# huggingface/tokenizers

Hardware: AMD Instinct MI355X
Metric: GB input text/sec (whole node), GPT-2 BPE encode_batch (higher is better)
Workload: dtype u8->u32

## Files before the change

### tokenizers_amd/csrc/capi/handle.cpp

```cpp

struct Workspace {
    std::mutex mu;
    std::function<uint32_t(uint32_t)> pad_exchange;
    uint32_t h_padmax = 0;
    bool busy = false;
    bool device_bound = false;
    hipStream_t bound_stream = nullptr;
    hipStream_t own_stream = nullptr;
    hipStream_t io_in = nullptr, io_out = nullptr;
    hipEvent_t ev_in[2] = {nullptr, nullptr}, ev_out[2] = {nullptr, nullptr};
    DevBuf w_l3_tiles;
    DevBuf w_ms_dmask, w_pprefix, w_pt_word;
    DevBuf w_docmask, w_startmask, w_wprefix, w_bsum, w_tile_w, w_pt_start, w_tok0, w_pt_tokoff, w_tmp_ids, w_tmp_end, w_rows;
    DevBuf w_len1, w_fin, w_fbsum, w_pad_count, w_keep, w_type_ids2, w_seq_ids2;
    DevBuf w_ovf_parts, w_enc_base, w_enc_doc, w_enc_start, w_enc_cnt;
    DevBuf w_enc_idx, w_enc_win;
    DevBuf w_queues, w_qcount, w_cstate;
    DevBuf w_doc_off;
    DevBuf w_chunk_lo;
    DevBuf w_ids, w_doc_pt, w_tok_offsets, w_scalars, w_offsets, w_word_ids;
    DevBuf dw_ids, dw_tok_off, dw_first, dw_bad, dw_dup, dw_len, dw_bsum, dw_pos, dw_out_off, dw_bytes, dw_total;
    DevBuf w_endmask, w_pt_end, w_keepmask, w_kprefix, w_ntext, w_norig, w_ndoc_off, w_slow_docs, w_leadmask, w_lprefix, w_need, w_need_bsum, w_huge, w_list_huge, w_wbase, w_norig_e, w_ids2, w_tok_offsets2, w_offsets2, w_word_ids2, w_candmask, w_matchmask, w_spanmask, w_stopmask, w_hardmask, w_boundmask, w_bprefix, w_seg_off, w_xseg_off,
        w_match_docs, w_match_list;
    DevBuf h_text, h_doc_off, h_seq_off, h_inp_off;
    DevBuf w_tok_b8;
    DevBuf w_trim1;
    const uint8_t* cur_trim1 = nullptr;
    DevBuf w_cache_keys, w_cache_rows;
    DevBuf w_claims, w_claim_rows, w_claim_pos;
    DevBuf w_phases;
    uint64_t cache_epoch = 0;
    DevBuf w_seq_off, w_seq_tok_off, w_word_idx, w_first_tok;
    std::vector<StageRec> pending;
    const uint8_t* last_text = nullptr;
    const int64_t* last_doc_off = nullptr;
    const int64_t* last_seq_off = nullptr;
    int64_t last_n_seqs = -1;
    const int64_t* last_inp_off = nullptr;
    int64_t last_n_inputs = -1;
    DevBuf w_inp_off;
    DevBuf w_mask_dirty;
    int64_t last_n_bytes = 0;
    uint32_t last_flags = 0;
    tkamd_device_result last_result{};
    int64_t last_n_docs = 0;
    int64_t last_n_enc = -1;
    int last_ntok_slot = 1;
    uint32_t last_counters[CNT_COUNT] = {0};
    bool force_general = false;
    bool last_note_added = false;
    bool last_used_claims = false;
    ~Workspace() {
        if (own_stream) (void)hipStreamDestroy(own_stream);
        if (io_in) (void)hipStreamDestroy(io_in);
        if (io_out) (void)hipStreamDestroy(io_out);
        for (int i = 0; i < 2; ++i) {
            if (ev_in[i]) (void)hipEventDestroy(ev_in[i]);
            if (ev_out[i]) (void)hipEventDestroy(ev_out[i]);
        }
    }
};

struct tkamd_tokenizer {
    HostModel hm;
    int device = -1;
    DevTables dt{};
    std::mutex mu;
    std::condition_variable cv;
    std::vector<std::unique_ptr<Workspace>> pool;
    Workspace* last_used = nullptr;
    DevBuf t_ucc1, t_ucc2;
    DevBuf t_uc1, t_uc2, t_byte_id, t_merges, t_long_blob, t_long_off, t_long_id, t_long_table;
    DevBuf t_hot;
    DevBuf t_shortw, t_shortw_k3, t_shortw_disp;
    DevBuf t_char_id;
    DevBuf t_at_id[2], t_at_flags[2], t_at_blob[2], t_at_off[2], t_at_first[2];
    DevBuf t_pp_single, t_pp_single_plain;
    DevBuf t_pp_pair, t_pp_pair_plain;
    DevBuf t_pp_prefix, t_pp_suffix, t_pp_prefix_ty, t_pp_suffix_ty, t_bn1, t_bn2, t_bn_map, t_merge_disp, t_dec_entry, t_dec_blob, t_trie;
    int n_cu = 256;
    int n_direct = 0;
    int n_hot = 0;
    int cp_grid = 0;
    std::atomic<int> claims_pause{0};
    std::atomic<int> added_spec_pause{0};
    int added_spec_len = 32;
    int claims_pause_len = 32;
    std::atomic<uint32_t> q16_div{4};
    std::atomic<bool> prof{false};
    std::atomic<bool> encode_special{false};
    std::atomic<bool> word_cache{false};
    std::atomic<uint64_t> cache_epoch{1};
    std::vector<tkamd_stage_time> acc;
    std::vector<int> devices;
    std::vector<std::unique_ptr<tkamd_tokenizer>> replicas;
    std::mutex group_mu;
    std::atomic<int> collect{0};
    std::string collect_note;
    std::vector<std::unique_ptr<DevBuf>> g_root;
    std::vector<void*> rccl_comms;
    int64_t shard_min_bytes = 1 << 20;
    std::vector<double> shard_ms;
    std::vector<int64_t> shard_bytes;
};

constexpr size_t PHASE_WGS = 1 << 17;
constexpr size_t MAX_HOST_WORKSPACES = 4;

struct PinnedBlock {
    void* p = nullptr;
    size_t cap = 0;
};
static std::mutex g_pin_mu;
static std::vector<PinnedBlock> g_pin_free;

static PinnedBlock pinned_get(size_t bytes) {
    if (bytes < 64) bytes = 64;
    {
        std::lock_guard<std::mutex> lk(g_pin_mu);
        size_t best = (size_t)-1;
        for (size_t i = 0; i < g_pin_free.size(); ++i)
            if (g_pin_free[i].cap >= bytes && (best == (size_t)-1 || g_pin_free[i].cap < g_pin_free[best].cap)) best = i;
        if (best != (size_t)-1 && g_pin_free[best].cap <= 2 * bytes + (1u << 20)) {
            PinnedBlock b = g_pin_free[best];
            g_pin_free.erase(g_pin_free.begin() + best);
            return b;
        }
    }
    PinnedBlock b;
    size_t want = bytes + bytes / 8;
    HIP_CHECK(hipHostMalloc(&b.p, want, hipHostMallocPortable));
    b.cap = want;
    return b;
}
static void pinned_put(PinnedBlock b) {
    if (!b.p || g_forked) return;
    std::lock_guard<std::mutex> lk(g_pin_mu);
    if (g_pin_free.size() >= 16) { (void)hipHostFree(b.p); return; }
    g_pin_free.push_back(b);
}

struct tkamd_batch {
    int64_t n_docs = 0, n_tokens = 0;
    PinnedBlock ids, tok_offsets, offsets, word_ids, pad_counts, type_ids, seq_ids, enc_docs, enc_parts;
    bool has_offsets = false, has_words = false, has_pads = false, has_types = false, has_enc_docs = false, has_enc_parts = false;
    ~tkamd_batch() { pinned_put(ids); pinned_put(tok_offsets); pinned_put(offsets); pinned_put(word_ids); pinned_put(pad_counts); pinned_put(type_ids); pinned_put(seq_ids); pinned_put(enc_docs); pinned_put(enc_parts); }
};

struct tkamd_text {
    int64_t n_docs = 0, n_bytes = 0;
    PinnedBlock bytes, doc_offsets;
    ~tkamd_text() { pinned_put(bytes); pinned_put(doc_offsets); }
};
```

### tokenizers_amd/csrc/capi/pipeline.cpp

```cpp

int lookup_grid(const tkamd_tokenizer* t) { return std::min(3 * t->n_cu, (int)NSQ); }

struct QueueSizes {
    uint32_t sq_cap[4], row_base[4];
    size_t total;
};
static bool rerun_wanted(tkamd_tokenizer* t, Workspace* w, int raw) {
    const int err = raw & ~NOTE_BITS;
    bool again = false;
    if (raw & NOTE_ADDED_SEEN) { t->added_spec_pause = t->added_spec_len; w->force_general = true; again = true; }
    if (err == ERR_QUEUE_FULL && t->q16_div > 1) { t->q16_div = t->q16_div > 2 ? 2 : 1; again = true; }
    return again;
}

QueueSizes queue_sizes(size_t N, uint32_t q16_div, int grid) {
    QueueSizes z{};
    const size_t n_tiles = N / LOOKUP_TILE_BYTES + 1;
    const size_t per_sq = ((n_tiles + grid - 1) / grid) * LOOKUP_TILE_BYTES;
    z.sq_cap[0] = (uint32_t)(per_sq / q16_div + 64);
    z.sq_cap[1] = (uint32_t)(per_sq / 17 + 16);
    z.sq_cap[2] = (uint32_t)(per_sq / 33 + 16);
    z.sq_cap[3] = (uint32_t)(per_sq / 65 + 16);
    size_t acc = 0;
    for (int c = 0; c < 4; ++c) { z.row_base[c] = (uint32_t)acc; acc += (size_t)z.sq_cap[c] * (size_t)grid; }
    z.total = acc;
    return z;
}

void reserve_workspace(tkamd_tokenizer* t, Workspace* w, int64_t n_bytes, int64_t n_docs, uint32_t flags, bool want_meta) {
    int64_t W = (n_bytes >> 6) + 2;
    size_t N = (size_t)n_bytes;
    w->w_docmask.reserve(W * 8);
    w->w_startmask.reserve(W * 8);
    w->w_wprefix.reserve(W * 4);
    w->w_bsum.reserve((W / 256 + 2) * 4);
    w->w_tok0.reserve((N + 4) * 4);
    w->w_tmp_ids.reserve((N + 4) * 4);
    const QueueSizes z = queue_sizes(N, t->q16_div, lookup_grid(t));
    w->w_rows.reserve(z.total * 16);
    w->w_queues.reserve(z.total * 8);
    w->w_cstate.reserve((N / COMPACT_CHUNK + 4) * 8 + 16);
    w->w_chunk_lo.reserve((N / COMPACT_CHUNK + 4) * 4);
    w->w_qcount.reserve((size_t)QCNT_WORDS * 4);
    w->w_pt_tokoff.reserve((N + 4) * 4);
    w->w_ids.reserve((N + 4) * 4);
    w->w_doc_pt.reserve((n_docs + 2) * 4);
    w->w_tok_offsets.reserve((n_docs + 2) * 8);
    w->w_scalars.reserve(SC_SLOTS * 8);
    if (want_meta) w->w_pt_start.reserve((N + 4) * 4);
    if (flags & TKAMD_OFFSETS_MASK) {
        w->w_tmp_end.reserve((N + 4) * 4);
        w->w_offsets.reserve((N + 4) * 8);
    }
    if (flags & TKAMD_WANT_WORD_IDS) w->w_word_ids.reserve((N + 4) * 4);
}

void run_pipeline(tkamd_tokenizer* t, Workspace* w, const uint8_t* d_text, const int64_t* d_doc_off, int64_t n_docs, int64_t n_bytes,
                  const int64_t* d_seq_off, int64_t n_seqs, uint32_t flags, hipStream_t st, tkamd_device_result* out,
                  const int64_t* d_inp_off = nullptr, int64_t n_inputs = -1) {
    HostModel& hm = t->hm;
    const int64_t* const d_doc_off_in = d_doc_off;
    const int64_t* const d_seq_off_in = d_seq_off;
    const int64_t* const d_inp_off_in = d_inp_off;
    const bool mixed = n_inputs >= 0;
    if (mixed && (flags & TKAMD_PAIRS)) throw Invalid("a mixed batch names the kind of every input itself: TKAMD_PAIRS must not be set");
    if (mixed && !d_inp_off) throw Invalid("null input offsets");
    bool rerun = false;
    const uint32_t off_mode = flags & TKAMD_OFFSETS_MASK;
    const bool want_words = (flags & TKAMD_WANT_WORD_IDS) != 0;
    const bool want_meta = off_mode != TKAMD_OFFSETS_NONE || want_words;
    if (off_mode == 3u) throw Invalid("bad offsets mode");
    const bool add_special = (flags & TKAMD_ADD_SPECIAL) != 0 && !(hm.pp_prefix.empty() && hm.pp_suffix.empty());
    if ((flags & TKAMD_ADD_SPECIAL) && !(flags & TKAMD_PAIRS) && !hm.pp_unsupported.empty()) throw Unsupported("add_special_tokens: " + hm.pp_unsupported);
    if (!(flags & TKAMD_PAIRS) && hm.pp_single_refused) throw Unsupported("post_processor: " + hm.pp_unsupported);
    if (mixed && (flags & TKAMD_ADD_SPECIAL) && !hm.pp_pair_unsupported.empty()) throw Unsupported("add_special_tokens on a pair: " + hm.pp_pair_unsupported);
    const bool prefix_space = hm.byte_level && hm.add_prefix_space;
    const bool metaspace = hm.pretok == PT_METASPACE;
    size_t at_min_len = (size_t)-1;
    for (int c = 0; c < 2; ++c)
        for (size_t k = 0; k + 1 < hm.at[c].off.size(); ++k) at_min_len = std::min<size_t>(at_min_len, hm.at[c].off[k + 1] - hm.at[c].off[k]);
    const bool have_added_tokens = at_min_len != (size_t)-1;
    const uint32_t mcap = have_added_tokens ? (uint32_t)std::min<size_t>((size_t)n_bytes / std::max<size_t>(at_min_len, 1) + 16, 0x7FFFFFF0u) : 0u;
    const int64_t n_x = (hm.norm == NORM_BERT) ? 3 * n_bytes + 64
                        : metaspace ? 3 * n_bytes + 3 * (n_docs + 2 * (int64_t)mcap + 1) + 64
                        : n_bytes + (prefix_space ? n_docs + (int64_t)mcap : 0);
    if (n_x >= (int64_t)0xFFFFFF00ll) throw Invalid("batch larger than 4 GiB: split it (byte offsets are 32-bit on the device)");
    const bool bpe_path = hm.model == MODEL_BPE && !hm.char_bpe && (hm.pretok == PT_BYTELEVEL_GPT2 || hm.pretok == PT_LLAMA3 || hm.pretok == PT_BYTELEVEL_NOREGEX);
    const bool local_pretok = hm.pretok == PT_WHITESPACE || hm.pretok == PT_WHITESPACE_SPLIT || hm.pretok == PT_BERT;
    const bool word_models = (hm.model == MODEL_WORDLEVEL || hm.model == MODEL_WORDPIECE) && local_pretok;
    const bool char_bpe = hm.model == MODEL_BPE && hm.char_bpe && (local_pretok || metaspace);
    if (!bpe_path && !word_models && !char_bpe)
        throw Unsupported("this build covers {ByteLevel(GPT-2 regex), Llama-3 Split+ByteLevel, ByteLevel(no regex)}+BPE and "
                          "{Whitespace,WhitespaceSplit,BertPreTokenizer}+{WordLevel,WordPiece,BPE over characters} and the U+2581 front+BPE over characters");
    if (prefix_space && hm.norm != NORM_NONE) throw Unsupported("ByteLevel add_prefix_space behind a normalizer");

    reserve_workspace(t, w, n_x, n_docs, flags, want_meta);
    int64_t* sc = w->w_scalars.as<int64_t>();
    int64_t* d_npretok = sc + SC_NPRETOK;
    int64_t* d_ntok_total = sc + SC_NTOK;
    int64_t* d_xlen = sc + SC_NKEPT;
    int* d_err = (int*)(sc + SC_ERR);
    uint32_t* d_counters = (uint32_t*)(sc + SC_COUNTERS);
    const int64_t W0 = (n_bytes >> 6) + 1;
    const int64_t W = (n_x >> 6) + 1;
    const int grid = t->n_cu * 8;
    Prof pf{t, w, st};
    using ull = unsigned long long;

    const char* const claims_hook = test_hook("TKAMD_CLAIMS");
    const bool claims_on = !(claims_hook && !strcmp(claims_hook, "0"));
    constexpr bool len_bound = true;
    bool use_claims = claims_on && !t->word_cache &&
                      (hm.model == MODEL_BPE || (hm.model == MODEL_WORDPIECE && hm.max_input_chars >= (uint32_t)WORD_MAX_KEY));
    if (use_claims) {
        int p = t->claims_pause.load();
        while (p > 0 && !t->claims_pause.compare_exchange_weak(p, p - 1)) {}
        if (p > 0) use_claims = false;
    }
    w->last_used_claims = use_claims;
    size_t claim_slots = 0;
    const size_t cstate_bytes = (((size_t)n_x / (size_t)COMPACT_CHUNK + 4) * 8 + 15) & ~(size_t)15;
    {
        ZeroRegions z{};
        z.add(sc, SC_SLOTS * 8);
        if (!(len_bound && (hm.norm == NORM_BERT || metaspace))) z.add(w->w_docmask.p, (size_t)(W + 1) * 8);
        z.add(w->w_qcount.p, (size_t)QCNT_WORDS * 4);
        z.add(w->w_cstate.p, cstate_bytes);
        if (hm.pretok == PT_LLAMA3 && split_rule_fast(hm.split_rule)) {
            w->w_l3_tiles.reserve(l3_tileflag_words(n_x) * 8);
            z.add(w->w_l3_tiles.p, l3_tileflag_words(n_x) * 8);
        }
        if (use_claims) {
            constexpr size_t per_slot = 64;
            int bits = 18;
            while (bits < 24 && ((size_t)1 << bits) < (size_t)n_bytes / per_slot) ++bits;
            claim_slots = (size_t)1 << bits;
            w->w_claims.reserve(claim_slots * 16);
            w->w_claim_rows.reserve(claim_slots * 16);
            z.add(w->w_claims.p, claim_slots * 16);
        }
        launch_zero_regions(st, t->n_cu * 4, z);
    }
    out->d_ids = w->w_ids.as<uint32_t>();
    out->d_tok_offsets = w->w_tok_offsets.as<int64_t>();
    out->d_offsets = nullptr;
    out->d_word_ids = nullptr;
    out->d_n_tokens = d_ntok_total;
    out->d_n_pretokens = d_npretok;
    out->ids_capacity = n_x + 4;
    w->last_n_docs = n_docs;
    w->cur_trim1 = nullptr;
    w->last_n_enc = -1;
    out->d_enc_docs = nullptr;
    out->d_n_encodings = nullptr;
    w->last_seq_off = d_seq_off;
    w->last_n_seqs = n_seqs;
    w->last_inp_off = d_inp_off;
    w->last_n_inputs = n_inputs;
    w->w_doc_off.reserve((size_t)(n_docs + 2) * 8);
    const bool lean = n_bytes > 0 && hm.at[0].size() == 0 && hm.at[1].size() == 0 && hm.norm == NORM_NONE && !prefix_space &&
                      (hm.pretok == PT_BYTELEVEL_GPT2 || hm.pretok == PT_BYTELEVEL_NOREGEX);
    const int64_t* const raw_doc_off = d_doc_off;
    if (!lean) {
        pf.begin("validate_csr");
        launch_validate_csr(st, d_doc_off, n_docs, n_bytes, d_err, w->w_doc_off.as<int64_t>());
        pf.end();
    }
    d_doc_off = w->w_doc_off.as<int64_t>();
    const bool words_in = n_seqs >= 0;
    if (words_in) {
        if (!d_seq_off) throw Invalid("null sequence offsets");
        w->w_seq_off.reserve((size_t)(n_seqs + 2) * 8);
        w->w_seq_tok_off.reserve((size_t)(n_seqs + 2) * 8);
        launch_validate_csr(st, d_seq_off, n_seqs, n_docs, d_err, w->w_seq_off.as<int64_t>());
        d_seq_off = w->w_seq_off.as<int64_t>();
        out->d_tok_offsets = w->w_seq_tok_off.as<int64_t>();
    }
    const int64_t* const e_tok_off = words_in ? w->w_seq_tok_off.as<int64_t>() : w->w_tok_offsets.as<int64_t>();
    const int64_t e_n = words_in ? n_seqs : n_docs;
    if (mixed) {
        w->w_inp_off.reserve((size_t)(n_inputs + 2) * 8);
        launch_validate_csr(st, d_inp_off, n_inputs, e_n, d_err, w->w_inp_off.as<int64_t>());
        d_inp_off = w->w_inp_off.as<int64_t>();
    }
    auto add_specials = [&]() {
        const size_t T2 = (size_t)n_x + 4 + (size_t)(e_n + 1) * (hm.pp_prefix.size() + hm.pp_suffix.size());
        w->w_ids2.reserve(T2 * 4);
        w->w_tok_offsets2.reserve((size_t)(e_n + 2) * 8);
        if (out->d_offsets) w->w_offsets2.reserve(T2 * 8);
        if (out->d_word_ids) w->w_word_ids2.reserve(T2 * 4);
        SpecialArgs sa{};
        sa.tok_offsets = e_tok_off;
        sa.n_docs = e_n;
        sa.ids = w->w_ids.as<uint32_t>();
        sa.offsets = out->d_offsets;
        sa.word_ids = out->d_word_ids;
        sa.prefix = t->t_pp_prefix.as<uint32_t>();
        sa.suffix = t->t_pp_suffix.as<uint32_t>();
        sa.n_prefix = (int32_t)hm.pp_prefix.size();
        sa.n_suffix = (int32_t)hm.pp_suffix.size();
        sa.tok_offsets2 = w->w_tok_offsets2.as<int64_t>();
        sa.ids2 = w->w_ids2.as<uint32_t>();
        sa.offsets2 = w->w_offsets2.as<uint32_t>();
        sa.word_ids2 = w->w_word_ids2.as<uint32_t>();
        sa.n_tok2 = sc + SC_NTOK2;
        pf.begin("add_specials");
        launch_add_specials(st, grid, sa);
        pf.end();
        out->d_ids = sa.ids2;
        out->ids_capacity = (int64_t)T2;
        out->d_tok_offsets = sa.tok_offsets2;
        if (out->d_offsets) out->d_offsets = sa.offsets2;
        if (out->d_word_ids) out->d_word_ids = sa.word_ids2;
        out->d_n_tokens = sa.n_tok2;
    };
    out->d_pad_counts = nullptr;
    out->d_type_ids = nullptr;
    out->d_seq_ids = nullptr;
    const bool pairs = (flags & TKAMD_PAIRS) != 0 || mixed;
    if (pairs && !mixed && (e_n & 1)) throw Invalid("TKAMD_PAIRS: an odd number of documents");
    if (pairs && (flags & TKAMD_ADD_SPECIAL) && !hm.pp_pair_unsupported.empty()) throw Unsupported("add_special_tokens on a pair: " + hm.pp_pair_unsupported);
    const bool typed_single = !pairs && hm.pp_single_typed;
    const bool epilogue = hm.trunc_on || hm.pad_on || pairs || typed_single;
    const bool want_overflow = (flags & TKAMD_WANT_OVERFLOW) != 0 && hm.trunc_on;
    out->d_enc_parts = nullptr;
    auto batch_longest = [&](uint32_t* d_target, bool* again) -> uint64_t {
        int64_t head[SC_PADMAX + 1];
        HIP_CHECK(hipMemcpyAsync(head, sc, sizeof(head), hipMemcpyDeviceToHost, st));
        uint32_t mx = 0;
        if (d_target != (uint32_t*)(sc + SC_PADMAX)) HIP_CHECK(hipMemcpyAsync(&mx, d_target, 4, hipMemcpyDeviceToHost, st));
        HIP_CHECK(hipStreamSynchronize(st));
        if (d_target == (uint32_t*)(sc + SC_PADMAX)) mx = *(const uint32_t*)&head[SC_PADMAX];
        if (!w->pad_exchange) return mx;
        if (rerun_wanted(t, w, *(const int*)&head[SC_ERR])) {
            *again = true;
            return 0;
        }
        const uint32_t all = w->pad_exchange(mx);
        if (all != mx) {
            w->h_padmax = all;
            HIP_CHECK(hipMemcpyAsync(d_target, &w->h_padmax, 4, hipMemcpyHostToDevice, st));
        }
        return all;
    };
    auto finalize_pairs = [&]() {
        const int64_t n_pairs = mixed ? n_inputs : e_n / 2;
        const bool tpl_on = (flags & TKAMD_ADD_SPECIAL) && !hm.pp_pair.empty();
        uint32_t n_special = 0;
        if (tpl_on) for (const HostModel::TplPiece& q : hm.pp_pair) n_special += q.kind == 2u;
        PairArgs pa{};
        pa.tok_offsets = e_tok_off;
        pa.n_pairs = n_pairs;
        if (mixed) {
            pa.inp_off = d_inp_off;
            pa.tpl1 = add_special ? t->t_pp_single.as<uint32_t>() : t->t_pp_single_plain.as<uint32_t>();
            pa.n_tpl1 = add_special ? (int32_t)hm.pp_single.size() : (int32_t)hm.pp_single_plain.size();
            pa.n_special1 = add_special ? (uint32_t)(hm.pp_prefix.size() + hm.pp_suffix.size()) : 0u;
        }
        const uint32_t n_special_max = std::max(n_special, pa.n_special1);
        pa.ids = w->w_ids.as<uint32_t>();
        pa.offsets = out->d_offsets;
        pa.word_ids = out->d_word_ids;
        pa.trim1 = pa.offsets ? w->cur_trim1 : nullptr;
        w->w_keep.reserve((size_t)(std::max(e_n, 2 * n_pairs) + 2) * 4);
        pa.tpl = tpl_on ? t->t_pp_pair.as<uint32_t>() : t->t_pp_pair_plain.as<uint32_t>();
        pa.n_tpl = tpl_on ? (int32_t)hm.pp_pair.size() : (int32_t)hm.pp_pair_plain.size();
        pa.n_special = n_special;
        pa.ovf_ty_tpl = (tpl_on && hm.pp_roberta) ? 1u : 0u;
        pa.trunc_on = hm.trunc_on ? 1u : 0u;
        pa.trunc_max = hm.trunc_max_length;
        pa.trunc_left = hm.trunc_left ? 1u : 0u;
        pa.trunc_strategy = (uint32_t)hm.trunc_strategy;
        pa.trunc_stride = hm.trunc_stride;
        pa.pad_on = hm.pad_on ? 1u : 0u;
        pa.pad_fixed = hm.pad_fixed ? 1u : 0u;
        pa.pad_length = hm.pad_length;
        pa.pad_multiple = hm.pad_multiple;
        pa.pad_left = hm.pad_left ? 1u : 0u;
        pa.pad_id = hm.pad_id;
        pa.pad_type_id = hm.pad_type_id;
        w->w_fbsum.reserve((size_t)((n_pairs + 1) / 256 + 2) * 4);
        pa.keep = w->w_keep.as<uint32_t>();
        pa.bsum = w->w_fbsum.as<uint32_t>();
        pa.target = (uint32_t*)(sc + SC_PADMAX);
        pa.n_tok2 = sc + SC_NTOK2;
        pa.err = d_err;
        for (int32_t k = 0; k < pa.n_tpl; ++k) {
            const uint32_t kind = (tpl_on ? hm.pp_pair : hm.pp_pair_plain)[(size_t)k].kind;
            if (kind < 2u) { pa.first_is_b = kind == 1u ? 1u : 0u; break; }
        }
        pf.begin("pair_epilogue");
        int64_t n_enc = n_pairs;
        bool overflow = want_overflow;
        if (overflow) {
            w->w_ovf_parts.reserve((size_t)(n_pairs + 2) * 4);
            w->w_enc_base.reserve((size_t)(n_pairs + 2) * 8);
            pa.ovf_parts = w->w_ovf_parts.as<uint32_t>();
            pa.enc_base = w->w_enc_base.as<int64_t>();
        } else {
            w->w_len1.reserve((size_t)(n_pairs + 2) * 4);
            pa.len1 = w->w_len1.as<uint32_t>();
        }
        launch_pair_lens(st, pa);
        if (overflow) {
            launch_pair_overflow_scan(st, pa, sc + SC_NENC);
            int64_t head[SC_NENC + 1];
            HIP_CHECK(hipMemcpyAsync(head, sc, sizeof(head), hipMemcpyDeviceToHost, st));
            HIP_CHECK(hipStreamSynchronize(st));
            const int err_now = *(const int*)&head[SC_ERR] & ~NOTE_BITS;
            if (rerun_wanted(t, w, *(const int*)&head[SC_ERR])) {
                rerun = true;
                pf.end();
                return;
            }
// ... 291 lines not shown
    if (have_added) HIP_CHECK(hipMemsetAsync(n_match, 0, 4, st));
    if (spec && setA.size() > 0) {
        pf.begin("added_token_match");
        launch_added_detect(st, args_of(0), d_text, n_bytes, nullptr, d_err);
        pf.end();
    }
    if (have_raw) {
        pf.begin("added_token_match");
        launch_added_match(st, args_of(0), d_text, n_bytes, nullptr, d_doc_off, n_docs, nullptr, nullptr, t->dt.uc1, t->dt.uc2, w->w_candmask.as<ull>(),
                           w->w_match_docs.as<uint32_t>(), d_counters + CNT_MATCH_DOCS, mlist, n_match, mcap, MATCH_LEN_ORIG, d_err);
        pf.end();
    }

    const uint8_t* x_text = d_text;
    bool lead_done = false;
    const int64_t* x_doc_off = d_doc_off;
    const int64_t* x_len_dev = nullptr;
    const uint32_t* norig = nullptr;
    const uint32_t* norig_e = nullptr;
    if (hm.norm == NORM_BERT || prefix_space || metaspace) {
        w->w_ntext.reserve((size_t)n_x + TKAMD_TEXT_PAD);
        w->w_ndoc_off.reserve((size_t)(n_docs + 2) * 8);
        if (hm.norm != NORM_BERT && !metaspace) HIP_CHECK(hipMemsetAsync(w->w_ntext.p, 0, (size_t)n_x + TKAMD_TEXT_PAD, st));
        else if (test_hook("TKAMD_POISON_NTEXT")) {
            HIP_CHECK(hipMemsetAsync(w->w_ntext.p, 0xFF, (size_t)n_x + TKAMD_TEXT_PAD, st));
            if (len_bound) HIP_CHECK(hipMemsetAsync(w->w_docmask.p, 0xFF, w->w_docmask.cap, st));
            HIP_CHECK(hipMemsetAsync(w->w_startmask.p, 0xFF, w->w_startmask.cap, st));
            HIP_CHECK(hipMemsetAsync(w->w_wprefix.p, 0xFF, w->w_wprefix.cap, st));
            if (w->w_endmask.p) HIP_CHECK(hipMemsetAsync(w->w_endmask.p, 0xFF, w->w_endmask.cap, st));
        }
        if (off_mode != TKAMD_OFFSETS_NONE) {
            w->w_norig.reserve(((size_t)n_x + 4) * 4);
            norig = w->w_norig.as<uint32_t>();
            if (hm.norm != NORM_BERT && !metaspace) {
                w->w_norig_e.reserve(((size_t)n_x + 4) * 4);
                norig_e = w->w_norig_e.as<uint32_t>();
            }
        }
    }
    if (hm.norm == NORM_BERT) {
        w->w_keepmask.reserve(bn_olen_bytes(n_bytes));
        w->w_kprefix.reserve((size_t)(W0 + 1) * 4);
        w->w_wbase.reserve((size_t)(W0 + 1) * 4);
        BnTables bt{t->t_bn1.as<uint16_t>(), t->t_bn2.as<uint8_t>(), t->t_bn_map.as<MergeSlot>(), hm.bn_mask, hm.bn_seed,
                    hm.bn_clean_text, hm.bn_handle_chinese, hm.bn_strip_accents, hm.bn_lowercase};
        const ull* verbatim = nullptr;
        if (have_raw) {
            scatter_masks(n_bytes, nullptr, false);
            launch_mask_or2(st, w->w_boundmask.as<ull>(), w->w_matchmask.as<ull>(), w->w_spanmask.as<ull>(), W0 + 1);
            verbatim = w->w_boundmask.as<ull>();
        }
        pf.begin("bert_normalize");
        launch_bert_normalize(st, bt, d_text, n_bytes, d_doc_off, n_docs, verbatim, w->w_keepmask.as<uint8_t>(), w->w_kprefix.as<uint32_t>(),
                              w->w_bsum.as<uint32_t>(), w->w_wbase.as<uint32_t>(), d_xlen, w->w_ntext.as<uint8_t>(), (uint32_t*)norig, (uint32_t*)norig_e,
                              w->w_ndoc_off.as<int64_t>(), d_err);
        launch_zero_tail(st, w->w_ntext.as<uint8_t>(), d_xlen, TKAMD_TEXT_PAD, len_bound ? w->w_docmask.as<ull>() : nullptr, W + 1, t->n_cu * 4);
        pf.end();
        if (have_raw) launch_translate_matches_norm(st, mlist, n_match, w->w_keepmask.as<uint8_t>(), w->w_wbase.as<uint32_t>(), n_bytes, d_xlen);
        x_text = w->w_ntext.as<uint8_t>();
        x_doc_off = w->w_ndoc_off.as<int64_t>();
        x_len_dev = d_xlen;
    }
    const int64_t n_in = hm.norm == NORM_BERT ? n_x : n_bytes;
    if (spec && setB.size() > 0) {
        pf.begin("added_token_match2");
        launch_added_detect(st, args_of(1), x_text, n_in, x_len_dev, d_err);
        pf.end();
    }
    if (have_norm) {
        const int64_t* seg = x_doc_off;
        const int64_t* nseg_dev = nullptr;
        int64_t nseg_bound = n_docs;
        if (have_raw) {
            scatter_masks(n_in, x_len_dev, false);
            seg = build_pieces(x_doc_off, n_in, x_len_dev);
            nseg_dev = d_nseg;
            nseg_bound = (int64_t)seg_cap;
        }
        pf.begin("added_token_match2");
        launch_added_match(st, args_of(1), x_text, n_in, x_len_dev, seg, nseg_bound, nseg_dev, have_raw ? w->w_matchmask.as<ull>() : nullptr, t->dt.uc1, t->dt.uc2,
                           w->w_candmask.as<ull>(), w->w_match_docs.as<uint32_t>(), d_counters + CNT_MATCH_DOCS2, mlist, n_match, mcap,
                           hm.norm == NORM_NONE ? MATCH_LEN_ORIG : 0u, d_err);
        pf.end();
    }
    if (have_added && !prefix_space && !metaspace) {
        scatter_masks(n_in, x_len_dev, off_mode != TKAMD_OFFSETS_NONE);
        matchmask = w->w_matchmask.as<ull>();
    }
    const int64_t* piece_off = nullptr;
    const int64_t* piece_n_dev = nullptr;
    if (prefix_space) {
        const int64_t* seg = d_doc_off;
        const int64_t* nseg_dev = nullptr;
        int64_t nseg_bound = n_docs;
        if (have_added) {
            scatter_masks(n_bytes, nullptr, false);
            seg = build_pieces(d_doc_off, n_bytes, nullptr);
            nseg_dev = d_nseg;
            nseg_bound = (int64_t)seg_cap;
            w->w_xseg_off.reserve((seg_cap + 2) * 8);
        }
        w->w_need.reserve((size_t)(nseg_bound + 2) * 4);
        w->w_need_bsum.reserve((size_t)((nseg_bound + 1) / 256 + 2) * 4);
        int64_t* xseg = have_added ? w->w_xseg_off.as<int64_t>() : w->w_ndoc_off.as<int64_t>();
        pf.begin("prefix_space");
        launch_prefix_space(st, d_text, seg, nseg_bound, nseg_dev, have_added ? w->w_matchmask.as<ull>() : nullptr, w->w_need.as<uint32_t>(),
                            w->w_need_bsum.as<uint32_t>(), xseg, d_xlen, w->w_ntext.as<uint8_t>(), (uint32_t*)norig, (uint32_t*)norig_e, grid);
        if (have_added) {
            launch_prefix_doc_csr(st, d_doc_off, n_docs, w->w_boundmask.as<ull>(), w->w_bprefix.as<uint32_t>(), n_bytes, nullptr, d_nseg, xseg, w->w_ndoc_off.as<int64_t>());
            launch_translate_matches_prefix(st, mlist, n_match, w->w_boundmask.as<ull>(), w->w_bprefix.as<uint32_t>(), n_bytes, nullptr, d_nseg, xseg);
        }
        pf.end();
        x_text = w->w_ntext.as<uint8_t>();
        x_doc_off = w->w_ndoc_off.as<int64_t>();
        x_len_dev = d_xlen;
        if (have_added) {
            scatter_masks(n_x, x_len_dev, off_mode != TKAMD_OFFSETS_NONE);
            matchmask = w->w_matchmask.as<ull>();
            piece_off = xseg;
            piece_n_dev = d_nseg;
        }
    } else if (metaspace) {
        w->w_ms_dmask.reserve((size_t)(W0 + 2) * 8);
        HIP_CHECK(hipMemsetAsync(w->w_ms_dmask.p, 0, (size_t)(W0 + 2) * 8, st));
        launch_mark_doc_starts_n(st, d_doc_off, n_docs, n_bytes, nullptr, w->w_ms_dmask.as<ull>(), d_err);
        const ull* pstart = w->w_ms_dmask.as<ull>();
        if (have_added) {
            scatter_masks(n_bytes, nullptr, false);
            build_pieces(d_doc_off, n_bytes, nullptr);
            pstart = w->w_boundmask.as<ull>();
        }
        w->w_keepmask.reserve(bn_olen_bytes(n_bytes));
        w->w_kprefix.reserve((size_t)(W0 + 1) * 4);
        w->w_wbase.reserve((size_t)(W0 + 1) * 4);
        pf.begin("metaspace");
        launch_metaspace(st, d_text, n_bytes, d_doc_off, n_docs, pstart, w->w_ms_dmask.as<ull>(), have_added ? w->w_matchmask.as<ull>() : nullptr,
                         have_added ? w->w_spanmask.as<ull>() : nullptr, (uint32_t)hm.ms_prepend, w->w_keepmask.as<uint8_t>(), w->w_kprefix.as<uint32_t>(),
                         w->w_bsum.as<uint32_t>(), w->w_wbase.as<uint32_t>(), d_xlen, w->w_ntext.as<uint8_t>(), (uint32_t*)norig, w->w_ndoc_off.as<int64_t>());
        launch_zero_tail(st, w->w_ntext.as<uint8_t>(), d_xlen, TKAMD_TEXT_PAD, len_bound ? w->w_docmask.as<ull>() : nullptr, W + 1, t->n_cu * 4);
        pf.end();
        if (have_added) launch_translate_matches_norm(st, mlist, n_match, w->w_keepmask.as<uint8_t>(), w->w_wbase.as<uint32_t>(), n_bytes, d_xlen);
        x_text = w->w_ntext.as<uint8_t>();
        x_doc_off = w->w_ndoc_off.as<int64_t>();
        x_len_dev = d_xlen;
        if (have_added) {
            scatter_masks(n_x, x_len_dev, off_mode != TKAMD_OFFSETS_NONE);
            matchmask = w->w_matchmask.as<ull>();
        }
    } else if (have_added && hm.pretok == PT_LLAMA3) {
        piece_off = build_pieces(x_doc_off, n_in, x_len_dev);
        piece_n_dev = d_nseg;
    }

    pf.begin("mark_doc_starts");
    launch_mark_doc_starts_n(st, lean ? raw_doc_off : x_doc_off, n_docs, n_x, x_len_dev, w->w_docmask.as<ull>(), d_err);
    if (matchmask) launch_mask_or(st, w->w_docmask.as<ull>(), w->w_hardmask.as<ull>(), W, n_match);
    pf.end();

    uint32_t* pt_end = nullptr;
    bool has_end = false;
    bool meta_masks = false;
    auto after_masks = [&]() {
        if (want_meta && !meta_masks) {
            pf.begin("emit_pretok");
            launch_emit_pretok(st, w->w_startmask.as<ull>(), w->w_wprefix.as<uint32_t>(), n_x, x_len_dev, d_npretok, w->w_pt_start.as<uint32_t>());
            if (pt_end) launch_emit_pretok_end(st, w->w_startmask.as<ull>(), w->w_endmask.as<ull>(), w->w_wprefix.as<uint32_t>(), n_x, x_len_dev, pt_end);
            pf.end();
        }
        pf.begin("doc_first_pretok");
        launch_doc_first_pretok(st, lean ? raw_doc_off : x_doc_off, n_docs, n_x, w->w_startmask.as<ull>(), w->w_wprefix.as<uint32_t>(),
                                d_npretok, w->w_doc_pt.as<uint32_t>(), w->w_chunk_lo.as<uint32_t>(),
                                lean ? d_err : nullptr, lean ? w->w_doc_off.as<int64_t>() : nullptr);
        pf.end();
    };
    if (hm.pretok == PT_BYTELEVEL_GPT2) {
        pf.begin("pretok_gpt2_seq");
        if (off_mode == TKAMD_OFFSETS_CHAR && x_text == d_text && !x_len_dev && n_x == n_bytes) {
            w->w_leadmask.reserve((size_t)(W0 + 1) * 8);
            lead_done = true;
        }
        launch_pretok_gpt2(st, x_text, n_x, x_len_dev, w->w_docmask.as<ull>(), t->dt.uc1, t->dt.uc2, w->w_startmask.as<ull>(), lead_done ? w->w_leadmask.as<ull>() : nullptr);
        pf.end();
    } else if (hm.pretok == PT_LLAMA3) {
        w->w_endmask.reserve((size_t)(W + 1) * 8);
        w->w_slow_docs.reserve((size_t)(n_docs + 1) * 4);
        if (off_mode == TKAMD_OFFSETS_CHAR && x_text == d_text && !x_len_dev && n_x == n_bytes && (split_rule_fast(hm.split_rule) || (split_rule_fast_cs(hm.split_rule) && t->t_ucc1.p))) {
            w->w_leadmask.reserve((size_t)(W0 + 1) * 8);
            lead_done = true;
        }
        pf.begin("pretok_llama3");
        w->w_slow_docs.reserve((size_t)((piece_off ? seg_cap : (size_t)n_docs) + 1) * 4);
        launch_pretok_llama3(st, x_text, n_x, x_len_dev, w->w_docmask.as<ull>(), t->dt.uc1, t->dt.uc2, w->w_startmask.as<ull>(),
                             w->w_endmask.as<ull>(), piece_off ? piece_off : x_doc_off, piece_off ? (int64_t)seg_cap : n_docs, piece_n_dev,
                             w->w_slow_docs.as<uint32_t>(), d_counters + CNT_SLOW_DOCS, hm.split_rule,
                             t->t_ucc1.p ? t->t_ucc1.as<uint16_t>() : nullptr, t->t_ucc2.p ? t->t_ucc2.as<uint8_t>() : nullptr,
                             w->w_l3_tiles.p ? w->w_l3_tiles.as<ull>() : nullptr, lead_done ? w->w_leadmask.as<ull>() : nullptr);
        pf.end();
    } else if (metaspace) {
        pf.begin("metaspace_units");
        launch_ms_units(st, x_text, n_x, x_len_dev, w->w_docmask.as<ull>(), w->w_startmask.as<ull>(), W, hm.ms_split);
        pf.end();
    } else if (hm.pretok == PT_BYTELEVEL_NOREGEX) {
        HIP_CHECK(hipMemcpyAsync(w->w_startmask.p, w->w_docmask.p, (size_t)W * 8, hipMemcpyDeviceToDevice, st));
    } else {
        w->w_endmask.reserve((size_t)(W + 1) * 8);
        has_end = true;
        if (want_meta) {
            w->w_pt_end.reserve(((size_t)n_x + 4) * 4);
            pt_end = w->w_pt_end.as<uint32_t>();
        }
        pf.begin("pretok_local");
        launch_pretok_local(st, (int)hm.pretok, x_text, n_x, x_len_dev, w->w_docmask.as<ull>(), t->dt.uc1, t->dt.uc2,
                            w->w_startmask.as<ull>(), w->w_endmask.as<ull>(), len_bound);
        pf.end();
    }
    if (matchmask)
        launch_apply_matches(st, w->w_startmask.as<ull>(), has_end ? w->w_endmask.as<ull>() : nullptr, matchmask, w->w_spanmask.as<ull>(),
                             w->w_stopmask.as<ull>(), W, n_match);
    {
        pf.begin("mask_scan");
        meta_masks = want_meta && !(hm.char_bpe && !hm.unk_configured && !hm.byte_fallback);
        if (meta_masks) w->w_tile_w.reserve(((size_t)n_x / META_TILE + 4) * 4);
        launch_mask_scan(st, w->w_startmask.as<ull>(), W, w->w_bsum.as<uint32_t>(), w->w_wprefix.as<uint32_t>(), d_npretok, len_bound ? x_len_dev : nullptr,
                         meta_masks ? w->w_tile_w.as<uint32_t>() : nullptr);
        pf.end();
        after_masks();
    }

    const uint32_t* pt_word = nullptr;
    if (metaspace && !hm.ms_split && want_words && !words_in) {
        w->w_pprefix.reserve((size_t)(W + 2) * 4);
        w->w_pt_word.reserve(((size_t)n_x + 4) * 4);
        pf.begin("metaspace_words");
        launch_mask_scan(st, w->w_docmask.as<ull>(), W, w->w_bsum.as<uint32_t>(), w->w_pprefix.as<uint32_t>(), sc + SC_NPIECE, len_bound ? x_len_dev : nullptr);
        launch_ms_piece_rank(st, w->w_startmask.as<ull>(), w->w_wprefix.as<uint32_t>(), w->w_docmask.as<ull>(), w->w_pprefix.as<uint32_t>(), n_x, x_len_dev,
                             w->w_pt_word.as<uint32_t>());
        pf.end();
        pt_word = w->w_pt_word.as<uint32_t>();
    }

    uint32_t* tmp_end = (off_mode != TKAMD_OFFSETS_NONE) ? w->w_tmp_end.as<uint32_t>() : nullptr;
    const size_t N = (size_t)n_x;
    const QueueSizes qz = queue_sizes(N, t->q16_div, lookup_grid(t));
    static const size_t row_limit = [] { const char* e = test_hook("TKAMD_ROW_LIMIT_BITS"); return e ? std::min<size_t>((size_t)1 << std::max(8, atoi(e)), ROW_INDEX_LIMIT) : (size_t)ROW_INDEX_LIMIT; }();
    if (qz.total >= row_limit) throw Invalid("batch too large for the work queues (row indices are 30-bit: about 3 GB of text): split it");
    QueuePlan plan{};
    for (int c = 0; c < 4; ++c) {
        plan.v[c].q = (QItem*)(w->w_queues.as<uint8_t>() + (size_t)qz.row_base[c] * 8);
        plan.v[c].counts = w->w_qcount.as<uint32_t>() + (size_t)c * NSQ * QCNT_STRIDE;
        plan.v[c].sq_cap = qz.sq_cap[c];
        plan.v[c].row_base = qz.row_base[c];
    }
    const ull* endmask = has_end ? w->w_endmask.as<ull>() : nullptr;
    const bool phases_on = test_hook("TKAMD_PHASES") != nullptr;
    auto phases_of = [&](int which) -> void* {
        if (!phases_on) return nullptr;
        if (!w->w_phases.p) {
            w->w_phases.reserve(2 * PHASE_WGS * 64);
            HIP_CHECK(hipMemsetAsync(w->w_phases.p, 0, 2 * PHASE_WGS * 64, st));
        }
        return (uint8_t*)w->w_phases.p + (size_t)which * PHASE_WGS * 64;
    };
    WordCache wc{nullptr, nullptr, nullptr, 0u, nullptr};
    auto open_word_cache = [&]() {
        const size_t slots = (size_t)1 << WORD_CACHE_BITS;
        if (use_claims) {
            uint32_t* cpos = nullptr;
            if (off_mode != TKAMD_OFFSETS_NONE) { w->w_claim_pos.reserve(claim_slots * 4); cpos = w->w_claim_pos.as<uint32_t>(); }
            wc = WordCache{nullptr, w->w_claim_rows.p, (unsigned long long*)w->w_claims.p, (uint32_t)(claim_slots - 1), cpos};
            return;
        }
        if (!t->word_cache || off_mode != TKAMD_OFFSETS_NONE) return;
        w->w_cache_keys.reserve(slots * sizeof(CacheKey));
        w->w_cache_rows.reserve(slots * 16);
        const uint64_t epoch = t->cache_epoch;
        if (w->cache_epoch != epoch) {
            HIP_CHECK(hipMemsetAsync(w->w_cache_keys.p, 0, slots * sizeof(CacheKey), st));
            w->cache_epoch = epoch;
        }
        wc = WordCache{(CacheKey*)w->w_cache_keys.p, w->w_cache_rows.p, nullptr, 0u, nullptr};
    };
    DevTables mdt = t->dt;
    mdt.err = d_err;
    mdt.probes = t->prof ? d_counters + CNT_MERGE_PROBES : nullptr;
    auto set_publish = [&]() {
        if (wc.claims) { mdt.pub_rows = wc.rows; mdt.pub_mask = wc.claim_mask; mdt.pub_pos = wc.claim_pos; }
    };
    if (hm.model == MODEL_BPE) {
        pf.begin("lookup");
        open_word_cache();
        set_publish();
        launch_lookup(st, lookup_grid(t), t->dt, x_text, n_x, x_len_dev, w->w_startmask.as<ull>(), endmask, w->w_wprefix.as<uint32_t>(),
                      w->w_tok0.as<uint32_t>(), plan, d_err, matchmask, t->t_hot.p, wc, 0u, 0u, phases_of(0), d_counters);
        pf.end();
        if (hm.ignore_merges)
            launch_long_vocab3(st, t->n_cu, t->dt, x_text, plan.v[1], plan.v[2], plan.v[3], w->w_rows.p, 0u, d_err, wc);
        const bool lds16 = t->dt.newid_affine && !test_hook("TKAMD_FORCE_LANE_MERGE");
        const bool lds32 = lds16;
        const bool can_one = wc.claims && lds16 && lds32 && !test_hook("TKAMD_MERGE_TWO");
        const char* const pair_hook = test_hook("TKAMD_MERGE_PAIR");
        const bool pair = can_one && !(pair_hook && pair_hook[0] == '0');
        const bool one = can_one && !pair;
        const size_t huge_words = std::min<size_t>((size_t)6 * N + 4096, (size_t)1 << 28);
        const bool huge_possible = N > (size_t)LONG_PT_MAX;
        if (huge_possible) {
            w->w_huge.reserve(huge_words * 4);
            w->w_list_huge.reserve((N / LONG_PT_MAX + 16) * 4);
        } else {
            w->w_huge.reserve(64);
            w->w_list_huge.reserve(64);
        }
        if (hm.char_bpe) {
            auto long_only = [&](const QView& q) {
                launch_bpe_merge_long_only(st, t->n_cu * 2, mdt, x_text, q, w->w_rows.p, w->w_tmp_ids.as<uint32_t>(), tmp_end, w->w_list_huge.as<uint32_t>(), d_counters + CNT_LISTH);
            };
            pf.begin("bpe_merge_lds32");
            if (t->dt.newid_affine) launch_bpe_merge(st, t->n_cu, 6, mdt, x_text, plan.v[1], w->w_rows.p, w->w_tmp_ids.as<uint32_t>(), tmp_end, nullptr);
            else long_only(plan.v[1]);
            pf.end();
            pf.begin("bpe_merge_lds");
            if (t->dt.newid_affine) launch_bpe_merge(st, t->n_cu, 5, mdt, x_text, plan.v[0], w->w_rows.p, w->w_tmp_ids.as<uint32_t>(), tmp_end);
            else long_only(plan.v[0]);
            pf.end();
            pf.begin("bpe_merge_long");
            long_only(plan.v[2]);
            launch_bpe_merge_long(st, t->n_cu, mdt, x_text, plan.v[3], w->w_rows.p, w->w_tmp_ids.as<uint32_t>(), tmp_end, w->w_list_huge.as<uint32_t>(),
                                  d_counters + CNT_LISTH, w->w_huge.as<uint32_t>(), (unsigned long long)(huge_possible ? huge_words : 0),
                                  (unsigned long long*)(sc + SC_HUGE_USED), d_err);
            pf.end();
        } else {
        if (pair) {
            pf.begin("bpe_merge_lds_pair");
            launch_bpe_merge_pair(st, t->n_cu, mdt, x_text, plan.v[0], plan.v[1], w->w_rows.p, w->w_tmp_ids.as<uint32_t>(), tmp_end);
            pf.end();
        } else {
            pf.begin(lds32 ? "bpe_merge_lds32" : "bpe_merge_lane32");
            launch_bpe_merge(st, lds32 ? t->n_cu : grid, lds32 ? 6 : 2, mdt, x_text, plan.v[1], w->w_rows.p, w->w_tmp_ids.as<uint32_t>(), tmp_end, one ? &plan.v[0] : nullptr);
            pf.end();
        }
        if (!can_one) {
            pf.begin(lds16 ? "bpe_merge_lds" : "bpe_merge_lane");
            launch_bpe_merge(st, lds16 ? t->n_cu : grid, lds16 ? 5 : 1, mdt, x_text, plan.v[0], w->w_rows.p, w->w_tmp_ids.as<uint32_t>(), tmp_end);
            pf.end();
        }
        pf.begin("bpe_merge64");
        launch_bpe_merge(st, grid, 64, mdt, x_text, plan.v[2], w->w_rows.p, w->w_tmp_ids.as<uint32_t>(), tmp_end);
        pf.end();
        pf.begin("bpe_merge_long");
        launch_bpe_merge_long(st, t->n_cu, mdt, x_text, plan.v[3], w->w_rows.p,
                              w->w_tmp_ids.as<uint32_t>(), tmp_end, w->w_list_huge.as<uint32_t>(), d_counters + CNT_LISTH, w->w_huge.as<uint32_t>(),
                              (unsigned long long)(huge_possible ? huge_words : 0), (unsigned long long*)(sc + SC_HUGE_USED), d_err);
        pf.end();
        }
        if (wc.keys) {
            pf.begin("word_cache_insert");
            launch_word_cache_insert(st, grid, mdt, x_text, plan.v[0], w->w_rows.p, wc);
            pf.end();
        }
    } else if (hm.model == MODEL_WORDLEVEL) {
        DevTables wt = t->dt;
        wt.ignore_merges = 1;
        pf.begin("wordlevel_lookup");
        launch_lookup(st, lookup_grid(t), wt, x_text, n_x, x_len_dev, w->w_startmask.as<ull>(), endmask, w->w_wprefix.as<uint32_t>(),
                      w->w_tok0.as<uint32_t>(), plan, d_err, matchmask, t->t_hot.p, WordCache{nullptr, nullptr, nullptr, 0u, nullptr}, 0u, 1u, nullptr, nullptr);
        launch_long_vocab3(st, t->n_cu, wt, x_text, plan.v[1], plan.v[2], plan.v[3], w->w_rows.p, 1u, d_err, WordCache{nullptr, nullptr, nullptr, 0u, nullptr});
        pf.end();
    } else {
        const bool shortcut = hm.max_input_chars >= (uint32_t)WORD_MAX_KEY;
        DevTables wt = t->dt;
        wt.ignore_merges = 1;
        wt.long_probe_max_len = hm.max_input_chars;
        if (shortcut) open_word_cache();
        set_publish();
        pf.begin("wordpiece_word_lookup");
        launch_lookup(st, lookup_grid(t), wt, x_text, n_x, x_len_dev, w->w_startmask.as<ull>(), endmask, w->w_wprefix.as<uint32_t>(),
                      w->w_tok0.as<uint32_t>(), plan, d_err, matchmask, t->t_hot.p, wc, shortcut ? 0u : 1u, 0u, phases_of(0), d_counters);
        pf.end();
        pf.begin("wordpiece");
        launch_wordpiece_all(st, grid, t->n_cu, mdt, x_text, plan, w->w_rows.p, w->w_tmp_ids.as<uint32_t>(), tmp_end, d_err);
        pf.end();
        if (wc.keys) {
            pf.begin("word_cache_insert");
            launch_word_cache_insert(st, grid, t->dt, x_text, plan.v[0], w->w_rows.p, wc);
            pf.end();
        }
    }
    if (matchmask)
        launch_apply_match_ids(st, w->w_match_list.as<uint32_t>(), d_counters + CNT_MATCHES, w->w_startmask.as<ull>(),
                               w->w_wprefix.as<uint32_t>(), w->w_tok0.as<uint32_t>());
    uint8_t* tok_b8 = nullptr;
    if (tmp_end) { w->w_tok_b8.reserve((size_t)n_x + 64); tok_b8 = w->w_tok_b8.as<uint8_t>(); }
    pf.begin("compact");
    launch_compact(st, t->cp_grid, w->w_tok0.as<uint32_t>(), w->w_rows.p, wc.rows, w->w_tmp_ids.as<uint32_t>(), d_npretok, w->w_cstate.as<ull>(),
                   d_ntok_total, want_meta ? w->w_pt_tokoff.as<uint32_t>() : nullptr, w->w_ids.as<uint32_t>(), w->w_chunk_lo.as<uint32_t>(),
                   w->w_doc_pt.as<uint32_t>(), n_docs, w->w_tok_offsets.as<int64_t>(), (size_t)t->cp_grid <= PHASE_WGS ? phases_of(1) : nullptr, tok_b8);
    pf.end();
    const uint32_t* word_of_doc = nullptr;
    const int64_t* first_tok = nullptr;
    if (words_in) {
        if (want_words) { w->w_word_idx.reserve((size_t)(n_docs + 2) * 4); word_of_doc = w->w_word_idx.as<uint32_t>(); }
        if (off_mode != TKAMD_OFFSETS_NONE && hm.trim_offsets) { w->w_first_tok.reserve((size_t)(n_docs + 2) * 8); first_tok = w->w_first_tok.as<int64_t>(); }
        launch_seq_regroup(st, d_seq_off, n_seqs, n_docs, w->w_tok_offsets.as<int64_t>(), w->w_seq_tok_off.as<int64_t>(), (uint32_t*)word_of_doc, (int64_t*)first_tok);
    }
    if (want_meta) {
        MetaArgs a{};
        a.word_of_doc = word_of_doc;
        a.pt_word = pt_word;
        a.first_tok = first_tok;
        a.x_text = x_text;
        a.text = d_text;
        a.pt_start = meta_masks ? nullptr : w->w_pt_start.as<uint32_t>();
        a.pt_end = meta_masks ? nullptr : pt_end;
        a.startmask = w->w_startmask.as<ull>();
        a.endmask = has_end ? w->w_endmask.as<ull>() : nullptr;
        a.wprefix = w->w_wprefix.as<uint32_t>();
        a.tile_w = meta_masks ? w->w_tile_w.as<uint32_t>() : nullptr;
        a.n_mask_words = W;
        a.x_len_dev = x_len_dev;
        a.x_len_host = n_x;
        a.n_tok = d_ntok_total;
        a.pt_tokoff = w->w_pt_tokoff.as<uint32_t>();
        a.tmp_end = tmp_end;
        a.tok_b8 = tok_b8;
        a.tok0 = wc.claims ? w->w_tok0.as<uint32_t>() : nullptr;
        a.claim_pos = wc.claims ? wc.claim_pos : nullptr;
        a.n_pretok = d_npretok;
        a.doc_pt = w->w_doc_pt.as<uint32_t>();
        a.chunk_lo = w->w_chunk_lo.as<uint32_t>();
        a.chunk = (uint32_t)COMPACT_CHUNK;
        a.n_docs = n_docs;
        a.x_doc_off = x_doc_off;
        a.doc_off = d_doc_off;
        a.norig = norig;
        a.norig_e = norig_e;
        a.byte_level = hm.byte_level;
        a.snap_chars = hm.byte_level || hm.char_bpe;
        if (hm.char_bpe && !hm.unk_configured && !hm.byte_fallback) {
            a.char_id = t->dt.char_id;
            a.cb = t->dt.cb;
            if (hm.ignore_merges) { a.ww_tok0 = w->w_tok0.as<uint32_t>(); a.ww_rows = w->w_rows.p; a.ww_crows = wc.rows; }
        }
        a.trim_offsets = hm.trim_offsets;
        a.trim_matches_only = !hm.byte_level;
        a.pp_add_prefix_space = hm.pp_add_prefix_space;
        a.want_offsets = off_mode != TKAMD_OFFSETS_NONE;
        a.char_mode = off_mode == TKAMD_OFFSETS_CHAR;
        a.want_words = want_words;
        a.matchmask = matchmask;
        a.uc1 = t->dt.uc1;
        a.uc2 = t->dt.uc2;
        a.offsets = w->w_offsets.as<uint32_t>();
        a.word_ids = w->w_word_ids.as<uint32_t>();
        if (a.want_offsets && a.trim_offsets && a.pp_add_prefix_space && hm.trunc_on) {
            w->w_trim1.reserve((size_t)n_x + 8);
            a.trim1 = w->w_trim1.as<uint8_t>();
            w->cur_trim1 = a.trim1;
        }
        if (a.char_mode) {
            w->w_leadmask.reserve((size_t)(W0 + 1) * 8);
            w->w_lprefix.reserve((size_t)(W0 + 1) * 4);
            pf.begin("leadmask_scan");
            if (!lead_done) launch_leadmask(st, d_text, n_bytes, w->w_leadmask.as<ull>());
            launch_mask_scan(st, w->w_leadmask.as<ull>(), W0, w->w_bsum.as<uint32_t>(), w->w_lprefix.as<uint32_t>(), sc + SC_NCHARS);
            pf.end();
            a.leadmask = w->w_leadmask.as<ull>();
            a.lprefix = w->w_lprefix.as<uint32_t>();
        }
        pf.begin("token_meta");
        launch_token_meta(st, grid, a);
        pf.end();
        if (a.want_offsets) out->d_offsets = a.offsets;
        if (a.want_words) out->d_word_ids = a.word_ids;
    }
    if (pairs) finalize_pairs();
    else if (epilogue) finalize();
    else if (add_special) add_specials();
    if (rerun) {
        run_pipeline(t, w, d_text, d_doc_off_in, n_docs, n_bytes, d_seq_off_in, n_seqs, flags, st, out, d_inp_off_in, n_inputs);
        return;
    }
    w->last_ntok_slot = (add_special || epilogue) ? SC_NTOK2 : SC_NTOK;
    HIP_CHECK(hipGetLastError());
}

int read_scalars(tkamd_tokenizer* t, Workspace* w, hipStream_t st, int64_t* n_tok, int64_t* n_pretok);

int finish_batch(tkamd_tokenizer* t, Workspace* w, hipStream_t st, int64_t* n_tok, int64_t* n_pretok) {
    int bits = read_scalars(t, w, st, n_tok, n_pretok);
    while (rerun_wanted(t, w, bits | (w->last_note_added ? NOTE_ADDED_SEEN : 0))) {
        tkamd_device_result again{};
        run_pipeline(t, w, w->last_text, w->last_doc_off, w->last_n_docs, w->last_n_bytes, w->last_seq_off, w->last_n_seqs, w->last_flags, st, &again,
                     w->last_inp_off, w->last_n_inputs);
        if (again.d_ids != w->last_result.d_ids || again.d_tok_offsets != w->last_result.d_tok_offsets ||
            again.d_offsets != w->last_result.d_offsets || again.d_word_ids != w->last_result.d_word_ids || again.d_pad_counts != w->last_result.d_pad_counts || again.d_type_ids != w->last_result.d_type_ids ||
            again.d_enc_docs != w->last_result.d_enc_docs) {
            if (w->device_bound) throw HipError("result buffers moved while a batch was run again");
            w->last_result = again;
        }
        bits = read_scalars(t, w, st, n_tok, n_pretok);
    }
    return bits;
}

int read_scalars(tkamd_tokenizer* t, Workspace* w, hipStream_t st, int64_t* n_tok, int64_t* n_pretok) {
// ... 55 lines not shown
```

### tokenizers_amd/csrc/kernels.hpp

```cpp
#pragma once
#include <hip/hip_runtime_api.h>
#include <cstdint>

#include "tables.hpp"

namespace tkamd {

struct DevTables {
    const uint16_t* uc1;
    const uint8_t* uc2;
    const uint32_t* byte_id;
    const MergeSlot* merges;
    const uint16_t* merge_disp;
    uint32_t merge_mask, merge_seed, merge_bmask;
    uint32_t newid_affine, newid_base;
    const uint32_t* char_id;
    uint32_t cb;
    int* err;
    uint32_t* probes;
    void* pub_rows;
    uint32_t* pub_pos;
    uint32_t pub_mask;
    uint32_t word_seed;
    const void* shortw;
// ... 96 lines not shown
    uint32_t byte_level, trim_offsets, pp_add_prefix_space, want_offsets, char_mode, want_words;
    uint32_t trim_matches_only;
    uint32_t snap_chars;
    const uint32_t* char_id;
    uint32_t cb;
    const uint32_t* ww_tok0;
    const void* ww_rows;
    const void* ww_crows;
    const unsigned long long* matchmask;
    const uint16_t* uc1;
    const uint8_t* uc2;
    uint32_t* offsets;
    uint32_t* word_ids;
    uint8_t* trim1;
};

struct AddedArgs {
    const uint8_t* blob;
    const uint32_t* off;
    const uint32_t* first;
    const uint32_t* id;
    const uint32_t* flags;
    unsigned long long first_set[4];
    uint32_t n_first;
    uint32_t first_byte[4];
    uint32_t skip_special;
};

struct SpecialArgs {
    const int64_t* tok_offsets;
    int64_t n_docs;
    const uint32_t* ids;
    const uint32_t* offsets;
    const uint32_t* word_ids;
    const uint32_t* prefix;
    const uint32_t* suffix;
    int32_t n_prefix, n_suffix;
    int64_t* tok_offsets2;
    uint32_t* ids2;
    uint32_t* offsets2;
    uint32_t* word_ids2;
    int64_t* n_tok2;
};

struct FinalArgs {
    const int64_t* tok_offsets;
    int64_t n_docs;
    const uint32_t* ids;
    const uint32_t* offsets;
    const uint32_t* word_ids;
    const uint8_t* trim1;
    const uint32_t* prefix;
    const uint32_t* suffix;
    int32_t n_prefix, n_suffix;
    uint32_t trunc_len;
    uint32_t trunc_left;
    uint32_t trunc_needs_pair;
    uint32_t trunc_stride;
    uint32_t pad_on, pad_fixed, pad_length, pad_multiple, pad_left, pad_id;
    uint32_t* ovf_parts;
    int64_t* enc_base;
    uint32_t* enc_doc;
    uint32_t* enc_start;
    uint32_t* enc_cnt;
    uint32_t* len1;
    uint32_t* fin;
    uint32_t* target;
    uint32_t* bsum;
    int64_t* tok_offsets2;
    uint32_t* ids2;
    uint32_t* offsets2;
    uint32_t* word_ids2;
    uint32_t* pad_count;
    int64_t* n_tok2;
    int* err;
    uint8_t* type_ids2;
    uint8_t* seq_ids2;
    const uint8_t* prefix_ty;
    const uint8_t* suffix_ty;
    uint32_t seq_ty;
    uint32_t pad_type_id;
};

struct PairArgs {
    const int64_t* tok_offsets;
    int64_t n_pairs;
    const uint32_t* ids;
    const uint32_t* offsets;
    const uint32_t* word_ids;
    const uint8_t* trim1;
    const uint32_t* tpl;
    int32_t n_tpl;
    uint32_t n_special;
    const int64_t* inp_off;
    const uint32_t* tpl1;
    int32_t n_tpl1;
    uint32_t n_special1;
    uint32_t trunc_on, trunc_max, trunc_left, trunc_strategy, trunc_stride;
    uint32_t pad_on, pad_fixed, pad_length, pad_multiple, pad_left, pad_id, pad_type_id;
    uint32_t* keep;
    uint32_t first_is_b;
    uint32_t ovf_ty_tpl;
    uint32_t* ovf_parts;
    int64_t* enc_base;
    uint32_t* enc_doc;
    uint32_t* enc_idx;
    uint32_t* enc_win;
    uint32_t* len1;
    uint32_t* fin;
    uint32_t* target;
    uint32_t* bsum;
    int64_t* tok_offsets2;
    uint32_t* ids2;
    uint32_t* offsets2;
    uint32_t* word_ids2;
    uint8_t* type_ids2;
    uint8_t* seq_ids2;
    uint32_t* pad_count;
    int64_t* n_tok2;
    int* err;
};

enum : int {
    ERR_BAD_OFFSETS = 1,
    ERR_PRETOKEN_TOO_LONG = 2,
    ERR_ADDED_SPLIT = 4,
    ERR_NON_ASCII_NORM = 8,
    ERR_MISSING_UNK = 16,
    ERR_INTERNAL = 32,
    ERR_QUEUE_FULL = 64,
    ERR_TRUNC_SECOND = 128,
    ERR_TOO_MANY_TOKENS = 256,
    ERR_TRUNC_SHORT = 512,
    ERR_TRUNC_STRIDE = 1024,
    ERR_INPUT_KIND = 8192,
    ERR_UNK_OOV = 4096,
    NOTE_REORDER_SEEN = 2048,
    NOTE_ADDED_SEEN = 16384,
    NOTE_BITS = NOTE_REORDER_SEEN | NOTE_ADDED_SEEN,
    ERR_QUEUE_FULL_PAD = 0,
};

enum : int { CNT_LIST16 = 0, CNT_LIST64 = 1, CNT_LISTL = 2, CNT_LIST32 = 3, CNT_SLOW_DOCS = 4, CNT_CLAIM_CANDS = 5, CNT_CLAIM_SHARED = 6, CNT_LISTH = 7, CNT_MATCH_DOCS = 8,
              CNT_MATCHES = 9, CNT_MATCH_DOCS2 = 10, CNT_CLAIM_GAVE_UP = 11, CNT_MERGE_PROBES = 12, CNT_COUNT = 13 };

constexpr uint32_t MATCH_LEN_ORIG = 0x80000000u;
constexpr int TEXT_PAD = 64;
constexpr int LONG_PT_MAX = 8192;

void launch_mark_doc_starts(hipStream_t st, const int64_t* doc_off, int64_t n_docs, int64_t n_bytes,
                            unsigned long long* docmask, int* err);
void launch_validate_csr(hipStream_t st, const int64_t* doc_off, int64_t n_docs, int64_t n_bytes, int* err, int64_t* san);
void launch_pretok_gpt2(hipStream_t st, const uint8_t* text, int64_t n_bytes, const int64_t* len_dev, const unsigned long long* docmask,
                        const uint16_t* uc1, const uint8_t* uc2, unsigned long long* startmask, unsigned long long* leadmask = nullptr);
void launch_mask_scan(hipStream_t st, const unsigned long long* mask, int64_t n_words, uint32_t* bsum, uint32_t* wprefix,
                      int64_t* total, const int64_t* len_dev = nullptr, uint32_t* tile_w = nullptr);
void launch_emit_pretok(hipStream_t st, const unsigned long long* startmask, const uint32_t* wprefix, int64_t n_bytes,
                        const int64_t* len_dev, const int64_t* n_pretok, uint32_t* pt_start);
void launch_prefix_space(hipStream_t st, const uint8_t* text, const int64_t* seg_off, int64_t n_bound, const int64_t* n_dev, const unsigned long long* matchmask,
                         uint32_t* need, uint32_t* bsum, int64_t* xseg_off, int64_t* x_len, uint8_t* xtext, uint32_t* nos, uint32_t* noe, int grid);
void launch_doc_first_pretok(hipStream_t st, const int64_t* doc_off, int64_t n_docs, int64_t n_bytes,
                             const unsigned long long* startmask, const uint32_t* wprefix, const int64_t* n_pretok, uint32_t* doc_pt, uint32_t* chunk_lo,
                             const int* err = nullptr, int64_t* san = nullptr);
void launch_lookup(hipStream_t st, int grid, const DevTables& t, const uint8_t* text, int64_t n_bytes, const int64_t* len_dev,
                   const unsigned long long* startmask, const unsigned long long* endmask, const uint32_t* wprefix, uint32_t* tok0,
                   const QueuePlan& plan, int* err, const unsigned long long* matchmask, const void* hot, const WordCache& wc,
                   uint32_t no_hits, uint32_t miss_is_unk, void* phases = nullptr, uint32_t* counters = nullptr);
void launch_bpe_merge(hipStream_t st, int grid, int group, const DevTables& t, const uint8_t* text, const QView& v, void* rows,
                      uint32_t* tmp_ids, uint32_t* tmp_end, const QView* also = nullptr);
void launch_bpe_merge_pair(hipStream_t st, int n_cu, const DevTables& t, const uint8_t* text, const QView& v16, const QView& v32, void* rows,
                           uint32_t* tmp_ids, uint32_t* tmp_end);
int pair_merge_occupancy();
inline size_t bn_olen_bytes(int64_t n_bytes) { return (((size_t)n_bytes + 64 + 15) & ~(size_t)15) + ((size_t)n_bytes >> 4) + 64; }
inline uint8_t* bn_ltot_of(uint8_t* olen, int64_t n_bytes) { return olen + (((size_t)n_bytes + 64 + 15) & ~(size_t)15); }
void launch_mark_doc_starts_n(hipStream_t st, const int64_t* doc_off, int64_t n_docs, int64_t n_bytes, const int64_t* len_dev,
                              unsigned long long* docmask, int* err);
void launch_pretok_local(hipStream_t st, int kind, const uint8_t* text, int64_t n_bytes, const int64_t* len_dev, const unsigned long long* docmask,
                         const uint16_t* uc1, const uint8_t* uc2, unsigned long long* startmask, unsigned long long* endmask, bool len_bound = false);
void launch_emit_pretok_end(hipStream_t st, const unsigned long long* startmask, const unsigned long long* endmask,
                            const uint32_t* wprefix, int64_t n_bytes, const int64_t* len_dev, uint32_t* pt_end);
void launch_bert_normalize(hipStream_t st, const BnTables& bt, const uint8_t* text, int64_t n_bytes, const int64_t* doc_off, int64_t n_docs,
                           const unsigned long long* verbatim, uint8_t* olen, uint32_t* wsum, uint32_t* bsum, uint32_t* wbase, int64_t* x_len, uint8_t* ntext,
                           uint32_t* nos, uint32_t* noe, int64_t* ndoc_off, int* err);
void launch_long_vocab3(hipStream_t st, int grid, const DevTables& t, const uint8_t* text, const QView& v1, const QView& v2, const QView& v3, void* rows, uint32_t miss_is_unk,
                        int* err, const WordCache& wc);
void launch_wordpiece_all(hipStream_t st, int grid_short, int grid_long, const DevTables& t, const uint8_t* text, const QueuePlan& plan, void* rows, uint32_t* tmp_ids,
                          uint32_t* tmp_end, int* err);
void launch_pretok_llama3(hipStream_t st, const uint8_t* text, int64_t n_bytes, const int64_t* len_dev, const unsigned long long* docmask,
                          const uint16_t* uc1, const uint8_t* uc2, unsigned long long* startmask, unsigned long long* slowmask,
                          const int64_t* doc_off, int64_t n_docs, const int64_t* n_docs_dev, uint32_t* slow_docs, uint32_t* n_slow_docs,
                          SplitRule rule, const uint16_t* ucc1, const uint8_t* ucc2, unsigned long long* tileflags, unsigned long long* leadmask = nullptr);
inline size_t l3_tileflag_words(int64_t n_bytes) { return (size_t)((n_bytes + 1) / 2048 + 1) / 64 + 2; }
void launch_leadmask(hipStream_t st, const uint8_t* text, int64_t n_bytes, unsigned long long* leadmask);
void launch_seq_regroup(hipStream_t st, const int64_t* seq_off, int64_t n_seqs, int64_t n_words, const int64_t* word_tok_off, int64_t* seq_tok_off, uint32_t* widx,
                        int64_t* first_tok);
void launch_token_meta(hipStream_t st, int grid, const MetaArgs& a);
void launch_add_specials(hipStream_t st, int grid, const SpecialArgs& a);
void launch_add_i64(hipStream_t st, int64_t* data, int64_t n, int64_t delta);
void launch_add_u32(hipStream_t st, uint32_t* data, int64_t n, uint32_t delta);
void launch_final_lens(hipStream_t st, const FinalArgs& a);
void launch_overflow_count(hipStream_t st, const FinalArgs& a, int64_t* n_enc);
void launch_overflow_ranges(hipStream_t st, const FinalArgs& a);
void launch_final_offsets(hipStream_t st, const FinalArgs& a);
void launch_finalize(hipStream_t st, int grid, const FinalArgs& a);
void launch_pair_lens(hipStream_t st, const PairArgs& a);
void launch_pair_overflow_scan(hipStream_t st, const PairArgs& a, int64_t* n_enc);
void launch_pair_ranges(hipStream_t st, const PairArgs& a);
void launch_pair_finalize(hipStream_t st, int grid, const PairArgs& a);
void launch_added_match(hipStream_t st, const AddedArgs& a, const uint8_t* text, int64_t n_bytes, const int64_t* len_dev, const int64_t* seg_off, int64_t n_segs,
                        const int64_t* n_segs_dev, const unsigned long long* skipmask, const uint16_t* uc1, const uint8_t* uc2, unsigned long long* candmask,
                        uint32_t* sents, uint32_t* n_sents, uint32_t* match_list, uint32_t* n_match, uint32_t cap, uint32_t len_flag, int* err);
void launch_added_detect(hipStream_t st, const AddedArgs& a, const uint8_t* text, int64_t n_bytes, const int64_t* len_dev, int* note);
void launch_scatter_matches(hipStream_t st, const uint32_t* list, const uint32_t* n_list, int64_t n_bytes, const int64_t* len_dev, unsigned long long* matchmask,
                            unsigned long long* spanmask, unsigned long long* stopmask, unsigned long long* hardmask, uint32_t* tmp_end, uint32_t* dirty);
void launch_mask_or2(hipStream_t st, unsigned long long* dst, const unsigned long long* a, const unsigned long long* b, int64_t n_words);
void launch_emit_boundaries(hipStream_t st, const unsigned long long* mask, const uint32_t* wprefix, int64_t n_bytes, const int64_t* len_dev, const int64_t* total, int64_t* out);
void launch_metaspace(hipStream_t st, const uint8_t* text, int64_t n_bytes, const int64_t* doc_off, int64_t n_docs, const unsigned long long* pstart,
                      const unsigned long long* dstart, const unsigned long long* mmask, const unsigned long long* smask, uint32_t prepend, uint8_t* olen,
                      uint32_t* wsum, uint32_t* bsum, uint32_t* wbase, int64_t* x_len, uint8_t* xtext, uint32_t* nos, int64_t* xdoc_off);
void launch_ms_units(hipStream_t st, const uint8_t* xtext, int64_t n_x, const int64_t* x_len, const unsigned long long* pmask, unsigned long long* startmask,
                     int64_t n_words, bool split);
void launch_ms_piece_rank(hipStream_t st, const unsigned long long* startmask, const uint32_t* wprefix, const unsigned long long* pmask, const uint32_t* pprefix,
                          int64_t n_x, const int64_t* x_len, uint32_t* pt_word);
void launch_translate_matches_norm(hipStream_t st, uint32_t* list, const uint32_t* n_list, const uint8_t* olen, const uint32_t* wbase, int64_t n_bytes, const int64_t* x_len);
void launch_translate_matches_prefix(hipStream_t st, uint32_t* list, const uint32_t* n_list, const unsigned long long* bmask, const uint32_t* wprefix, int64_t n_bytes,
                                     const int64_t* len_dev, const int64_t* total, const int64_t* xseg_off);
void launch_prefix_doc_csr(hipStream_t st, const int64_t* doc_off, int64_t n_docs, const unsigned long long* bmask, const uint32_t* wprefix, int64_t n_bytes,
                           const int64_t* len_dev, const int64_t* total, const int64_t* xseg_off, int64_t* xdoc_off);
void launch_mask_or(hipStream_t st, unsigned long long* dst, const unsigned long long* src, int64_t n_words, const uint32_t* n_list);
void launch_apply_matches(hipStream_t st, unsigned long long* startmask, unsigned long long* endmask, const unsigned long long* matchmask,
                          const unsigned long long* spanmask, const unsigned long long* stopmask, int64_t n_words, const uint32_t* n_list);
void launch_apply_match_ids(hipStream_t st, const uint32_t* match_list, const uint32_t* n_match, const unsigned long long* startmask,
                            const uint32_t* wprefix, uint32_t* tok0);
void launch_decode(hipStream_t st, const uint32_t* ids, const int64_t* tok_off, int64_t n_docs, int64_t n_tok, const void* entry, uint32_t n_ids,
                   const uint8_t* blob, uint32_t skip_special, uint32_t* firstmask, uint32_t* len, uint32_t* bsum, uint32_t* pos, int64_t* total,
                   int64_t* out_off, uint8_t* out_bytes_or_null, uint32_t from_end = 0, uint32_t* badmask = nullptr, uint32_t* dupmask = nullptr);
int prepare_long_kernel();
void launch_bpe_merge_long(hipStream_t st, int grid, const DevTables& t, const uint8_t* text, const QView& v, void* rows,
                           uint32_t* tmp_ids, uint32_t* tmp_end, uint32_t* list_huge, uint32_t* n_huge,
                           uint32_t* scratch, unsigned long long scratch_words, unsigned long long* scratch_used, int* err);
void launch_bpe_merge_long_only(hipStream_t st, int grid, const DevTables& t, const uint8_t* text, const QView& v, void* rows, uint32_t* tmp_ids, uint32_t* tmp_end,
                                uint32_t* list_huge, uint32_t* n_huge);
void launch_word_cache_insert(hipStream_t st, int grid, const DevTables& t, const uint8_t* text, const QView& v, const void* rows, const WordCache& wc);
void launch_compact(hipStream_t st, int grid, const uint32_t* tok0, const void* rows, const void* cache_rows, const uint32_t* tmp_ids, const int64_t* n_pretok,
                    unsigned long long* state, int64_t* n_tok, uint32_t* pt_tokoff, uint32_t* ids, const uint32_t* chunk_lo, const uint32_t* doc_pt,
                    int64_t n_docs, int64_t* tok_offsets, void* phases = nullptr, uint8_t* tok_b8 = nullptr);
int compact_grid(int n_cu);
void launch_zero_regions(hipStream_t st, int grid, const ZeroRegions& z);
void launch_zero_tail(hipStream_t st, uint8_t* p, const int64_t* len_dev, int n, unsigned long long* mask = nullptr, int64_t mask_words = 0, int grid = 1);
constexpr int CP_ITEMS_PER_LANE = 4;
constexpr int COMPACT_CHUNK = 256 * CP_ITEMS_PER_LANE;
const char* test_hook(const char* name);

}
```

### tokenizers_amd/csrc/kernels/bpe.hip

```cpp


__device__ __forceinline__ void load_key16(const uint8_t* __restrict__ text, uint32_t s, uint32_t len, uint64_t* lo, uint64_t* hi) {
    const Unaligned16 v = *(const Unaligned16*)(text + s);
    uint32_t nl = min(len, 8u), nh = min(len, 16u) - nl;
    uint32_t m0 = nl >= 4 ? 0xFFFFFFFFu : ((1u << (8 * nl)) - 1u);
    uint32_t m1 = nl >= 8 ? 0xFFFFFFFFu : (nl > 4 ? ((1u << (8 * (nl - 4))) - 1u) : 0u);
    uint32_t m2 = nh >= 4 ? 0xFFFFFFFFu : ((1u << (8 * nh)) - 1u);
    uint32_t m3 = nh >= 8 ? 0xFFFFFFFFu : (nh > 4 ? ((1u << (8 * (nh - 4))) - 1u) : 0u);
    *lo = ((uint64_t)(v.b & m1) << 32) | (v.a & m0);
    *hi = ((uint64_t)(v.d & m3) << 32) | (v.c & m2);
}

constexpr uint32_t CLAIM_MAX_LEN = 32u;
constexpr uint32_t CLAIM_KEY_MAX = 15u;
__device__ __forceinline__ uint32_t claim_hash_long(uint32_t h16, uint32_t k4, uint32_t k5, uint32_t k6, uint32_t k7) {
    return mix32(h16 ^ (k4 * 0x9E3779B1u) ^ (k5 * 0x85EBCA77u) ^ (k6 * 0xC2B2AE3Du) ^ (k7 * 0x27D4EB2Fu));
}
__device__ __forceinline__ uint32_t claim_slot(uint32_t h, uint32_t mask) { return (word_hash2(h) >> 7) & mask; }
__device__ __forceinline__ uint32_t claim_slot_of(const uint8_t* __restrict__ text, uint32_t s, uint32_t len, uint32_t seed, uint32_t mask) {
    uint64_t lo, hi;
    load_key16(text, s, min(len, 16u), &lo, &hi);
    uint32_t h = word_hash1(lo, hi, len, seed);
    if (len > 16u) {
        uint64_t lo2, hi2;
        load_key16(text, s + 16u, len - 16u, &lo2, &hi2);
        h = claim_hash_long(h, (uint32_t)lo2, (uint32_t)(lo2 >> 32), (uint32_t)hi2, (uint32_t)(hi2 >> 32));
    }
    return claim_slot(h, mask);
}
__device__ __forceinline__ void claim_publish_item(const uint8_t* __restrict__ text, uint32_t seed, uint32_t s, uint32_t len_word, const uint4& row,
                                                   uint32_t claim_mask, uint4* __restrict__ crows, uint32_t* __restrict__ cpos) {
    if (!(len_word & QLEN_CLAIM)) return;
    const uint32_t slot = claim_slot_of(text, s, qitem_len(len_word), seed, claim_mask);
    crows[slot] = row;
    if (cpos) cpos[slot] = s;
}
#define TKAMD_PUBLISH_ROW(t_, text_, s_, lenw_, row_) do { if ((t_).pub_rows) claim_publish_item((text_), (t_).word_seed, (s_), (lenw_), (row_), (t_).pub_mask, (uint4*)(t_).pub_rows, (t_).pub_pos); } while (0)

__device__ __forceinline__ bool long_probe(const DevTables& t, const uint8_t* __restrict__ w, uint32_t len, uint32_t* id) {
    uint32_t h = long_key_hash_init(len);
    const uint32_t nw = len >> 2, tail = len & 3u, tmask = (1u << (8u * tail)) - 1u;
    for (uint32_t i = 0; i < nw; ++i) h = long_key_hash_step(h, ((const Unaligned4*)(w + 4u * i))->v);
    if (tail) h = long_key_hash_step(h, ((const Unaligned4*)(w + 4u * nw))->v & tmask);
    h &= t.long_mask;
    for (;;) {
        uint32_t e = t.long_table[h];
        if (!e) return false;
        uint32_t o = t.long_off[e - 1], l = t.long_off[e] - o;
        if (l == len) {
            const uint8_t* b = t.long_blob + o;
            uint32_t i = 0;
            while (i < nw && ((const Unaligned4*)(b + 4u * i))->v == ((const Unaligned4*)(w + 4u * i))->v) ++i;
            if (i == nw && (!tail || ((((const Unaligned4*)(b + 4u * nw))->v ^ ((const Unaligned4*)(w + 4u * nw))->v) & tmask) == 0u)) { *id = t.long_id[e - 1]; return true; }
        }
        h = (h + 1) & t.long_mask;
    }
}


__device__ __forceinline__ void merge_probe_d(const DevTables& t, const uint16_t* disp, uint32_t a, uint32_t b, uint32_t* rank, uint32_t* new_id) {
    uint32_t d = disp[merge_hash1(a, b, t.merge_seed) & t.merge_bmask];
    uint4 x = ((const uint4*)t.merges)[ph_slot(merge_hash2(a, b, t.merge_seed), d, t.merge_mask)];
    bool hit = x.x == a && x.y == b;
    *rank = hit ? x.z : RANK_NONE;
    *new_id = hit ? x.w : 0u;
}
__device__ __forceinline__ void merge_probe2_d(const DevTables& t, const uint16_t* disp, uint32_t a1, uint32_t b1, uint32_t a2, uint32_t b2, uint32_t* rank1, uint32_t* rank2) {
    const uint32_t d1 = disp[merge_hash1(a1, b1, t.merge_seed) & t.merge_bmask], d2 = disp[merge_hash1(a2, b2, t.merge_seed) & t.merge_bmask];
    const uint4* const m = (const uint4*)t.merges;
    const uint32_t s1 = ph_slot(merge_hash2(a1, b1, t.merge_seed), d1, t.merge_mask), s2 = ph_slot(merge_hash2(a2, b2, t.merge_seed), d2, t.merge_mask);
    __builtin_amdgcn_sched_barrier(0);
    const uint4 x1 = m[s1], x2 = m[s2];
    __builtin_amdgcn_sched_barrier(0);
    *rank1 = (x1.x == a1 && x1.y == b1) ? x1.z : RANK_NONE;
    *rank2 = (x2.x == a2 && x2.y == b2) ? x2.z : RANK_NONE;
}
__device__ __forceinline__ void merge_probe(const DevTables& t, uint32_t a, uint32_t b, uint32_t* rank, uint32_t* new_id) {
    merge_probe_d(t, t.merge_disp, a, b, rank, new_id);
}

template <int G>
__global__ __launch_bounds__(256) void k_bpe_merge(DevTables t, const uint8_t* __restrict__ text, QView v, uint4* __restrict__ rows,
                                                   uint32_t* __restrict__ tmp_ids, uint32_t* __restrict__ tmp_end) {
    constexpr int GPW = 64 / G;
    __shared__ uint32_t s_qpre[NSQ + 1];
    const int lane = lane_id();
    const int sub = lane / G, c = lane % G, gbase = sub * G;
    const uint32_t n = qview_prefix(v, s_qpre);
    const uint32_t wave_global = blockIdx.x * 4 + (threadIdx.x >> 6);
    const uint32_t n_waves = gridDim.x * 4;
    for (uint32_t base = wave_global * GPW; base < n; base += n_waves * GPW) {
        uint32_t item = base + sub;
        bool valid = item < n;
        uint32_t s = 0, len = 0, pos = 0, lenw = 0;
        if (valid) { pos = qview_pos(s_qpre, v.sq_cap, item); const QItem it = v.q[pos]; s = it.s; lenw = it.len; len = qitem_len(lenw); }
        valid = valid && len != 0u;
        bool act = (uint32_t)c < len;
        uint32_t id = act ? t.byte_id[text[s + c]] : 0xFFFFFFFFu;
        uint64_t am = (len >= 64) ? ~0ull : ((1ull << len) - 1ull);
        uint32_t rank = RANK_NONE, new_id = 0;
        {
            uint32_t nid = (uint32_t)__shfl((int)id, gbase + ((c + 1) % G), 64);
            if ((uint32_t)(c + 1) < len) merge_probe(t, id, nid, &rank, &new_id);
        }
        while (true) {
            uint32_t key = (rank == RANK_NONE) ? 0xFFFFFFFFu : ((rank << 6) | (uint32_t)c);
            uint32_t mn = (G == 16) ? row16_allmin(key) : wave_allmin(key);
            bool has = mn != 0xFFFFFFFFu;
            if (!__any(has)) break;
            uint32_t wpos = mn & 63u;
            uint32_t npos = 0;
            if (has) {
                uint64_t rest = am >> (wpos + 1);
                npos = wpos + 1 + (uint32_t)(__ffsll((unsigned long long)rest) - 1);
                am &= ~(1ull << npos);
                if ((uint32_t)c == wpos) id = new_id;
                if ((uint32_t)c == npos) rank = RANK_NONE;
            }
            uint64_t mine = ((uint32_t)c + 1 < 64u) ? (am >> (c + 1)) : 0ull;
            bool has_next = mine != 0ull;
            uint32_t nx = has_next ? (uint32_t)c + 1 + (uint32_t)(__ffsll((unsigned long long)mine) - 1) : (uint32_t)c;
            uint32_t nid = (uint32_t)__shfl((int)id, gbase + (int)nx, 64);
            bool alive = (am >> c) & 1ull;
            if (has && alive && ((uint32_t)c == wpos || (has_next && nx == wpos))) {
                if (has_next) merge_probe(t, id, nid, &rank, &new_id);
                else rank = RANK_NONE;
            }
        }
        const uint32_t count = (uint32_t)__popcll(am);
        uint32_t r1 = 0, r2 = 0, r3 = 0;
        {
            uint64_t m = am & ~1ull;
            const int p1 = m ? __ffsll((unsigned long long)m) - 1 : 0; m &= m - 1ull;
            const int p2 = m ? __ffsll((unsigned long long)m) - 1 : 0; m &= m - 1ull;
            const int p3 = m ? __ffsll((unsigned long long)m) - 1 : 0;
            r1 = (uint32_t)__shfl((int)id, gbase + p1, 64);
            r2 = (uint32_t)__shfl((int)id, gbase + p2, 64);
            r3 = (uint32_t)__shfl((int)id, gbase + p3, 64);
        }
        bool alive = act && ((am >> c) & 1ull);
        if (valid && alive) {
            uint32_t j = (uint32_t)__popcll(am & ((1ull << c) - 1ull));
            if (j == 0) { const uint4 row_ = make_row(count, s, id, r1, r2, r3); rows[v.row_base + pos] = row_; TKAMD_PUBLISH_ROW(t, text, s, lenw, row_); }
            else if (count > 4u) tmp_ids[s + j] = id;
            if (tmp_end) {
                uint64_t mine = ((uint32_t)c + 1 < 64u) ? (am >> (c + 1)) : 0ull;
                uint32_t endc = mine ? (uint32_t)c + 1 + (uint32_t)(__ffsll((unsigned long long)mine) - 1) : len;
                tmp_end[s + j] = endc;
            }
        }
    }
}
template __global__ void k_bpe_merge<64>(DevTables, const uint8_t*, QView, uint4*, uint32_t*, uint32_t*);

__device__ __forceinline__ uint32_t select_bit32(uint32_t m, uint32_t k) {
    uint32_t pos = 0, c;
    c = __popc(m & 0xFFFFu); if (k >= c) { k -= c; pos += 16; m >>= 16; }
    c = __popc(m & 0xFFu);   if (k >= c) { k -= c; pos += 8;  m >>= 8; }
    c = __popc(m & 0xFu);    if (k >= c) { k -= c; pos += 4;  m >>= 4; }
    c = __popc(m & 0x3u);    if (k >= c) { k -= c; pos += 2;  m >>= 2; }
    c = m & 1u;              if (k >= c) { pos += 1; }
    return pos;
}

template <int S>
__global__ __launch_bounds__(256) void k_bpe_merge_lane(DevTables t, const uint8_t* __restrict__ text, QView v, uint4* __restrict__ rows,
                                                        uint32_t* __restrict__ tmp_ids, uint32_t* __restrict__ tmp_end) {
    __shared__ uint32_t s_qpre[NSQ + 1];
    constexpr uint32_t PB = (S == 16) ? 4 : 5;
    __shared__ uint32_t s_byte_id[256];
    __shared__ uint16_t s_disp[DISP_LDS_MAX];
    __shared__ uint32_t s_hist[S + 1];
    __shared__ uint4 s_sort[256];
    s_byte_id[threadIdx.x] = t.byte_id[threadIdx.x];
    const bool disp_in_lds = t.merge_bmask < (uint32_t)DISP_LDS_MAX;
    if (disp_in_lds)
        for (uint32_t i = threadIdx.x; i <= t.merge_bmask; i += 256) s_disp[i] = t.merge_disp[i];
    __syncthreads();
    const uint16_t* disp = disp_in_lds ? (const uint16_t*)s_disp : t.merge_disp;
    const uint32_t n_items = qview_prefix(v, s_qpre);
    const uint32_t stride = gridDim.x * 256;
    for (uint32_t base = blockIdx.x * 256; base < n_items; base += stride) {
        const uint32_t item = base + threadIdx.x;
        bool valid = item < n_items;
        uint32_t p = 0, s = 0, len = 0, claim = 0;
        if (valid) { p = qview_pos(s_qpre, v.sq_cap, item); const QItem it = v.q[p]; s = it.s; len = qitem_len(it.len); claim = it.len & QLEN_CLAIM; }
        valid = valid && len != 0u;
        {
            __syncthreads();
            if (threadIdx.x <= S) s_hist[threadIdx.x] = 0;
            __syncthreads();
            const uint32_t bin = valid ? len : (uint32_t)S;
            const uint32_t within = atomicAdd(&s_hist[bin], 1u);
            __syncthreads();
            uint32_t before = 0;
            for (uint32_t b = 0; b < bin; ++b) before += s_hist[b];
            const uint32_t slot = before + within;
            s_sort[slot] = make_uint4(p, s, len | claim, valid ? 1u : 0u);
            __syncthreads();
            const uint4 it = s_sort[threadIdx.x];
            p = it.x; s = it.y; len = qitem_len(it.z); claim = it.z & QLEN_CLAIM; valid = it.w != 0u;
        }
        uint64_t key[S / 8];
#pragma unroll
        for (int q = 0; q < S / 8; ++q) key[q] = 0;
        if (valid) {
            load_key16(text, s, min(len, 16u), &key[0], &key[1]);
            if (S == 32 && len > 16) load_key16(text, s + 16, len - 16, &key[S / 8 - 2], &key[S / 8 - 1]);
        }
        uint32_t ids[S], rk[S], nd[S];
#pragma unroll
        for (int i = 0; i < S; ++i) {
            uint32_t b = (uint32_t)((key[i / 8] >> (8 * (i % 8))) & 0xFFu);
            ids[i] = s_byte_id[b];
            rk[i] = RANK_NONE;
            nd[i] = 0;
        }
#pragma unroll
        for (int i = 0; i < S - 1; ++i)
            if ((uint32_t)(i + 1) < len) merge_probe_d(t, disp, ids[i], ids[i + 1], &rk[i], &nd[i]);
        uint32_t n = len;
        uint32_t starts = (len >= 32) ? 0xFFFFFFFFu : ((1u << len) - 1u);
        bool active = valid && len > 1;
        while (__any(active)) {
            if (active) {
                uint32_t best = 0xFFFFFFFFu;
#pragma unroll
                for (int i = 0; i < S - 1; ++i) {
                    uint32_t k = (rk[i] << PB) | (uint32_t)i;
                    if ((uint32_t)(i + 1) < n && rk[i] != RANK_NONE) best = min(best, k);
                }
                if (best == 0xFFFFFFFFu) active = false;
                else {
                    const uint32_t w = best & (uint32_t)(S - 1);
                    uint32_t new_id = 0;
#pragma unroll
                    for (int i = 0; i < S - 1; ++i) new_id = ((uint32_t)i == w) ? nd[i] : new_id;
#pragma unroll
                    for (int i = 0; i < S; ++i) {
                        uint32_t nxt_id = (i + 1 < S) ? ids[i + 1] : 0u;
                        ids[i] = ((uint32_t)i == w) ? new_id : (((uint32_t)i > w) ? nxt_id : ids[i]);
                    }
#pragma unroll
                    for (int i = 0; i < S - 1; ++i) {
                        uint32_t nr = (i + 1 < S - 1) ? rk[i + 1] : RANK_NONE, nn = (i + 1 < S - 1) ? nd[i + 1] : 0u;
                        if ((uint32_t)i >= w) { rk[i] = nr; nd[i] = nn; }
                    }
                    if (tmp_end) starts &= ~(1u << select_bit32(starts, w + 1));
                    n -= 1;
                    uint32_t left = 0, right = 0;
#pragma unroll
                    for (int i = 0; i < S; ++i) {
                        left = ((uint32_t)i + 1 == w) ? ids[i] : left;
                        right = ((uint32_t)i == w + 1) ? ids[i] : right;
                    }
                    uint32_t r1 = RANK_NONE, n1 = 0, r2 = RANK_NONE, n2 = 0;
                    if (w > 0) merge_probe_d(t, disp, left, new_id, &r1, &n1);
                    if (w + 1 < n) merge_probe_d(t, disp, new_id, right, &r2, &n2);
#pragma unroll
                    for (int i = 0; i < S - 1; ++i) {
                        if ((uint32_t)i + 1 == w) { rk[i] = r1; nd[i] = n1; }
                        if ((uint32_t)i == w) { rk[i] = r2; nd[i] = n2; }
                    }
                    if (n < 2) active = false;
                }
            }
        }
        if (valid) {
            if (tmp_end && n >= 2u && n <= 4u) {
                uint32_t m = starts & (starts - 1u);
#pragma unroll
                for (int j = 1; j < 4; ++j)
                    if (m) { ids[j] |= row_boundary(text, s, (uint32_t)(__ffs(m) - 1), true); m &= m - 1u; }
            }
            { const uint4 row_ = make_row(n, s, ids[0], ids[1], ids[2], ids[3]); rows[v.row_base + p] = row_; TKAMD_PUBLISH_ROW(t, text, s, len | claim, row_); }
            if (n > 4u) {
#pragma unroll
                for (int j = 1; j < S; ++j)
                    if ((uint32_t)j < n) tmp_ids[s + j] = ids[j];
            }
            if (tmp_end) {
                uint32_t m = starts & (starts - 1u);
#pragma unroll
                for (int j = 0; j < S; ++j) {
                    if ((uint32_t)j < n) {
                        uint32_t e = m ? (uint32_t)(__ffs(m) - 1) : len;
                        tmp_end[s + j] = e;
                        m &= m - 1u;
                    }
                }
            }
        }
    }
}
template __global__ void k_bpe_merge_lane<16>(DevTables, const uint8_t*, QView, uint4*, uint32_t*, uint32_t*);
template __global__ void k_bpe_merge_lane<32>(DevTables, const uint8_t*, QView, uint4*, uint32_t*, uint32_t*);

template <int S, int NT, int NL, bool SYM_REGS, bool CHARS, bool TWO_Q>
__device__ __forceinline__ void bpe_merge_lds_unit(const DevTables& t, const uint8_t* __restrict__ text, const QView& v, const uint32_t* s_qpre, const uint32_t n_first,
                                                   const QView& v2, const uint32_t* s_qpre2, const uint32_t n_items, const uint32_t base, const uint32_t take,
                                                   uint32_t* lds_words, const uint16_t* const disp, uint32_t* s_probes, uint4* __restrict__ rows,
                                                   uint32_t* __restrict__ tmp_ids, uint32_t* __restrict__ tmp_end) {
    static_assert(NL <= NT && NL % 64 == 0 && 4 * NT <= S * NL, "whole wavefronts hold the words; the sort's items fit the key area");
    constexpr uint32_t PB = (S == 16) ? 4 : 5;
// ... 472 lines not shown
```

### tokenizers_amd/csrc/kernels/bpe_huge.hip

```cpp

constexpr int HUGE_CHUNK = 64;

__device__ __forceinline__ unsigned long long huge_chunk_min(const uint32_t* __restrict__ rnk, uint32_t c, uint32_t len) {
    unsigned long long best = ~0ull;
    uint32_t lo = c * HUGE_CHUNK, hi = min(lo + (uint32_t)HUGE_CHUNK, len);
    for (uint32_t i = lo; i < hi; ++i) {
        uint32_t r = rnk[i];
        if (r != RANK_NONE) { unsigned long long k = ((unsigned long long)r << 32) | i; best = k < best ? k : best; }
    }
    return best;
}

__global__ __launch_bounds__(256) void k_bpe_merge_huge(DevTables t, const uint8_t* __restrict__ text,
                                                        const QItem* __restrict__ q, uint4* __restrict__ rows, uint32_t row_base,
                                                        const uint32_t* __restrict__ list, const uint32_t* __restrict__ n_list,
                                                        uint32_t* __restrict__ tmp_ids, uint32_t* __restrict__ tmp_end,
                                                        uint32_t* __restrict__ scratch, unsigned long long scratch_words,
                                                        unsigned long long* __restrict__ scratch_used, int* __restrict__ err) {
    __shared__ unsigned long long red[4];
    __shared__ unsigned long long base_s;
    __shared__ uint32_t touched[3];
    __shared__ uint32_t cnt_s;
    __shared__ uint32_t wcnt[4];
    const int tid = (int)threadIdx.x;
    __shared__ uint32_t first_s;
    const uint32_t n = *n_list;
    for (uint32_t item = blockIdx.x; item < n; item += gridDim.x) {
        const uint32_t p = list[item];
        const QItem it = q[p];
        const uint32_t s = it.s, len = qitem_len(it.len);
        const uint32_t n_chunks = (len + HUGE_CHUNK - 1) / HUGE_CHUNK;
        const unsigned long long need = 5ull * len + 2ull * n_chunks + 1ull;
        __syncthreads();
        if (tid == 0) base_s = atomicAdd(scratch_used, need);
        __syncthreads();
        if (base_s + need > scratch_words) {
            if (tid == 0) { atomicOr(err, ERR_PRETOKEN_TOO_LONG); rows[row_base + p] = make_uint4(0u, 0u, 0u, 0u); }
            continue;
        }
        uint32_t* sym = scratch + base_s;
        uint32_t* rnk = sym + len;
        uint32_t* nid = rnk + len;
        uint32_t* nxt = nid + len;
        uint32_t* prv = nxt + len;
        unsigned long long* cmin = (unsigned long long*)(prv + len + ((base_s + 5ull * len) & 1ull));
        if (!(t.cb & CB_ON)) {
            for (uint32_t i = tid; i < len; i += 256) {
                sym[i] = t.byte_id[text[s + i]];
                nxt[i] = (i + 1 < len) ? i + 1 : 0xFFFFFFFFu;
                prv[i] = (i > 0) ? i - 1 : 0xFFFFFFFFu;
            }
        } else {
            for (uint32_t i = tid; i < len; i += 256) {
                const uint32_t b0 = text[s + i];
                uint32_t own = CHAR_NONE;
                if ((b0 & 0xC0u) != 0x80u) {
                    const uint32_t cl = b0 < 0x80u ? 1u : b0 < 0xE0u ? 2u : b0 < 0xF0u ? 3u : 4u;
                    uint32_t cp = b0 < 0x80u ? b0 : b0 < 0xE0u ? (b0 & 0x1Fu) : b0 < 0xF0u ? (b0 & 0x0Fu) : (b0 & 0x07u);
                    for (uint32_t q = 1; q < cl; ++q) cp = (cp << 6) | (i + q < len ? (text[s + i + q] & 0x3Fu) : 0u);
                    const uint32_t var = ((i != 0 && (t.cb & CB_PREFIX)) ? 1u : 0u) | ((i + cl >= len && (t.cb & CB_SUFFIX)) ? 2u : 0u);
                    if (cp < 0x110000u) own = t.char_id[(cp << 2) | var];
                }
                nid[i] = own;
                sym[i] = 0xFFFFFFFFu;
                nxt[i] = prv[i] = 0xFFFFFFFFu;
            }
            __syncthreads();
            if (tid == 0) {
                bool unknown = false, prev_unk = false;
                uint32_t last = 0xFFFFFFFFu;
                for (uint32_t i = 0; i < len; ++i) {
                    const uint32_t b0 = text[s + i];
                    const bool lead = (b0 & 0xC0u) != 0x80u;
                    if (lead) unknown = nid[i] == CHAR_NONE;
                    uint32_t id = 0xFFFFFFFFu;
                    if (!unknown) { if (lead) { id = nid[i]; prev_unk = false; } }
                    else if (t.cb & CB_BYTES) { id = t.byte_id[b0]; prev_unk = false; }
                    else if (lead) {
                        if (t.cb & CB_UNK) {
                            if (!(prev_unk && (t.cb & CB_FUSE))) id = t.unk_id;
                            prev_unk = true;
                        } else if (t.cb & CB_UNK_MISSING) atomicOr(err, ERR_UNK_OOV);
                    }
                    if (id != 0xFFFFFFFFu) {
                        sym[i] = id;
                        prv[i] = last;
                        if (last != 0xFFFFFFFFu) nxt[last] = i;
                        last = i;
                    }
                }
            }
        }
        __syncthreads();
        for (uint32_t i = tid; i < len; i += 256) {
            uint32_t r = RANK_NONE, ni = 0;
            const uint32_t j = nxt[i];
            if (sym[i] != 0xFFFFFFFFu && j != 0xFFFFFFFFu) merge_probe(t, sym[i], sym[j], &r, &ni);
            rnk[i] = r;
            nid[i] = ni;
        }
        __syncthreads();
        for (uint32_t c = tid; c < n_chunks; c += 256) cmin[c] = huge_chunk_min(rnk, c, len);
        __syncthreads();
        while (true) {
            unsigned long long best = ~0ull;
            for (uint32_t c = tid; c < n_chunks; c += 256) { unsigned long long k = cmin[c]; best = k < best ? k : best; }
#pragma unroll
            for (int d = 32; d >= 1; d >>= 1) {
                unsigned long long o = __shfl_xor(best, d, 64);
                best = o < best ? o : best;
            }
            if ((tid & 63) == 0) red[tid >> 6] = best;
            __syncthreads();
            unsigned long long m01 = red[0] < red[1] ? red[0] : red[1];
            unsigned long long m23 = red[2] < red[3] ? red[2] : red[3];
            best = m01 < m23 ? m01 : m23;
            __syncthreads();
            if (best == ~0ull) break;
            if (tid == 0) {
                const uint32_t w = (uint32_t)best;
                const uint32_t r = nxt[w], rn = nxt[r], pw = prv[w];
                sym[w] = nid[w];
                rnk[r] = RANK_NONE;
                sym[r] = 0xFFFFFFFFu;
                nxt[w] = rn;
                if (rn != 0xFFFFFFFFu) prv[rn] = w;
                uint32_t r1 = RANK_NONE, n1 = 0, r2 = RANK_NONE, n2 = 0;
                if (pw != 0xFFFFFFFFu) merge_probe(t, sym[pw], sym[w], &r1, &n1);
                if (rn != 0xFFFFFFFFu) merge_probe(t, sym[w], sym[rn], &r2, &n2);
                if (pw != 0xFFFFFFFFu) { rnk[pw] = r1; nid[pw] = n1; }
                rnk[w] = r2;
                nid[w] = n2;
                touched[0] = w / HUGE_CHUNK;
                touched[1] = r / HUGE_CHUNK;
                touched[2] = (pw != 0xFFFFFFFFu) ? pw / HUGE_CHUNK : w / HUGE_CHUNK;
            }
            __syncthreads();
            if (tid < 3) {
                uint32_t c = touched[tid];
                bool dup = (tid == 1 && c == touched[0]) || (tid == 2 && (c == touched[0] || c == touched[1]));
                if (!dup) cmin[c] = huge_chunk_min(rnk, c, len);
            }
            __syncthreads();
        }
        if (tid == 0) cnt_s = 0;
        __syncthreads();
        for (uint32_t base = 0; base < len; base += 256) {
            uint32_t i = base + tid;
            bool alive = i < len && sym[i] != 0xFFFFFFFFu;
            uint64_t bm = __ballot(alive);
            if ((tid & 63) == 0) wcnt[tid >> 6] = (uint32_t)__popcll(bm);
            __syncthreads();
            uint32_t off = cnt_s;
            for (int w = 0; w < (tid >> 6); ++w) off += wcnt[w];
            if (alive) {
                uint32_t j = off + (uint32_t)mbcnt64(bm);
                if (j == 0) first_s = sym[i];
                else tmp_ids[s + j] = sym[i];
                if (tmp_end) { uint32_t e = nxt[i]; tmp_end[s + j] = (e == 0xFFFFFFFFu) ? len : e; }
            }
            __syncthreads();
            if (tid == 0) cnt_s += wcnt[0] + wcnt[1] + wcnt[2] + wcnt[3];
            __syncthreads();
        }
        if (tid == 0) rows[row_base + p] = make_uint4((cnt_s ? first_s : 0u) | (ROW_CNT_MORE << ROW_CNT_SHIFT), s, cnt_s, 0u);
    }
}
```

### tokenizers_amd/csrc/kernels/documents.hip

```cpp

__global__ void k_mark_doc_starts(const int64_t* __restrict__ doc_off, int64_t n_docs, int64_t n_bytes_host,
                                  const int64_t* __restrict__ len_dev,
                                  unsigned long long* __restrict__ docmask, int* __restrict__ err) {
    int64_t d = (int64_t)blockIdx.x * blockDim.x + threadIdx.x;
    if (d > n_docs) return;
    const int64_t n_bytes = len_dev ? *len_dev : n_bytes_host;
    int64_t g = doc_off[d];
    if (d == 0 && g != 0) atomicOr(err, ERR_BAD_OFFSETS);
    if (d == n_docs) {
        if (g != n_bytes) atomicOr(err, ERR_BAD_OFFSETS);
        return;
    }
    int64_t g1 = doc_off[d + 1];
    if (g < 0 || g1 < g || g1 > n_bytes) { atomicOr(err, ERR_BAD_OFFSETS); return; }
    if (docmask && g < n_bytes) atomicOr(&docmask[g >> 6], 1ull << (g & 63));
}
__global__ void k_sanitize_csr(const int64_t* __restrict__ doc_off, int64_t n_docs, int64_t n_bytes, const int* __restrict__ err,
                               int64_t* __restrict__ san) {
    int64_t d = (int64_t)blockIdx.x * blockDim.x + threadIdx.x;
    if (d > n_docs) return;
    const bool bad = (*err & ERR_BAD_OFFSETS) != 0;
    san[d] = bad ? (d == n_docs ? n_bytes : 0) : doc_off[d];
}

__device__ __forceinline__ void pair_probe2(const MergeSlot* __restrict__ tab, uint32_t mask, uint32_t seed, uint32_t a, uint32_t b,
                                            uint32_t* v0, uint32_t* v1) {
    uint4 x = ((const uint4*)tab)[merge_hash1(a, b, seed) & mask];
    uint4 y = ((const uint4*)tab)[merge_hash2(a, b, seed) & mask];
    if (x.x == a && x.y == b) { *v0 = x.z; *v1 = x.w; }
    else if (y.x == a && y.y == b) { *v0 = y.z; *v1 = y.w; }
    else { *v0 = RANK_NONE; *v1 = 0; }
}


__device__ __forceinline__ int added_longest(const AddedArgs& a, const uint8_t* __restrict__ text, int64_t i, int64_t end, uint32_t* len) {
    uint32_t b = text[i];
    int best = -1;
    uint32_t best_len = 0;
    for (uint32_t k = a.first[b]; k < a.first[b + 1]; ++k) {
        uint32_t o = a.off[k], l = a.off[k + 1] - o;
        if (i + l > end || l <= best_len) continue;
        uint32_t j = 1;
        while (j < l && text[i + j] == a.blob[o + j]) ++j;
        if (j == l) { best = (int)k; best_len = l; }
    }
    *len = best_len;
    return best;
}

__global__ __launch_bounds__(256) void k_added_candidates(AddedArgs a, const uint8_t* __restrict__ text, int64_t n_bytes_host,
                                                          const int64_t* __restrict__ len_dev, unsigned long long* __restrict__ candmask, int* __restrict__ note) {
    const int64_t n_bytes = len_dev ? *len_dev : n_bytes_host;
    const int64_t i0 = ((int64_t)blockIdx.x * 256 + threadIdx.x) * 16;
    uint32_t cand = 0u;
    if (i0 < n_bytes) {
        const Unaligned16 t = *(const Unaligned16*)(text + i0);
        const uint32_t x[4] = {t.a, t.b, t.c, t.d};
        bool any = a.n_first > 4u;
        if (!any) {
            uint32_t f = 0u;
            for (uint32_t q = 0; q < a.n_first; ++q) {
                const uint32_t c = a.first_byte[q] * 0x01010101u;
#pragma unroll
                for (int k = 0; k < 4; ++k) { const uint32_t z = x[k] ^ c; f |= (z - 0x01010101u) & ~z; }
            }
            any = (f & 0x80808080u) != 0u;
        }
        if (any) {
            const int nv = (int)min((int64_t)16, n_bytes - i0);
            for (int j = 0; j < nv; ++j) {
                const uint32_t b = (x[j >> 2] >> (8 * (j & 3))) & 0xFFu;
                const unsigned long long set = b < 128u ? (b < 64u ? a.first_set[0] : a.first_set[1]) : (b < 192u ? a.first_set[2] : a.first_set[3]);
                if ((set >> (b & 63u)) & 1ull) { uint32_t l; if (added_longest(a, text, i0 + j, n_bytes, &l) >= 0) cand |= 1u << j; }
            }
        }
    }
    if (note) {
        if (__ballot(cand != 0u) != 0ull && lane_id() == 0) atomicOr(note, NOTE_ADDED_SEEN);
        return;
    }
    unsigned long long m = (unsigned long long)cand << (16 * (threadIdx.x & 3));
    m |= ((unsigned long long)(uint32_t)__shfl_xor((int)(uint32_t)(m >> 32), 1, 64) << 32) | (uint32_t)__shfl_xor((int)(uint32_t)m, 1, 64);
    m |= ((unsigned long long)(uint32_t)__shfl_xor((int)(uint32_t)(m >> 32), 2, 64) << 32) | (uint32_t)__shfl_xor((int)(uint32_t)m, 2, 64);
    if ((threadIdx.x & 3) == 0 && i0 <= n_bytes_host) candmask[i0 >> 6] = m;
}

__device__ __forceinline__ void mask_set_range(unsigned long long* m, int64_t a, int64_t b) {
    for (int64_t w = a >> 6; a < b && w <= (b - 1) >> 6; ++w) {
        int64_t lo = w << 6, hi = lo + 64;
        unsigned long long v = ~0ull;
        if (a > lo) v &= ~0ull << (a - lo);
        if (b < hi) v &= ~0ull >> (hi - b);
        atomicOr(&m[w], v);
    }
}

__global__ void k_added_resolve(AddedArgs a, const uint8_t* __restrict__ text, const int64_t* __restrict__ seg_off,
                                const uint32_t* __restrict__ sents, const uint32_t* __restrict__ n_sents,
                                const unsigned long long* __restrict__ candmask, const unsigned long long* __restrict__ skipmask,
                                const uint16_t* __restrict__ uc1, const uint8_t* __restrict__ uc2,
                                uint32_t* __restrict__ match_list, uint32_t* __restrict__ n_match, uint32_t cap, uint32_t len_flag, int* __restrict__ err) {
    const uint32_t n = *n_sents;
    for (uint32_t q = blockIdx.x * blockDim.x + threadIdx.x; q < n; q += gridDim.x * blockDim.x) {
        const int64_t da = seg_off[sents[q]], db = seg_off[sents[q] + 1];
        if (db <= da) continue;
        if (skipmask && ((skipmask[da >> 6] >> (da & 63)) & 1ull)) continue;
        int64_t cursor = da, start_offset = da;
        uint32_t prev = 0xFFFFFFFFu;
        for (int64_t w = da >> 6; w <= (db - 1) >> 6; ++w) {
            unsigned long long cm = candmask[w];
            while (cm) {
                const int64_t pos = (w << 6) + (__ffsll((unsigned long long)cm) - 1);
                cm &= cm - 1;
                if (pos < cursor || pos < da || pos >= db) continue;
                uint32_t len;
                const int k = added_longest(a, text, pos, db, &len);
                if (k < 0) continue;
                int64_t start = pos, stop = pos + len;
                cursor = stop;
                const uint32_t fl = a.flags[k];
                if ((fl & 8u) && a.skip_special) continue;
                if (fl & 1u) {
                    bool ok = true;
                    if (start > da) {
                        int64_t p = start - 1;
                        while (p > da && (text[p] & 0xC0u) == 0x80u) --p;
                        uint32_t l2;
                        ok = !(uc_flags(utf8_global(text, p, &l2), uc1, uc2) & UC_RX_W);
                    }
                    if (ok && stop < db) { uint32_t l2; ok = !(uc_flags(utf8_global(text, stop, &l2), uc1, uc2) & UC_RX_W); }
                    if (!ok) continue;
                }
                if (fl & 2u) {
                    int64_t ns = start;
                    while (ns > da) {
                        int64_t p = ns - 1;
                        while (p > da && (text[p] & 0xC0u) == 0x80u) --p;
                        uint32_t l2;
                        if (!(uc_flags(utf8_global(text, p, &l2), uc1, uc2) & UC_RX_S)) break;
                        ns = p;
                    }
                    start = ns > start_offset ? ns : start_offset;
                }
                if (fl & 4u) {
                    while (stop < db) {
                        uint32_t l2;
                        if (!(uc_flags(utf8_global(text, stop, &l2), uc1, uc2) & UC_RX_S)) break;
                        stop += l2;
                    }
                }
                if (prev != 0xFFFFFFFFu && start < start_offset) match_list[4 * prev + 1] = (uint32_t)start;
                if (stop <= start) {
                    if (stop < start) atomicOr(err, ERR_ADDED_SPLIT);
                    start_offset = stop > start_offset ? stop : start_offset;
                    continue;
                }
                const uint32_t mi = atomicAdd(n_match, 1u);
                if (mi < cap) {
                    match_list[4 * mi] = (uint32_t)start;
                    match_list[4 * mi + 1] = (uint32_t)stop;
                    match_list[4 * mi + 2] = a.id[k];
                    match_list[4 * mi + 3] = (uint32_t)(stop - start) | len_flag;
                    prev = mi;
                } else atomicOr(err, ERR_INTERNAL);
                start_offset = stop;
            }
        }
    }
// ... 145 lines not shown
```

### tokenizers_amd/csrc/kernels/launch.hip

```cpp

void launch_mark_doc_starts_n(hipStream_t st, const int64_t* doc_off, int64_t n_docs, int64_t n_bytes, const int64_t* len_dev,
                              unsigned long long* docmask, int* err) {
    hipLaunchKernelGGL(k_mark_doc_starts, dim3(blocks_for(n_docs + 1, 256)), dim3(256), 0, st, doc_off, n_docs, n_bytes, len_dev, docmask, err);
}
void launch_mark_doc_starts(hipStream_t st, const int64_t* doc_off, int64_t n_docs, int64_t n_bytes,
                            unsigned long long* docmask, int* err) {
    launch_mark_doc_starts_n(st, doc_off, n_docs, n_bytes, nullptr, docmask, err);
}
void launch_validate_csr(hipStream_t st, const int64_t* doc_off, int64_t n_docs, int64_t n_bytes, int* err, int64_t* san) {
    hipLaunchKernelGGL(k_mark_doc_starts, dim3(blocks_for(n_docs + 1, 256)), dim3(256), 0, st, doc_off, n_docs, n_bytes, (const int64_t*)nullptr,
                       (unsigned long long*)nullptr, err);
    hipLaunchKernelGGL(k_sanitize_csr, dim3(blocks_for(n_docs + 1, 256)), dim3(256), 0, st, doc_off, n_docs, n_bytes, (const int*)err, san);
}
void launch_pretok_gpt2(hipStream_t st, const uint8_t* text, int64_t n_bytes, const int64_t* len_dev, const unsigned long long* docmask,
                        const uint16_t* uc1, const uint8_t* uc2, unsigned long long* startmask, unsigned long long* leadmask) {
    if (leadmask) hipLaunchKernelGGL((k_pretok_gpt2_seq<SQ_LUT_COPIES, true>), dim3(blocks_for(n_bytes + 1, 256 * SQ_MAIN)), dim3(256), 0, st, text, n_bytes, len_dev, docmask, uc1, uc2, startmask, leadmask);
    else hipLaunchKernelGGL((k_pretok_gpt2_seq<SQ_LUT_COPIES, false>), dim3(blocks_for(n_bytes + 1, 256 * SQ_MAIN)), dim3(256), 0, st, text, n_bytes, len_dev, docmask, uc1, uc2, startmask, (unsigned long long*)nullptr);
}
void launch_mask_scan(hipStream_t st, const unsigned long long* mask, int64_t n_words, uint32_t* bsum, uint32_t* wprefix,
                      int64_t* total, const int64_t* len_dev, uint32_t* tile_w) {
    unsigned nb = blocks_for(n_words, 256 * WS_PER);
    hipLaunchKernelGGL(k_words_reduce, dim3(nb), dim3(256), 0, st, mask, n_words, bsum, len_dev);
    hipLaunchKernelGGL(k_scan_single, dim3(1), dim3(1024), 0, st, bsum, (int64_t)nb, (const int64_t*)nullptr, (int64_t)1, total);
    hipLaunchKernelGGL(k_words_down, dim3(nb), dim3(256), 0, st, mask, n_words, (const uint32_t*)bsum, wprefix, len_dev, tile_w);
}
void launch_emit_pretok(hipStream_t st, const unsigned long long* startmask, const uint32_t* wprefix, int64_t n_bytes,
                        const int64_t* len_dev, const int64_t* n_pretok, uint32_t* pt_start) {
    hipLaunchKernelGGL(k_emit_pretok, dim3(blocks_for(n_bytes + 1, 4 * 4096)), dim3(256), 0, st, startmask, wprefix, n_bytes, len_dev, n_pretok, pt_start);
}
void launch_doc_first_pretok(hipStream_t st, const int64_t* doc_off, int64_t n_docs, int64_t n_bytes,
                             const unsigned long long* startmask, const uint32_t* wprefix, const int64_t* n_pretok, uint32_t* doc_pt, uint32_t* chunk_lo,
                             const int* err, int64_t* san) {
    hipLaunchKernelGGL(k_doc_first_pretok, dim3(blocks_for(n_docs + 1, 256)), dim3(256), 0, st, doc_off, n_docs, n_bytes, startmask, wprefix, n_pretok, doc_pt, chunk_lo,
                       (uint32_t)COMPACT_CHUNK, err, san);
}

void launch_lookup(hipStream_t st, int grid, const DevTables& t, const uint8_t* text, int64_t n_bytes, const int64_t* len_dev,
                   const unsigned long long* startmask, const unsigned long long* endmask, const uint32_t* wprefix, uint32_t* tok0,
                   const QueuePlan& plan, int* err, const unsigned long long* matchmask, const void* hot, const WordCache& wc,
                   uint32_t no_hits, uint32_t miss_is_unk, void* phases, uint32_t* counters) {
    LookupArgs a{};
    a.counters = counters;
    a.shortw = (const uint4*)t.shortw;
    a.shortw_mask = t.shortw_mask;
    a.shortw_bmask = t.shortw_bmask;
    a.shortw_disp = t.shortw_disp;
    a.shortw_k3 = t.shortw_k3;
    a.word_seed = t.word_seed;
    a.any_hit_final = t.ignore_merges;
    a.unk_id = t.unk_id;
    a.has_unk = t.has_unk;
    a.text = text;
    a.n_bytes_host = n_bytes;
    a.len_dev = len_dev;
    a.startmask = startmask;
    a.endmask = endmask;
    a.wprefix = wprefix;
    a.tok0 = tok0;
    for (int c = 0; c < 4; ++c) a.v[c] = plan.v[c];
    a.err = err;
    a.matchmask = matchmask;
    a.hot = (const uint4*)hot;
    a.cache_keys = wc.keys;
    a.claims = wc.claims;
    a.claim_mask = wc.claim_mask;
    a.no_hits = no_hits;
    a.miss_is_unk = miss_is_unk;
    a.phases = (unsigned long long*)phases;
    const int lds = lookup_lds_bytes();
    if (phases) { if (endmask) hipLaunchKernelGGL((k_lookup<true, true>), dim3(grid), dim3(LU_NT), lds, st, a); else hipLaunchKernelGGL((k_lookup<false, true>), dim3(grid), dim3(LU_NT), lds, st, a); }
    else if (endmask) hipLaunchKernelGGL((k_lookup<true, false>), dim3(grid), dim3(LU_NT), lds, st, a);
    else hipLaunchKernelGGL((k_lookup<false, false>), dim3(grid), dim3(LU_NT), lds, st, a);
}
void launch_bpe_merge(hipStream_t st, int grid, int group, const DevTables& t, const uint8_t* text, const QView& v, void* rows,
                      uint32_t* tmp_ids, uint32_t* tmp_end, const QView* also) {
    uint4* r = (uint4*)rows;
    const QView none{};
    const bool disp_fits = t.merge_bmask < (uint32_t)DISP_LDS_MAX;
    if (group == 5 && disp_fits) launch_lds_merge<16, 640, true, true>(st, grid * 2, t, text, v, none, r, tmp_ids, tmp_end);
    else if (group == 5) launch_lds_merge<16, 640, false, true>(st, grid * 2, t, text, v, none, r, tmp_ids, tmp_end);
    else if (group == 6 && disp_fits) launch_lds_merge<32, 768, true, true>(st, grid, t, text, v, also ? *also : none, r, tmp_ids, tmp_end);
    else if (group == 6) launch_lds_merge<32, 768, false, true>(st, grid, t, text, v, also ? *also : none, r, tmp_ids, tmp_end);
    else if (group == 1)
        hipLaunchKernelGGL(k_bpe_merge_lane<16>, dim3(grid), dim3(256), 0, st, t, text, v, r, tmp_ids, tmp_end);
    else if (group == 2)
        hipLaunchKernelGGL(k_bpe_merge_lane<32>, dim3(grid), dim3(256), 0, st, t, text, v, r, tmp_ids, tmp_end);
    else
        hipLaunchKernelGGL(k_bpe_merge<64>, dim3(grid), dim3(256), 0, st, t, text, v, r, tmp_ids, tmp_end);
}
void launch_bpe_merge_pair(hipStream_t st, int n_cu, const DevTables& t, const uint8_t* text, const QView& v16, const QView& v32, void* rows,
                           uint32_t* tmp_ids, uint32_t* tmp_end) {
    launch_lds_merge_pair(st, n_cu, t, text, v16, v32, (uint4*)rows, tmp_ids, tmp_end);
}
template <int KIND>
static void launch_pretok_local_t(hipStream_t st, const uint8_t* text, int64_t n_bytes, const int64_t* len_dev, const unsigned long long* docmask,
                                  const uint16_t* uc1, const uint8_t* uc2, unsigned long long* startmask, unsigned long long* endmask, bool len_bound) {
    hipLaunchKernelGGL(k_pretok_local_lane<KIND>, dim3(blocks_for(n_bytes + 2, 256 * PLW_MAIN)), dim3(256), 0, st, text, n_bytes, len_dev, docmask, uc1, uc2, startmask, endmask,
                       (len_bound && len_dev) ? 1 : 0);
}
void launch_pretok_local(hipStream_t st, int kind, const uint8_t* text, int64_t n_bytes, const int64_t* len_dev, const unsigned long long* docmask,
                         const uint16_t* uc1, const uint8_t* uc2, unsigned long long* startmask, unsigned long long* endmask, bool len_bound) {
    if (kind == PT_WHITESPACE) launch_pretok_local_t<PT_WHITESPACE>(st, text, n_bytes, len_dev, docmask, uc1, uc2, startmask, endmask, len_bound);
    else if (kind == PT_WHITESPACE_SPLIT) launch_pretok_local_t<PT_WHITESPACE_SPLIT>(st, text, n_bytes, len_dev, docmask, uc1, uc2, startmask, endmask, len_bound);
    else launch_pretok_local_t<PT_BERT>(st, text, n_bytes, len_dev, docmask, uc1, uc2, startmask, endmask, len_bound);
}
void launch_emit_pretok_end(hipStream_t st, const unsigned long long* startmask, const unsigned long long* endmask,
                            const uint32_t* wprefix, int64_t n_bytes, const int64_t* len_dev, uint32_t* pt_end) {
    hipLaunchKernelGGL(k_emit_pretok_end, dim3(blocks_for(n_bytes + 64, 4 * 4096)), dim3(256), 0, st, startmask, endmask, wprefix, n_bytes, len_dev, pt_end);
}
void launch_bert_normalize(hipStream_t st, const BnTables& bt, const uint8_t* text, int64_t n_bytes, const int64_t* doc_off, int64_t n_docs,
                           const unsigned long long* verbatim, uint8_t* olen, uint32_t* wsum, uint32_t* bsum, uint32_t* wbase, int64_t* x_len, uint8_t* ntext,
                           uint32_t* nos, uint32_t* noe, int64_t* ndoc_off, int* err) {
    const int64_t n_words = (n_bytes >> 6) + 1;
    uint8_t* const ltot = bn_ltot_of(olen, n_bytes);
    const BnOlen ol{olen, ltot};
    hipLaunchKernelGGL(k_bn_count, dim3(blocks_for(n_bytes + 1, 256 * BN_LANE)), dim3(256), 0, st, bt, text, n_bytes, verbatim, olen, ltot, wsum, err);

    unsigned nb = blocks_for(n_words, 256);
    hipLaunchKernelGGL(k_u32_reduce, dim3(nb), dim3(256), 0, st, (const uint32_t*)wsum, n_words, bsum);
    hipLaunchKernelGGL(k_scan_single, dim3(1), dim3(1024), 0, st, bsum, (int64_t)nb, (const int64_t*)nullptr, (int64_t)1, x_len);
    hipLaunchKernelGGL(k_u32_down, dim3(nb), dim3(256), 0, st, (const uint32_t*)wsum, n_words, (const uint32_t*)bsum, wbase);
    hipLaunchKernelGGL(k_bn_write, dim3(blocks_for(n_bytes, 256 * BN_LANE)), dim3(256), 0, st, bt, text, n_bytes, verbatim, ol, (const uint32_t*)wbase, ntext, nos, noe);
    hipLaunchKernelGGL(k_bn_reorder_fix, dim3(std::min<unsigned>(blocks_for(n_bytes + 1, 256), 2048u)), dim3(256), 0, st, bt, text, n_bytes, verbatim, doc_off, n_docs,
                       ol, (const uint32_t*)wbase, ntext, nos, noe, err);
    hipLaunchKernelGGL(k_bn_doc_offsets, dim3(blocks_for(n_docs + 1, 256)), dim3(256), 0, st, doc_off, n_docs, n_bytes, ol,
                       (const uint32_t*)wbase, (const int64_t*)x_len, ndoc_off);
}
void launch_metaspace(hipStream_t st, const uint8_t* text, int64_t n_bytes, const int64_t* doc_off, int64_t n_docs, const unsigned long long* pstart,
                      const unsigned long long* dstart, const unsigned long long* mmask, const unsigned long long* smask, uint32_t prepend, uint8_t* olen,
                      uint32_t* wsum, uint32_t* bsum, uint32_t* wbase, int64_t* x_len, uint8_t* xtext, uint32_t* nos, int64_t* xdoc_off) {
    const int64_t n_words = (n_bytes >> 6) + 1;
    uint8_t* const ltot = bn_ltot_of(olen, n_bytes);
    const BnOlen ol{olen, ltot};
    const MsArgs a{text, n_bytes, pstart, dstart, mmask, smask, prepend};
    hipLaunchKernelGGL(k_ms_count, dim3(blocks_for(n_bytes + 1, 256 * BN_LANE)), dim3(256), 0, st, a, olen, ltot, wsum);
    unsigned nb = blocks_for(n_words, 256);
    hipLaunchKernelGGL(k_u32_reduce, dim3(nb), dim3(256), 0, st, (const uint32_t*)wsum, n_words, bsum);
    hipLaunchKernelGGL(k_scan_single, dim3(1), dim3(1024), 0, st, bsum, (int64_t)nb, (const int64_t*)nullptr, (int64_t)1, x_len);
    hipLaunchKernelGGL(k_u32_down, dim3(nb), dim3(256), 0, st, (const uint32_t*)wsum, n_words, (const uint32_t*)bsum, wbase);
    hipLaunchKernelGGL(k_ms_write, dim3(blocks_for(n_bytes, 256 * BN_LANE)), dim3(256), 0, st, a, ol, (const uint32_t*)wbase, xtext, nos);
    hipLaunchKernelGGL(k_bn_doc_offsets, dim3(blocks_for(n_docs + 1, 256)), dim3(256), 0, st, doc_off, n_docs, n_bytes, ol,
                       (const uint32_t*)wbase, (const int64_t*)x_len, xdoc_off);
}
void launch_ms_units(hipStream_t st, const uint8_t* xtext, int64_t n_x, const int64_t* x_len, const unsigned long long* pmask, unsigned long long* startmask,
                     int64_t n_words, bool split) {
    hipLaunchKernelGGL(k_ms_units, dim3(blocks_for(n_words, 256)), dim3(256), 0, st, xtext, n_x, x_len, pmask, startmask, n_words, split ? 1u : 0u);
}
void launch_ms_piece_rank(hipStream_t st, const unsigned long long* startmask, const uint32_t* wprefix, const unsigned long long* pmask, const uint32_t* pprefix,
                          int64_t n_x, const int64_t* x_len, uint32_t* pt_word) {
    hipLaunchKernelGGL(k_ms_piece_rank, dim3(blocks_for((n_x >> 6) + 1, 256)), dim3(256), 0, st, startmask, wprefix, pmask, pprefix, n_x, x_len, pt_word);
}
void launch_long_vocab3(hipStream_t st, int grid, const DevTables& t, const uint8_t* text, const QView& v1, const QView& v2, const QView& v3, void* rows, uint32_t miss_is_unk,
                        int* err, const WordCache& wc) {
    hipLaunchKernelGGL(k_long_vocab3, dim3(3 * grid), dim3(256), 0, st, t, text, v1, v2, v3, (uint4*)rows, miss_is_unk, err, wc.claim_mask,
                       wc.claims ? (uint4*)wc.rows : (uint4*)nullptr, wc.claim_pos);
}
void launch_wordpiece_all(hipStream_t st, int grid_short, int grid_long, const DevTables& t, const uint8_t* text, const QueuePlan& plan, void* rows, uint32_t* tmp_ids,
                          uint32_t* tmp_end, int* err) {
    hipLaunchKernelGGL(k_wordpiece_all, dim3(3 * grid_long + grid_short), dim3(256), 0, st, t, text, plan.v[0], plan.v[1], plan.v[2], plan.v[3], (uint4*)rows, tmp_ids, tmp_end, err,
                       (uint32_t)(3 * grid_long));
}
void launch_pretok_llama3(hipStream_t st, const uint8_t* text, int64_t n_bytes, const int64_t* len_dev, const unsigned long long* docmask,
                          const uint16_t* uc1, const uint8_t* uc2, unsigned long long* startmask, unsigned long long* slowmask,
                          const int64_t* doc_off, int64_t n_docs, const int64_t* n_docs_dev, uint32_t* slow_docs, uint32_t* n_slow_docs,
                          SplitRule rule, const uint16_t* ucc1, const uint8_t* ucc2, unsigned long long* tileflags, unsigned long long* leadmask) {
    const L3Seq q{uc1, uc2, ucc1, ucc2, rule};
    const unsigned doc_blocks = std::min<unsigned>(blocks_for(n_docs, 256), 4096u);
    if (split_rule_fast(rule)) {
        if (leadmask) hipLaunchKernelGGL((k_pretok_llama3_lane<false, true>), dim3(blocks_for(n_bytes + 1, 256 * L3W_MAIN)), dim3(256), 0, st, text, n_bytes, len_dev, docmask, uc1, uc2, startmask, slowmask, rule,
                           (const uint16_t*)nullptr, (const uint8_t*)nullptr, tileflags, leadmask);
        else hipLaunchKernelGGL((k_pretok_llama3_lane<false, false>), dim3(blocks_for(n_bytes + 1, 256 * L3W_MAIN)), dim3(256), 0, st, text, n_bytes, len_dev, docmask, uc1, uc2, startmask, slowmask, rule,
                           (const uint16_t*)nullptr, (const uint8_t*)nullptr, tileflags, (unsigned long long*)nullptr);
        const unsigned n_tiles = blocks_for(n_bytes + 1, PT_TILE);
        hipLaunchKernelGGL(k_pretok_llama3, dim3(tileflags ? blocks_for(n_tiles, 64) : n_tiles), dim3(256), 0, st, text, n_bytes, len_dev, docmask, uc1, uc2, startmask, slowmask,
                           (const unsigned long long*)tileflags, rule);
        hipLaunchKernelGGL(k_l3_slow_docs, dim3(doc_blocks), dim3(256), 0, st, (const unsigned long long*)slowmask, doc_off, n_docs, n_docs_dev, slow_docs, n_slow_docs);
        hipLaunchKernelGGL(k_pretok_llama3_slow, dim3(1024), dim3(64), 0, st, text, doc_off, (const uint32_t*)slow_docs, (const uint32_t*)n_slow_docs, q, startmask);
    } else if (split_rule_fast_cs(rule) && ucc1) {
        if (leadmask) hipLaunchKernelGGL((k_pretok_llama3_lane<true, true>), dim3(blocks_for(n_bytes + 1, 256 * L3W_MAIN)), dim3(256), 0, st, text, n_bytes, len_dev, docmask, uc1, uc2, startmask, slowmask, rule, ucc1, ucc2,
                           (unsigned long long*)nullptr, leadmask);
        else hipLaunchKernelGGL((k_pretok_llama3_lane<true, false>), dim3(blocks_for(n_bytes + 1, 256 * L3W_MAIN)), dim3(256), 0, st, text, n_bytes, len_dev, docmask, uc1, uc2, startmask, slowmask, rule, ucc1, ucc2,
                           (unsigned long long*)nullptr, (unsigned long long*)nullptr);
        hipLaunchKernelGGL(k_l3_slow_docs, dim3(doc_blocks), dim3(256), 0, st, (const unsigned long long*)slowmask, doc_off, n_docs, n_docs_dev, slow_docs, n_slow_docs);
        hipLaunchKernelGGL(k_pretok_llama3_slow, dim3(1024), dim3(64), 0, st, text, doc_off, (const uint32_t*)slow_docs, (const uint32_t*)n_slow_docs, q, startmask);
    } else {
        (void)hipMemsetAsync(startmask, 0, (size_t)((n_bytes >> 6) + 1) * 8, st);
        hipLaunchKernelGGL(k_l3_slow_docs, dim3(doc_blocks), dim3(256), 0, st, (const unsigned long long*)nullptr, doc_off, n_docs, n_docs_dev, slow_docs, n_slow_docs);
        hipLaunchKernelGGL(k_pretok_llama3_slow, dim3(8192), dim3(64), 0, st, text, doc_off, (const uint32_t*)slow_docs, (const uint32_t*)n_slow_docs, q, startmask);
    }
}
void launch_leadmask(hipStream_t st, const uint8_t* text, int64_t n_bytes, unsigned long long* leadmask) {
    hipLaunchKernelGGL(k_leadmask, dim3(blocks_for(n_bytes + 64, 256 * 16)), dim3(256), 0, st, text, n_bytes, leadmask);
}
void launch_seq_regroup(hipStream_t st, const int64_t* seq_off, int64_t n_seqs, int64_t n_words, const int64_t* word_tok_off, int64_t* seq_tok_off, uint32_t* widx,
                        int64_t* first_tok) {
    hipLaunchKernelGGL(k_seq_tok_offsets, dim3(blocks_for(n_seqs + 1, 256)), dim3(256), 0, st, seq_off, n_seqs, word_tok_off, seq_tok_off);
    if ((widx || first_tok) && n_words)
        hipLaunchKernelGGL(k_word_index, dim3(blocks_for(n_words, 256)), dim3(256), 0, st, seq_off, n_seqs, n_words, widx, (const int64_t*)seq_tok_off, first_tok);
}
template <bool E, bool S, bool C, bool M, bool N>
static void launch_tm(hipStream_t st, int grid, const MetaArgs& a) {
    static const int per_cu = [] {
        int n = 0;
        if (hipOccupancyMaxActiveBlocksPerMultiprocessor(&n, (const void*)k_token_meta<E, S, C, M, N>, 256, 0) != hipSuccess || n < 1) n = 4;
        return std::min(n, 8);
    }();
    hipLaunchKernelGGL((k_token_meta<E, S, C, M, N>), dim3(std::max(1, grid / 8) * per_cu), dim3(256), 0, st, a);
}
void launch_token_meta(hipStream_t st, int grid, const MetaArgs& a) {
    if (a.char_id) { hipLaunchKernelGGL(k_token_meta_seq, dim3(grid), dim3(256), 0, st, a); return; }
    const bool simple = !a.norig && !a.matchmask && !a.trim_offsets && !a.word_of_doc && !a.first_tok && a.x_doc_off == a.doc_off && a.x_text == a.text;
    const bool chars = simple && a.char_mode && a.want_offsets;
    const bool masks = !a.pt_start;
    const bool ends = a.pt_end || (masks && a.endmask);
    const bool norig_simple = masks && a.norig && !a.norig_e && !a.trim_offsets && !a.word_of_doc && !a.first_tok;
#define TKAMD_TM(E, S, C, M) launch_tm<E, S, C, M, false>(st, grid, a)
    if (norig_simple) { if (ends) launch_tm<true, true, false, true, true>(st, grid, a); else launch_tm<false, true, false, true, true>(st, grid, a); }
    else if (ends && masks) { if (chars) TKAMD_TM(true, true, true, true); else if (simple) TKAMD_TM(true, true, false, true); else TKAMD_TM(true, false, false, true); }
    else if (ends) { if (chars) TKAMD_TM(true, true, true, false); else if (simple) TKAMD_TM(true, true, false, false); else TKAMD_TM(true, false, false, false); }
    else if (masks) { if (chars) TKAMD_TM(false, true, true, true); else if (simple) TKAMD_TM(false, true, false, true); else TKAMD_TM(false, false, false, true); }
    else { if (chars) TKAMD_TM(false, true, true, false); else if (simple) TKAMD_TM(false, true, false, false); else TKAMD_TM(false, false, false, false); }
#undef TKAMD_TM
}
void launch_prefix_space(hipStream_t st, const uint8_t* text, const int64_t* seg_off, int64_t n_bound, const int64_t* n_dev, const unsigned long long* matchmask,
                         uint32_t* need, uint32_t* bsum, int64_t* xseg_off, int64_t* x_len, uint8_t* xtext, uint32_t* nos, uint32_t* noe, int grid) {
    unsigned nb = blocks_for(n_bound + 1, 256);
    hipLaunchKernelGGL(k_prefix_need, dim3(nb), dim3(256), 0, st, text, seg_off, n_bound, n_dev, matchmask, need);
    hipLaunchKernelGGL(k_u32_reduce, dim3(nb), dim3(256), 0, st, (const uint32_t*)need, n_bound + 1, bsum);
    hipLaunchKernelGGL(k_scan_single, dim3(1), dim3(1024), 0, st, bsum, (int64_t)nb, (const int64_t*)nullptr, (int64_t)1, x_len);
    hipLaunchKernelGGL(k_prefix_doc_offsets, dim3(nb), dim3(256), 0, st, (const uint32_t*)need, n_bound, n_dev, (const uint32_t*)bsum, seg_off, xseg_off, x_len);
    hipLaunchKernelGGL(k_prefix_copy, dim3(grid), dim3(256), 0, st, text, seg_off, (const int64_t*)xseg_off, n_bound, n_dev, xtext, nos, noe);
}
void launch_add_u32(hipStream_t st, uint32_t* data, int64_t n, uint32_t delta) {
    if (n > 0) hipLaunchKernelGGL(k_add_u32, dim3(blocks_for(n, 256)), dim3(256), 0, st, data, n, delta);
}
void launch_add_i64(hipStream_t st, int64_t* data, int64_t n, int64_t delta) {
    hipLaunchKernelGGL(k_add_i64, dim3(blocks_for(n, 256)), dim3(256), 0, st, data, n, delta);
}
void launch_added_match(hipStream_t st, const AddedArgs& a, const uint8_t* text, int64_t n_bytes, const int64_t* len_dev, const int64_t* seg_off, int64_t n_segs,
                        const int64_t* n_segs_dev, const unsigned long long* skipmask, const uint16_t* uc1, const uint8_t* uc2, unsigned long long* candmask,
                        uint32_t* sents, uint32_t* n_sents, uint32_t* match_list, uint32_t* n_match, uint32_t cap, uint32_t len_flag, int* err) {
    hipLaunchKernelGGL(k_added_candidates, dim3(blocks_for(n_bytes + 1, 256 * 16)), dim3(256), 0, st, a, text, n_bytes, len_dev, candmask, (int*)nullptr);
    hipLaunchKernelGGL(k_l3_slow_docs, dim3(std::min<unsigned>(blocks_for(n_segs, 256), 4096u)), dim3(256), 0, st, (const unsigned long long*)candmask, seg_off, n_segs, n_segs_dev, sents, n_sents);
    hipLaunchKernelGGL(k_added_resolve, dim3(1024), dim3(64), 0, st, a, text, seg_off, (const uint32_t*)sents, (const uint32_t*)n_sents,
                       (const unsigned long long*)candmask, skipmask, uc1, uc2, match_list, n_match, cap, len_flag, err);
}
void launch_added_detect(hipStream_t st, const AddedArgs& a, const uint8_t* text, int64_t n_bytes, const int64_t* len_dev, int* note) {
    hipLaunchKernelGGL(k_added_candidates, dim3(blocks_for(n_bytes + 1, 256 * 16)), dim3(256), 0, st, a, text, n_bytes, len_dev, (unsigned long long*)nullptr, note);
}
void launch_scatter_matches(hipStream_t st, const uint32_t* list, const uint32_t* n_list, int64_t n_bytes, const int64_t* len_dev, unsigned long long* matchmask,
                            unsigned long long* spanmask, unsigned long long* stopmask, unsigned long long* hardmask, uint32_t* tmp_end, uint32_t* dirty) {
    hipLaunchKernelGGL(k_scatter_matches, dim3(256), dim3(256), 0, st, list, n_list, n_bytes, len_dev, matchmask, spanmask, stopmask, hardmask, tmp_end, dirty);
}
void launch_mask_or2(hipStream_t st, unsigned long long* dst, const unsigned long long* a, const unsigned long long* b, int64_t n_words) {
    hipLaunchKernelGGL(k_mask_or2, dim3(blocks_for(n_words, 256)), dim3(256), 0, st, dst, a, b, n_words);
}
void launch_emit_boundaries(hipStream_t st, const unsigned long long* mask, const uint32_t* wprefix, int64_t n_bytes, const int64_t* len_dev, const int64_t* total, int64_t* out) {
    hipLaunchKernelGGL(k_emit_boundaries, dim3(blocks_for((n_bytes >> 6) + 2, 256)), dim3(256), 0, st, mask, wprefix, n_bytes, len_dev, total, out);
}
void launch_translate_matches_norm(hipStream_t st, uint32_t* list, const uint32_t* n_list, const uint8_t* olen, const uint32_t* wbase, int64_t n_bytes, const int64_t* x_len) {
    hipLaunchKernelGGL(k_translate_matches_norm, dim3(256), dim3(256), 0, st, list, n_list, BnOlen{olen, bn_ltot_of((uint8_t*)olen, n_bytes)}, wbase, n_bytes, x_len);
}
void launch_translate_matches_prefix(hipStream_t st, uint32_t* list, const uint32_t* n_list, const unsigned long long* bmask, const uint32_t* wprefix, int64_t n_bytes,
                                     const int64_t* len_dev, const int64_t* total, const int64_t* xseg_off) {
    hipLaunchKernelGGL(k_translate_matches_prefix, dim3(256), dim3(256), 0, st, list, n_list, bmask, wprefix, n_bytes, len_dev, total, xseg_off);
}
void launch_prefix_doc_csr(hipStream_t st, const int64_t* doc_off, int64_t n_docs, const unsigned long long* bmask, const uint32_t* wprefix, int64_t n_bytes,
                           const int64_t* len_dev, const int64_t* total, const int64_t* xseg_off, int64_t* xdoc_off) {
    hipLaunchKernelGGL(k_prefix_doc_csr, dim3(blocks_for(n_docs + 1, 256)), dim3(256), 0, st, doc_off, n_docs, bmask, wprefix, n_bytes, len_dev, total, xseg_off, xdoc_off);
}
void launch_mask_or(hipStream_t st, unsigned long long* dst, const unsigned long long* src, int64_t n_words, const uint32_t* n_list) {
    hipLaunchKernelGGL(k_mask_or, dim3(blocks_for(n_words, 256)), dim3(256), 0, st, dst, src, n_words, n_list);
}
void launch_apply_matches(hipStream_t st, unsigned long long* startmask, unsigned long long* endmask, const unsigned long long* matchmask,
                          const unsigned long long* spanmask, const unsigned long long* stopmask, int64_t n_words, const uint32_t* n_list) {
    hipLaunchKernelGGL(k_apply_matches, dim3(blocks_for(n_words, 256)), dim3(256), 0, st, startmask, endmask, matchmask, spanmask, stopmask, n_words, n_list);
}
void launch_apply_match_ids(hipStream_t st, const uint32_t* match_list, const uint32_t* n_match, const unsigned long long* startmask,
                            const uint32_t* wprefix, uint32_t* tok0) {
    hipLaunchKernelGGL(k_apply_match_ids, dim3(64), dim3(256), 0, st, match_list, n_match, startmask, wprefix, tok0);
}
int long_kernel_lds_bytes() { return LONG_PT_MAX * (4 + 4 + 4 + 2 + 2); }
int prepare_long_kernel() {
    int rc = (int)hipFuncSetAttribute((const void*)k_bpe_merge_long, hipFuncAttributeMaxDynamicSharedMemorySize, long_kernel_lds_bytes());
#define TKAMD_LU_ATTR(E, P) if (rc == 0) rc = (int)hipFuncSetAttribute((const void*)k_lookup<E, P>, hipFuncAttributeMaxDynamicSharedMemorySize, lookup_lds_bytes())
    TKAMD_LU_ATTR(true, false); TKAMD_LU_ATTR(false, false); TKAMD_LU_ATTR(true, true); TKAMD_LU_ATTR(false, true);
#undef TKAMD_LU_ATTR
    if (rc == 0) rc = prepare_lds_merge<16, 640, true, true>();
    if (rc == 0) rc = prepare_lds_merge<32, 768, true, true>();
    if (rc == 0) rc = prepare_lds_merge<16, 640, false, true>();
    if (rc == 0) rc = prepare_lds_merge<32, 768, false, true>();
    if (rc == 0) rc = prepare_pair_merge();
    return rc;
}
void launch_bpe_merge_long(hipStream_t st, int grid, const DevTables& t, const uint8_t* text, const QView& v, void* rows,
                           uint32_t* tmp_ids, uint32_t* tmp_end, uint32_t* list_huge, uint32_t* n_huge,
                           uint32_t* scratch, unsigned long long scratch_words, unsigned long long* scratch_used, int* err) {
    hipLaunchKernelGGL(k_bpe_merge_long, dim3(grid), dim3(256), long_kernel_lds_bytes(), st, t, text, v, (uint4*)rows, tmp_ids, tmp_end, list_huge, n_huge);
    hipLaunchKernelGGL(k_bpe_merge_huge, dim3(64), dim3(256), 0, st, t, text, (const QItem*)v.q, (uint4*)rows, v.row_base, (const uint32_t*)list_huge,
                       (const uint32_t*)n_huge, tmp_ids, tmp_end, scratch, scratch_words, scratch_used, err);
}
void launch_bpe_merge_long_only(hipStream_t st, int grid, const DevTables& t, const uint8_t* text, const QView& v, void* rows, uint32_t* tmp_ids, uint32_t* tmp_end,
                                uint32_t* list_huge, uint32_t* n_huge) {
    hipLaunchKernelGGL(k_bpe_merge_long, dim3(grid), dim3(256), long_kernel_lds_bytes(), st, t, text, v, (uint4*)rows, tmp_ids, tmp_end, list_huge, n_huge);
}
void launch_zero_tail(hipStream_t st, uint8_t* p, const int64_t* len_dev, int n, unsigned long long* mask, int64_t mask_words, int grid) {
    hipLaunchKernelGGL(k_zero_tail, dim3(mask ? std::max(1, grid) : 1), dim3(256), 0, st, p, len_dev, n, mask, mask_words);
}
void launch_zero_regions(hipStream_t st, int grid, const ZeroRegions& z) {
    if (z.n > 0) hipLaunchKernelGGL(k_zero_regions, dim3(grid), dim3(256), 0, st, z);
}
int compact_grid(int n_cu) {
    int per_cu = 0;
    if (hipOccupancyMaxActiveBlocksPerMultiprocessor(&per_cu, (const void*)k_compact<CP_ITEMS_PER_LANE>, CP_NT, 0) != hipSuccess || per_cu < 1) per_cu = 1;
    per_cu = std::min(per_cu, 32 / (CP_NT / 64));
    return per_cu * n_cu;
}
void launch_word_cache_insert(hipStream_t st, int grid, const DevTables& t, const uint8_t* text, const QView& v, const void* rows, const WordCache& wc) {
    hipLaunchKernelGGL(k_word_cache_insert, dim3(grid), dim3(256), 0, st, t, text, v, (const uint4*)rows, wc);
}
void launch_compact(hipStream_t st, int grid, const uint32_t* tok0, const void* rows, const void* cache_rows, const uint32_t* tmp_ids, const int64_t* n_pretok,
                    unsigned long long* state, int64_t* n_tok, uint32_t* pt_tokoff, uint32_t* ids, const uint32_t* chunk_lo, const uint32_t* doc_pt,
                    int64_t n_docs, int64_t* tok_offsets, void* phases, uint8_t* tok_b8) {
    static_assert(COMPACT_CHUNK == CpShape<CP_ITEMS_PER_LANE>::CHUNK, "the host sizes the look-back state and chunk_lo by the chunk");
    unsigned long long* const ph = (unsigned long long*)phases;
    const char* const e = test_hook("TKAMD_LB_PATIENCE");
    const uint32_t patience = e ? (uint32_t)std::max(0, atoi(e)) : LB_PATIENCE;
    if (ph)
        hipLaunchKernelGGL((k_compact<CP_ITEMS_PER_LANE, true>), dim3(grid), dim3(CP_NT), 0, st, tok0, (const uint4*)rows, (const uint4*)cache_rows, tmp_ids, n_pretok, state, n_tok, pt_tokoff, ids,
                           chunk_lo, doc_pt, n_docs, tok_offsets, ph, patience, tok_b8);
    else
        hipLaunchKernelGGL(k_compact<CP_ITEMS_PER_LANE>, dim3(grid), dim3(CP_NT), 0, st, tok0, (const uint4*)rows, (const uint4*)cache_rows, tmp_ids, n_pretok, state, n_tok, pt_tokoff, ids,
                           chunk_lo, doc_pt, n_docs, tok_offsets, ph, patience, tok_b8);
}
```

### tokenizers_amd/csrc/kernels/pretok_gpt2.hip

```cpp

constexpr int PT_TILE = 2048;
constexpr int PT_HALO = 8;
constexpr int PT_R = PT_TILE + 2 * PT_HALO;

constexpr uint32_t IF_CLS = 3;
constexpr uint32_t IF_LEAD = 4;
constexpr uint32_t IF_DOC = 8;
constexpr uint32_t IF_VALID = 16;
constexpr uint32_t IF_SP = 32;
constexpr int IF_LEN_SHIFT = 6;


__device__ __forceinline__ uint32_t cls_lns(uint32_t cp, const uint16_t* __restrict__ uc1, const uint8_t* __restrict__ uc2) {
    if (cp < 0x80u) {
        uint32_t lower = cp | 0x20u;
        if (lower - 'a' < 26u) return 1;
        if (cp - '0' < 10u) return 2;
        if (cp == 0x20u || cp - 9u < 5u) return 3;
        return 0;
    }
    uint32_t f = uc_flags(cp, uc1, uc2);
    return (f & UC_ONIG_L) ? 1u : (f & UC_ONIG_N) ? 2u : (f & UC_ONIG_S) ? 3u : 0u;
}

__device__ __forceinline__ uint32_t utf8_at(const uint8_t* sb, int k, uint32_t* len) {
    uint32_t b = sb[k];
    if (b < 0x80u) { *len = 1; return b; }
    if (b < 0xE0u) { *len = 2; return ((b & 0x1Fu) << 6) | (sb[k + 1] & 0x3Fu); }
    if (b < 0xF0u) { *len = 3; return ((b & 0x0Fu) << 12) | ((sb[k + 1] & 0x3Fu) << 6) | (sb[k + 2] & 0x3Fu); }
    *len = 4;
    return ((b & 0x07u) << 18) | ((sb[k + 1] & 0x3Fu) << 12) | ((sb[k + 2] & 0x3Fu) << 6) | (sb[k + 3] & 0x3Fu);
}

constexpr int SQ_MAIN = 48, SQ_HALO = 8, SQ_LUT_COPIES = 1;
struct __attribute__((packed, aligned(8))) SqChunk { uint32_t a, b, c, d; };

template <int COPIES = SQ_LUT_COPIES, bool LEAD = false>
__global__ __launch_bounds__(256) void k_pretok_gpt2_seq(const uint8_t* __restrict__ text, int64_t n_bytes_host,
                                                         const int64_t* __restrict__ len_dev,
                                                         const unsigned long long* __restrict__ docmask,
                                                         const uint16_t* __restrict__ uc1, const uint8_t* __restrict__ uc2,
                                                         unsigned long long* __restrict__ startmask, unsigned long long* __restrict__ leadmask) {
    __shared__ Gpt2Flags lut[COPIES * 256];
    {
        const Gpt2Flags f = gpt2_byte_flags(threadIdx.x);
#pragma unroll
        for (int c = 0; c < COPIES; ++c) lut[c * 256 + threadIdx.x] = f;
    }
    __syncthreads();
    const int64_t n_bytes = len_dev ? *len_dev : n_bytes_host;
    const int64_t n_words_host = (n_bytes_host >> 6) + 1;
    const int64_t Lg = (int64_t)blockIdx.x * 256 + threadIdx.x;
    uint64_t ld = 0;
    const unsigned long long out = gpt2_lane_starts(text, n_bytes, n_words_host, (const uint64_t*)docmask,
                                                    lut + (threadIdx.x & (COPIES - 1)) * 256, Lg, uc1, uc2, LEAD ? &ld : nullptr);
    const unsigned long long nxt = __shfl_down(out, 1, 64);
    const int q = (int)(threadIdx.x & 3);
    if (q < 3) {
        const int64_t word = 3 * (Lg >> 2) + q;
        if (word < n_words_host) startmask[word] = (out >> (16 * q)) | (nxt << (SQ_MAIN - 16 * q));
    }
    if constexpr (LEAD) {
        const unsigned long long ld_n = __shfl_down((unsigned long long)ld, 1, 64);
        if (q < 3) {
            const int64_t word = 3 * (Lg >> 2) + q;
            if (word < n_words_host) leadmask[word] = ((unsigned long long)ld >> (16 * q)) | (ld_n << (SQ_MAIN - 16 * q));
        }
    }
}
```

### tokenizers_amd/csrc/kernels/scan_emit.hip

```cpp

constexpr int WS_PER = 8;
__global__ __launch_bounds__(256) void k_words_reduce(const unsigned long long* __restrict__ mask, int64_t n_words,
                                                      uint32_t* __restrict__ bsum, const int64_t* __restrict__ len_dev) {
    __shared__ uint32_t sm[4];
    if (len_dev) n_words = min(n_words, (*len_dev >> 6) + 2);
    const int64_t w0 = ((int64_t)blockIdx.x * 256 + threadIdx.x) * WS_PER;
    uint32_t v = 0;
    if (w0 + WS_PER <= n_words) {
        const ulonglong2* const q = (const ulonglong2*)(mask + w0);
#pragma unroll
        for (int k = 0; k < WS_PER / 2; ++k) { const ulonglong2 m = q[k]; v += (uint32_t)(__popcll(m.x) + __popcll(m.y)); }
    } else {
        for (int k = 0; k < WS_PER; ++k) v += (w0 + k < n_words) ? (uint32_t)__popcll(mask[w0 + k]) : 0u;
    }
    uint32_t tot;
    block256_excl_scan(v, sm, &tot);
    if (threadIdx.x == 0) bsum[blockIdx.x] = tot;
}

__global__ __launch_bounds__(256) void k_words_down(const unsigned long long* __restrict__ mask, int64_t n_words,
                                                    const uint32_t* __restrict__ bsum, uint32_t* __restrict__ wprefix, const int64_t* __restrict__ len_dev,
                                                    uint32_t* __restrict__ tile_w) {
    __shared__ uint32_t sm[4];
    if (len_dev) n_words = min(n_words, (*len_dev >> 6) + 2);
    if ((int64_t)blockIdx.x * 256 * WS_PER >= n_words) return;
    const int64_t w0 = ((int64_t)blockIdx.x * 256 + threadIdx.x) * WS_PER;
    uint32_t c[WS_PER], v = 0;
    const bool whole = w0 + WS_PER <= n_words;
    if (whole) {
        const ulonglong2* const q = (const ulonglong2*)(mask + w0);
#pragma unroll
        for (int k = 0; k < WS_PER / 2; ++k) { const ulonglong2 m = q[k]; c[2 * k] = (uint32_t)__popcll(m.x); c[2 * k + 1] = (uint32_t)__popcll(m.y); }
    } else {
#pragma unroll
        for (int k = 0; k < WS_PER; ++k) c[k] = (w0 + k < n_words) ? (uint32_t)__popcll(mask[w0 + k]) : 0u;
    }
#pragma unroll
    for (int k = 0; k < WS_PER; ++k) v += c[k];
    uint32_t tot;
    uint32_t run = bsum[blockIdx.x] + block256_excl_scan(v, sm, &tot);
    if (tile_w) {
        uint32_t ex = run;
#pragma unroll
        for (int k = 0; k < WS_PER; ++k) {
            const uint32_t kk = (ex + (uint32_t)META_TILE - 1u) / (uint32_t)META_TILE;
            if (c[k] && kk * (uint32_t)META_TILE < ex + c[k]) tile_w[kk] = (uint32_t)(w0 + k);
            ex += c[k];
        }
    }
    if (whole) {
        uint4 o0, o1;
        o0.x = run; run += c[0]; o0.y = run; run += c[1]; o0.z = run; run += c[2]; o0.w = run; run += c[3];
        o1.x = run; run += c[4]; o1.y = run; run += c[5]; o1.z = run; run += c[6]; o1.w = run;
        ((uint4*)(wprefix + w0))[0] = o0;
        ((uint4*)(wprefix + w0))[1] = o1;
    } else {
#pragma unroll
        for (int k = 0; k < WS_PER; ++k) { if (w0 + k < n_words) wprefix[w0 + k] = run; run += c[k]; }
    }
}

__global__ __launch_bounds__(256) void k_emit_pretok(const unsigned long long* __restrict__ startmask,
                                                     const uint32_t* __restrict__ wprefix, int64_t n_bytes,
                                                     const int64_t* __restrict__ len_dev,
                                                     const int64_t* __restrict__ n_pretok,
                                                     uint32_t* __restrict__ pt_start) {
    const int lane = lane_id();
    const int64_t wave = (int64_t)blockIdx.x * 4 + (threadIdx.x >> 6);
    if (wave == 0 && lane == 0) pt_start[*n_pretok] = (uint32_t)(len_dev ? *len_dev : n_bytes);
    if (len_dev) n_bytes = min(n_bytes, *len_dev);
    const int64_t n_words = (n_bytes + 63) >> 6;
    const int64_t w0 = wave * 64;
    if (w0 >= n_words) return;
    const int64_t wi = w0 + lane;
    const unsigned long long mw = (wi < n_words) ? startmask[wi] : 0ull;
    const uint32_t pw = (wi < n_words) ? wprefix[wi] : 0u;
    const uint32_t mlo = (uint32_t)mw, mhi = (uint32_t)(mw >> 32);
    if (__ballot(mw != 0ull) == 0ull) return;
    const int kmax = (int)min((int64_t)64, n_words - w0);
    const unsigned long long below = (1ull << lane) - 1ull;
    for (int k = 0; k < kmax; ++k) {
        const unsigned long long m = ((unsigned long long)(uint32_t)__builtin_amdgcn_readlane((int)mhi, k) << 32) |
                                     (uint32_t)__builtin_amdgcn_readlane((int)mlo, k);
        const uint32_t base = (uint32_t)__builtin_amdgcn_readlane((int)pw, k);
        if ((m >> lane) & 1ull) pt_start[base + (uint32_t)__popcll(m & below)] = (uint32_t)(((w0 + k) << 6) + lane);
    }
}

__global__ __launch_bounds__(256) void k_emit_pretok_end(const unsigned long long* __restrict__ startmask,
                                                         const unsigned long long* __restrict__ endmask,
                                                         const uint32_t* __restrict__ wprefix, int64_t n_bytes, const int64_t* __restrict__ len_dev,
                                                         uint32_t* __restrict__ pt_end) {
    const int lane = lane_id();
    const int64_t wave = (int64_t)blockIdx.x * 4 + (threadIdx.x >> 6);
    if (len_dev) n_bytes = min(n_bytes, *len_dev);
    const int64_t n_words = (n_bytes >> 6) + 1;
    const int64_t w0 = wave * 64;
    if (w0 >= n_words) return;
    const int64_t wi = w0 + lane;
    const unsigned long long ms = (wi < n_words) ? startmask[wi] : 0ull, me = (wi < n_words) ? endmask[wi] : 0ull;
    const uint32_t pw = (wi < n_words) ? wprefix[wi] : 0u;
    const uint32_t slo = (uint32_t)ms, shi = (uint32_t)(ms >> 32), elo = (uint32_t)me, ehi = (uint32_t)(me >> 32);
    if (__ballot(me != 0ull) == 0ull) return;
    const int kmax = (int)min((int64_t)64, n_words - w0);
    const unsigned long long below = (1ull << lane) - 1ull;
    for (int k = 0; k < kmax; ++k) {
        const unsigned long long e = ((unsigned long long)(uint32_t)__builtin_amdgcn_readlane((int)ehi, k) << 32) |
                                     (uint32_t)__builtin_amdgcn_readlane((int)elo, k);
        if (e == 0ull) continue;
        const unsigned long long m = ((unsigned long long)(uint32_t)__builtin_amdgcn_readlane((int)shi, k) << 32) |
                                     (uint32_t)__builtin_amdgcn_readlane((int)slo, k);
        const uint32_t base = (uint32_t)__builtin_amdgcn_readlane((int)pw, k);
        if ((e >> lane) & 1ull) pt_end[base + (uint32_t)__popcll(m & below) - 1u] = (uint32_t)(((w0 + k) << 6) + lane);
    }
}

__device__ __forceinline__ uint32_t doc_first_rank(int64_t g, int64_t n_bytes, const unsigned long long* __restrict__ startmask,
                                                   const uint32_t* __restrict__ wprefix, const int64_t* __restrict__ n_pretok) {
    if (g >= n_bytes) return (uint32_t)*n_pretok;
    const unsigned long long m = startmask[g >> 6];
    const int b = (int)(g & 63);
    return wprefix[g >> 6] + (uint32_t)__popcll(m & ((1ull << b) - 1ull));
}
__global__ void k_doc_first_pretok(const int64_t* __restrict__ doc_off, int64_t n_docs, int64_t n_bytes,
                                   const unsigned long long* __restrict__ startmask, const uint32_t* __restrict__ wprefix,
                                   const int64_t* __restrict__ n_pretok, uint32_t* __restrict__ doc_pt, uint32_t* __restrict__ chunk_lo, uint32_t chunk,
                                   const int* __restrict__ err, int64_t* __restrict__ san) {
    int64_t d = (int64_t)blockIdx.x * blockDim.x + threadIdx.x;
    if (d > n_docs) return;
    const bool bad = san && (*err & ERR_BAD_OFFSETS) != 0;
    const int64_t g = bad ? (d == n_docs ? n_bytes : 0) : doc_off[d];
    if (san) san[d] = g;
    const uint32_t r = doc_first_rank(g, n_bytes, startmask, wprefix, n_pretok);
    doc_pt[d] = r;
    const uint32_t c_hi = r / chunk;
    uint32_t c = d ? doc_first_rank(bad ? 0 : doc_off[d - 1], n_bytes, startmask, wprefix, n_pretok) / chunk + 1u : 0u;
    for (; c <= c_hi; ++c) chunk_lo[c] = (uint32_t)d;
    if (d == n_docs) chunk_lo[c_hi + 1u] = (uint32_t)n_docs + 1u;
}

__global__ void k_add_u32(uint32_t* __restrict__ data, int64_t n, uint32_t delta) {
    int64_t i = (int64_t)blockIdx.x * blockDim.x + threadIdx.x;
    if (i < n) data[i] += delta;
}
__global__ void k_add_i64(int64_t* __restrict__ data, int64_t n, int64_t delta) {
    int64_t i = (int64_t)blockIdx.x * blockDim.x + threadIdx.x;
    if (i < n) data[i] += delta;
}
```

### tokenizers_amd/csrc/kernels/scan_util.hip

```cpp

__global__ __launch_bounds__(256) void k_u32_reduce(const uint32_t* __restrict__ v, int64_t n, uint32_t* __restrict__ bsum) {
    __shared__ uint32_t sm[4];
    int64_t i = (int64_t)blockIdx.x * 256 + threadIdx.x;
    uint32_t x = (i < n) ? v[i] : 0u, tot;
    block256_excl_scan(x, sm, &tot);
    if (threadIdx.x == 0) bsum[blockIdx.x] = tot;
}

__global__ __launch_bounds__(1024) void k_scan_single(uint32_t* __restrict__ data, int64_t n_host,
                                                      const int64_t* __restrict__ n_dev, int64_t div,
                                                      int64_t* __restrict__ total_out) {
    __shared__ uint32_t sm[16];
    __shared__ uint64_t carry_s;
    int64_t n = n_dev ? ((*n_dev + div - 1) / div) : n_host;
    const int lane = lane_id(), wave = (int)(threadIdx.x >> 6);
    if (threadIdx.x == 0) carry_s = 0;
    __syncthreads();
    for (int64_t base = 0; base < n; base += 1024) {
        int64_t i = base + threadIdx.x;
        uint32_t v = (i < n) ? data[i] : 0u;
        uint32_t inc = wave_incl_scan(v);
        if (lane == 63) sm[wave] = inc;
        __syncthreads();
        uint32_t wbase = 0, tot = 0;
        for (int w = 0; w < 16; ++w) {
            uint32_t s = sm[w];
            if (w < wave) wbase += s;
            tot += s;
        }
        uint64_t carry = carry_s;
        if (i < n) data[i] = (uint32_t)(carry + wbase + inc - v);
        __syncthreads();
        if (threadIdx.x == 0) carry_s = carry + tot;
        __syncthreads();
    }
    if (threadIdx.x == 0) *total_out = (int64_t)carry_s;
}

__global__ __launch_bounds__(256) void k_zero_regions(ZeroRegions z) {
    if (z.only_if && z.only_if[0] == 0u) return;
    const size_t extent = z.only_if ? (size_t)z.only_if[1] : ~(size_t)0;
    const size_t stride = (size_t)gridDim.x * 256;
    for (int r = 0; r < z.n; ++r) {
        uint4* const p = (uint4*)(r == 0 ? z.p[0] : r == 1 ? z.p[1] : r == 2 ? z.p[2] : r == 3 ? z.p[3] : r == 4 ? z.p[4] : z.p[5]);
        const size_t n = min(extent, (size_t)(r == 0 ? z.n16[0] : r == 1 ? z.n16[1] : r == 2 ? z.n16[2] : r == 3 ? z.n16[3] : r == 4 ? z.n16[4] : z.n16[5]));
        for (size_t i = (size_t)blockIdx.x * 256 + threadIdx.x; i < n; i += stride) p[i] = make_uint4(0u, 0u, 0u, 0u);
    }
}
__global__ void k_zero_tail(uint8_t* __restrict__ p, const int64_t* __restrict__ len, int n, unsigned long long* __restrict__ mask, int64_t mask_words) {
    const int i = (int)threadIdx.x;
    if (blockIdx.x == 0 && i < n) p[*len + i] = 0;
    if (mask) {
        const int64_t nw = min(mask_words, (*len >> 6) + 3);
        for (int64_t w = (int64_t)blockIdx.x * blockDim.x + threadIdx.x; w < nw; w += (int64_t)gridDim.x * blockDim.x) mask[w] = 0ull;
    }
}
```

Baseline: 269.3.

## Fuse lean prologue, keep docmask clean, emit pretok sums, merge tail kernels

Several independent changes. First, on the lean GPT-2 path, the docmask is kept clean across calls: doc_first_pretok clears only the bits it set, so the full docmask zeroing can be skipped, and zeroing, doc-start marking and CSR validation are fused into a single prologue launch. Second, the GPT-2 pretok kernel writes per-group popcount sums so the mask scan can build block sums from them instead of re-reading the mask. Third, the merge64 and huge-merge passes are fused into one tail kernel that splits its blocks by role. These cut launch count and memory traffic, at the cost of cross-call state (dirty flags, stamps) that must stay correct.

```diff
diff --git a/tokenizers_amd/csrc/capi/handle.cpp b/tokenizers_amd/csrc/capi/handle.cpp
--- a/tokenizers_amd/csrc/capi/handle.cpp
+++ b/tokenizers_amd/csrc/capi/handle.cpp
@@ -40,6 +40,10 @@
     int64_t last_n_inputs = -1;
     DevBuf w_inp_off;
     DevBuf w_mask_dirty;
+    bool docmask_dirty = true;
+    DevBuf w_gsum;
+    DevBuf w_csr_bad;
+    uint64_t csr_stamp = 0;
     int64_t last_n_bytes = 0;
     uint32_t last_flags = 0;
     tkamd_device_result last_result{};
diff --git a/tokenizers_amd/csrc/capi/pipeline.cpp b/tokenizers_amd/csrc/capi/pipeline.cpp
--- a/tokenizers_amd/csrc/capi/pipeline.cpp
+++ b/tokenizers_amd/csrc/capi/pipeline.cpp
@@ -30,7 +30,9 @@
 void reserve_workspace(tkamd_tokenizer* t, Workspace* w, int64_t n_bytes, int64_t n_docs, uint32_t flags, bool want_meta) {
     int64_t W = (n_bytes >> 6) + 2;
     size_t N = (size_t)n_bytes;
+    const size_t docmask_cap = w->w_docmask.cap;
     w->w_docmask.reserve(W * 8);
+    if (w->w_docmask.cap != docmask_cap) w->docmask_dirty = true;
     w->w_startmask.reserve(W * 8);
     w->w_wprefix.reserve(W * 4);
     w->w_bsum.reserve((W / 256 + 2) * 4);
@@ -119,11 +121,18 @@
     }
     w->last_used_claims = use_claims;
     size_t claim_slots = 0;
+    const bool lean = n_bytes > 0 && hm.at[0].size() == 0 && hm.at[1].size() == 0 && hm.norm == NORM_NONE && !prefix_space &&
+                      (hm.pretok == PT_BYTELEVEL_GPT2 || hm.pretok == PT_BYTELEVEL_NOREGEX);
+    const char* const clean_hook = test_hook("TKAMD_DOCMASK_CLEAN");
+    const bool keep_clean = lean && !(clean_hook && clean_hook[0] == '0');
+    const bool one_prologue = keep_clean && !w->docmask_dirty;
+    if (n_bytes > 0) w->docmask_dirty = true;
     const size_t cstate_bytes = (((size_t)n_x / (size_t)COMPACT_CHUNK + 4) * 8 + 15) & ~(size_t)15;
     {
         ZeroRegions z{};
         z.add(sc, SC_SLOTS * 8);
-        if (!(len_bound && (hm.norm == NORM_BERT || metaspace))) z.add(w->w_docmask.p, (size_t)(W + 1) * 8);
+        if (keep_clean) { if (!one_prologue) z.add(w->w_docmask.p, w->w_docmask.cap & ~(size_t)15); }
+        else if (!(len_bound && (hm.norm == NORM_BERT || metaspace))) z.add(w->w_docmask.p, (size_t)(W + 1) * 8);
         z.add(w->w_qcount.p, (size_t)QCNT_WORDS * 4);
         z.add(w->w_cstate.p, cstate_bytes);
         if (hm.pretok == PT_LLAMA3 && split_rule_fast(hm.split_rule)) {
@@ -139,7 +148,17 @@
             w->w_claim_rows.reserve(claim_slots * 16);
             z.add(w->w_claims.p, claim_slots * 16);
         }
-        launch_zero_regions(st, t->n_cu * 4, z);
+        if (one_prologue) {
+            if (!w->w_csr_bad.p) {
+                w->w_csr_bad.reserve(16);
+                HIP_CHECK(hipMemsetAsync(w->w_csr_bad.p, 0, 16, st));
+            }
+            pf.begin("mark_doc_starts");
+            launch_lean_prologue(st, d_doc_off, n_docs, n_bytes, w->w_docmask.as<ull>(), w->w_csr_bad.as<ull>(), ++w->csr_stamp, t->n_cu * 4, z);
+            pf.end();
+        } else {
+            launch_zero_regions(st, t->n_cu * 4, z);
+        }
     }
     out->d_ids = w->w_ids.as<uint32_t>();
     out->d_tok_offsets = w->w_tok_offsets.as<int64_t>();
@@ -158,8 +177,6 @@
     w->last_inp_off = d_inp_off;
     w->last_n_inputs = n_inputs;
     w->w_doc_off.reserve((size_t)(n_docs + 2) * 8);
-    const bool lean = n_bytes > 0 && hm.at[0].size() == 0 && hm.at[1].size() == 0 && hm.norm == NORM_NONE && !prefix_space &&
-                      (hm.pretok == PT_BYTELEVEL_GPT2 || hm.pretok == PT_BYTELEVEL_NOREGEX);
     const int64_t* const raw_doc_off = d_doc_off;
     if (!lean) {
         pf.begin("validate_csr");
@@ -757,10 +774,12 @@
         piece_n_dev = d_nseg;
     }
 
-    pf.begin("mark_doc_starts");
-    launch_mark_doc_starts_n(st, lean ? raw_doc_off : x_doc_off, n_docs, n_x, x_len_dev, w->w_docmask.as<ull>(), d_err);
-    if (matchmask) launch_mask_or(st, w->w_docmask.as<ull>(), w->w_hardmask.as<ull>(), W, n_match);
-    pf.end();
+    if (!one_prologue) {
+        pf.begin("mark_doc_starts");
+        launch_mark_doc_starts_n(st, lean ? raw_doc_off : x_doc_off, n_docs, n_x, x_len_dev, w->w_docmask.as<ull>(), d_err);
+        if (matchmask) launch_mask_or(st, w->w_docmask.as<ull>(), w->w_hardmask.as<ull>(), W, n_match);
+        pf.end();
+    }
 
     uint32_t* pt_end = nullptr;
     bool has_end = false;
@@ -775,16 +794,26 @@
         pf.begin("doc_first_pretok");
         launch_doc_first_pretok(st, lean ? raw_doc_off : x_doc_off, n_docs, n_x, w->w_startmask.as<ull>(), w->w_wprefix.as<uint32_t>(),
                                 d_npretok, w->w_doc_pt.as<uint32_t>(), w->w_chunk_lo.as<uint32_t>(),
-                                lean ? d_err : nullptr, lean ? w->w_doc_off.as<int64_t>() : nullptr);
-        pf.end();
+                                lean ? d_err : nullptr, lean ? w->w_doc_off.as<int64_t>() : nullptr, keep_clean ? w->w_docmask.as<ull>() : nullptr,
+                                one_prologue ? w->w_csr_bad.as<ull>() : nullptr, w->csr_stamp);
+        pf.end();
+        if (keep_clean) w->docmask_dirty = false;
     };
+    uint32_t* gsum = nullptr;
+    int64_t n_gsum = 0;
     if (hm.pretok == PT_BYTELEVEL_GPT2) {
         pf.begin("pretok_gpt2_seq");
         if (off_mode == TKAMD_OFFSETS_CHAR && x_text == d_text && !x_len_dev && n_x == n_bytes) {
             w->w_leadmask.reserve((size_t)(W0 + 1) * 8);
             lead_done = true;
         }
-        launch_pretok_gpt2(st, x_text, n_x, x_len_dev, w->w_docmask.as<ull>(), t->dt.uc1, t->dt.uc2, w->w_startmask.as<ull>(), lead_done ? w->w_leadmask.as<ull>() : nullptr);
+        const char* const sums_hook = test_hook("TKAMD_PRETOK_SUMS");
+        if (lean && !matchmask && !x_len_dev && !(sums_hook && sums_hook[0] == '0')) {
+            n_gsum = (int64_t)pretok_gpt2_sums(n_x);
+            w->w_gsum.reserve((size_t)n_gsum * 4 + 16);
+            gsum = w->w_gsum.as<uint32_t>();
+        }
+        launch_pretok_gpt2(st, x_text, n_x, x_len_dev, w->w_docmask.as<ull>(), t->dt.uc1, t->dt.uc2, w->w_startmask.as<ull>(), lead_done ? w->w_leadmask.as<ull>() : nullptr, gsum);
         pf.end();
     } else if (hm.pretok == PT_LLAMA3) {
         w->w_endmask.reserve((size_t)(W + 1) * 8);
@@ -827,7 +856,7 @@
         meta_masks = want_meta && !(hm.char_bpe && !hm.unk_configured && !hm.byte_fallback);
         if (meta_masks) w->w_tile_w.reserve(((size_t)n_x / META_TILE + 4) * 4);
         launch_mask_scan(st, w->w_startmask.as<ull>(), W, w->w_bsum.as<uint32_t>(), w->w_wprefix.as<uint32_t>(), d_npretok, len_bound ? x_len_dev : nullptr,
-                         meta_masks ? w->w_tile_w.as<uint32_t>() : nullptr);
+                         meta_masks ? w->w_tile_w.as<uint32_t>() : nullptr, gsum, n_gsum);
         pf.end();
         after_masks();
     }
@@ -948,13 +977,22 @@
             launch_bpe_merge(st, lds16 ? t->n_cu : grid, lds16 ? 5 : 1, mdt, x_text, plan.v[0], w->w_rows.p, w->w_tmp_ids.as<uint32_t>(), tmp_end);
             pf.end();
         }
-        pf.begin("bpe_merge64");
-        launch_bpe_merge(st, grid, 64, mdt, x_text, plan.v[2], w->w_rows.p, w->w_tmp_ids.as<uint32_t>(), tmp_end);
-        pf.end();
+        const char* const tail_hook = test_hook("TKAMD_MERGE_TAIL");
+        const bool tail = !(tail_hook && tail_hook[0] == '0');
+        if (!tail) {
+            pf.begin("bpe_merge64");
+            launch_bpe_merge(st, grid, 64, mdt, x_text, plan.v[2], w->w_rows.p, w->w_tmp_ids.as<uint32_t>(), tmp_end);
+            pf.end();
+        }
         pf.begin("bpe_merge_long");
-        launch_bpe_merge_long(st, t->n_cu, mdt, x_text, plan.v[3], w->w_rows.p,
-                              w->w_tmp_ids.as<uint32_t>(), tmp_end, w->w_list_huge.as<uint32_t>(), d_counters + CNT_LISTH, w->w_huge.as<uint32_t>(),
-                              (unsigned long long)(huge_possible ? huge_words : 0), (unsigned long long*)(sc + SC_HUGE_USED), d_err);
+        if (tail)
+            launch_bpe_merge_long_tail(st, t->n_cu, grid, mdt, x_text, plan.v[2], plan.v[3], w->w_rows.p,
+                                       w->w_tmp_ids.as<uint32_t>(), tmp_end, w->w_list_huge.as<uint32_t>(), d_counters + CNT_LISTH, w->w_huge.as<uint32_t>(),
+                                       (unsigned long long)(huge_possible ? huge_words : 0), (unsigned long long*)(sc + SC_HUGE_USED), d_err);
+        else
+            launch_bpe_merge_long(st, t->n_cu, mdt, x_text, plan.v[3], w->w_rows.p,
+                                  w->w_tmp_ids.as<uint32_t>(), tmp_end, w->w_list_huge.as<uint32_t>(), d_counters + CNT_LISTH, w->w_huge.as<uint32_t>(),
+                                  (unsigned long long)(huge_possible ? huge_words : 0), (unsigned long long*)(sc + SC_HUGE_USED), d_err);
         pf.end();
         }
         if (wc.keys) {
diff --git a/tokenizers_amd/csrc/kernels.hpp b/tokenizers_amd/csrc/kernels.hpp
--- a/tokenizers_amd/csrc/kernels.hpp
+++ b/tokenizers_amd/csrc/kernels.hpp
@@ -272,16 +272,20 @@
                             unsigned long long* docmask, int* err);
 void launch_validate_csr(hipStream_t st, const int64_t* doc_off, int64_t n_docs, int64_t n_bytes, int* err, int64_t* san);
 void launch_pretok_gpt2(hipStream_t st, const uint8_t* text, int64_t n_bytes, const int64_t* len_dev, const unsigned long long* docmask,
-                        const uint16_t* uc1, const uint8_t* uc2, unsigned long long* startmask, unsigned long long* leadmask = nullptr);
+                        const uint16_t* uc1, const uint8_t* uc2, unsigned long long* startmask, unsigned long long* leadmask = nullptr, uint32_t* gsum = nullptr);
+size_t pretok_gpt2_sums(int64_t n_bytes);
 void launch_mask_scan(hipStream_t st, const unsigned long long* mask, int64_t n_words, uint32_t* bsum, uint32_t* wprefix,
-                      int64_t* total, const int64_t* len_dev = nullptr, uint32_t* tile_w = nullptr);
+                      int64_t* total, const int64_t* len_dev = nullptr, uint32_t* tile_w = nullptr, const uint32_t* gsum = nullptr, int64_t n_gsum = 0);
 void launch_emit_pretok(hipStream_t st, const unsigned long long* startmask, const uint32_t* wprefix, int64_t n_bytes,
                         const int64_t* len_dev, const int64_t* n_pretok, uint32_t* pt_start);
 void launch_prefix_space(hipStream_t st, const uint8_t* text, const int64_t* seg_off, int64_t n_bound, const int64_t* n_dev, const unsigned long long* matchmask,
                          uint32_t* need, uint32_t* bsum, int64_t* xseg_off, int64_t* x_len, uint8_t* xtext, uint32_t* nos, uint32_t* noe, int grid);
 void launch_doc_first_pretok(hipStream_t st, const int64_t* doc_off, int64_t n_docs, int64_t n_bytes,
                              const unsigned long long* startmask, const uint32_t* wprefix, const int64_t* n_pretok, uint32_t* doc_pt, uint32_t* chunk_lo,
-                             const int* err = nullptr, int64_t* san = nullptr);
+                             int* err = nullptr, int64_t* san = nullptr, unsigned long long* docmask_clean = nullptr, const unsigned long long* csr_bad = nullptr,
+                             unsigned long long stamp = 0);
+void launch_lean_prologue(hipStream_t st, const int64_t* doc_off, int64_t n_docs, int64_t n_bytes, unsigned long long* docmask, unsigned long long* csr_bad,
+                          unsigned long long stamp, int zero_grid, const ZeroRegions& z);
 void launch_lookup(hipStream_t st, int grid, const DevTables& t, const uint8_t* text, int64_t n_bytes, const int64_t* len_dev,
                    const unsigned long long* startmask, const unsigned long long* endmask, const uint32_t* wprefix, uint32_t* tok0,
                    const QueuePlan& plan, int* err, const unsigned long long* matchmask, const void* hot, const WordCache& wc,
@@ -359,6 +363,9 @@
 void launch_bpe_merge_long(hipStream_t st, int grid, const DevTables& t, const uint8_t* text, const QView& v, void* rows,
                            uint32_t* tmp_ids, uint32_t* tmp_end, uint32_t* list_huge, uint32_t* n_huge,
                            uint32_t* scratch, unsigned long long scratch_words, unsigned long long* scratch_used, int* err);
+void launch_bpe_merge_long_tail(hipStream_t st, int grid, int grid64, const DevTables& t, const uint8_t* text, const QView& v64, const QView& v, void* rows,
+                                uint32_t* tmp_ids, uint32_t* tmp_end, uint32_t* list_huge, uint32_t* n_huge,
+                                uint32_t* scratch, unsigned long long scratch_words, unsigned long long* scratch_used, int* err);
 void launch_bpe_merge_long_only(hipStream_t st, int grid, const DevTables& t, const uint8_t* text, const QView& v, void* rows, uint32_t* tmp_ids, uint32_t* tmp_end,
                                 uint32_t* list_huge, uint32_t* n_huge);
 void launch_word_cache_insert(hipStream_t st, int grid, const DevTables& t, const uint8_t* text, const QView& v, const void* rows, const WordCache& wc);
diff --git a/tokenizers_amd/csrc/kernels/bpe.hip b/tokenizers_amd/csrc/kernels/bpe.hip
--- a/tokenizers_amd/csrc/kernels/bpe.hip
+++ b/tokenizers_amd/csrc/kernels/bpe.hip
@@ -80,15 +80,14 @@
 }
 
 template <int G>
-__global__ __launch_bounds__(256) void k_bpe_merge(DevTables t, const uint8_t* __restrict__ text, QView v, uint4* __restrict__ rows,
-                                                   uint32_t* __restrict__ tmp_ids, uint32_t* __restrict__ tmp_end) {
+__device__ __forceinline__ void bpe_merge_body(const DevTables& t, const uint8_t* __restrict__ text, const QView& v, uint4* __restrict__ rows,
+                                               uint32_t* __restrict__ tmp_ids, uint32_t* __restrict__ tmp_end, uint32_t* s_qpre, uint32_t block, uint32_t n_blocks) {
     constexpr int GPW = 64 / G;
-    __shared__ uint32_t s_qpre[NSQ + 1];
     const int lane = lane_id();
     const int sub = lane / G, c = lane % G, gbase = sub * G;
     const uint32_t n = qview_prefix(v, s_qpre);
-    const uint32_t wave_global = blockIdx.x * 4 + (threadIdx.x >> 6);
-    const uint32_t n_waves = gridDim.x * 4;
+    const uint32_t wave_global = block * 4 + (threadIdx.x >> 6);
+    const uint32_t n_waves = n_blocks * 4;
     for (uint32_t base = wave_global * GPW; base < n; base += n_waves * GPW) {
         uint32_t item = base + sub;
         bool valid = item < n;
@@ -150,6 +149,12 @@
             }
         }
     }
+}
+template <int G>
+__global__ __launch_bounds__(256) void k_bpe_merge(DevTables t, const uint8_t* __restrict__ text, QView v, uint4* __restrict__ rows,
+                                                   uint32_t* __restrict__ tmp_ids, uint32_t* __restrict__ tmp_end) {
+    __shared__ uint32_t s_qpre[NSQ + 1];
+    bpe_merge_body<G>(t, text, v, rows, tmp_ids, tmp_end, s_qpre, blockIdx.x, gridDim.x);
 }
 template __global__ void k_bpe_merge<64>(DevTables, const uint8_t*, QView, uint4*, uint32_t*, uint32_t*);
 
diff --git a/tokenizers_amd/csrc/kernels/bpe_huge.hip b/tokenizers_amd/csrc/kernels/bpe_huge.hip
--- a/tokenizers_amd/csrc/kernels/bpe_huge.hip
+++ b/tokenizers_amd/csrc/kernels/bpe_huge.hip
@@ -11,12 +11,12 @@
     return best;
 }
 
-__global__ __launch_bounds__(256) void k_bpe_merge_huge(DevTables t, const uint8_t* __restrict__ text,
-                                                        const QItem* __restrict__ q, uint4* __restrict__ rows, uint32_t row_base,
-                                                        const uint32_t* __restrict__ list, const uint32_t* __restrict__ n_list,
-                                                        uint32_t* __restrict__ tmp_ids, uint32_t* __restrict__ tmp_end,
-                                                        uint32_t* __restrict__ scratch, unsigned long long scratch_words,
-                                                        unsigned long long* __restrict__ scratch_used, int* __restrict__ err) {
+__device__ __forceinline__ void bpe_merge_huge_body(const DevTables& t, const uint8_t* __restrict__ text,
+                                                    const QItem* __restrict__ q, uint4* __restrict__ rows, uint32_t row_base,
+                                                    const uint32_t* __restrict__ list, const uint32_t* __restrict__ n_list,
+                                                    uint32_t* __restrict__ tmp_ids, uint32_t* __restrict__ tmp_end,
+                                                    uint32_t* __restrict__ scratch, unsigned long long scratch_words,
+                                                    unsigned long long* __restrict__ scratch_used, int* __restrict__ err, uint32_t block, uint32_t n_blocks) {
     __shared__ unsigned long long red[4];
     __shared__ unsigned long long base_s;
     __shared__ uint32_t touched[3];
@@ -25,7 +25,7 @@
     const int tid = (int)threadIdx.x;
     __shared__ uint32_t first_s;
     const uint32_t n = *n_list;
-    for (uint32_t item = blockIdx.x; item < n; item += gridDim.x) {
+    for (uint32_t item = block; item < n; item += n_blocks) {
         const uint32_t p = list[item];
         const QItem it = q[p];
         const uint32_t s = it.s, len = qitem_len(it.len);
@@ -166,3 +166,23 @@
         if (tid == 0) rows[row_base + p] = make_uint4((cnt_s ? first_s : 0u) | (ROW_CNT_MORE << ROW_CNT_SHIFT), s, cnt_s, 0u);
     }
 }
+__global__ __launch_bounds__(256) void k_bpe_merge_huge(DevTables t, const uint8_t* __restrict__ text,
+                                                        const QItem* __restrict__ q, uint4* __restrict__ rows, uint32_t row_base,
+                                                        const uint32_t* __restrict__ list, const uint32_t* __restrict__ n_list,
+                                                        uint32_t* __restrict__ tmp_ids, uint32_t* __restrict__ tmp_end,
+                                                        uint32_t* __restrict__ scratch, unsigned long long scratch_words,
+                                                        unsigned long long* __restrict__ scratch_used, int* __restrict__ err) {
+    bpe_merge_huge_body(t, text, q, rows, row_base, list, n_list, tmp_ids, tmp_end, scratch, scratch_words, scratch_used, err, blockIdx.x, gridDim.x);
+}
+__global__ __launch_bounds__(256) void k_bpe_merge_tail(DevTables t, const uint8_t* __restrict__ text, QView v64, QView vlong, uint4* __restrict__ rows,
+                                                        const uint32_t* __restrict__ list, const uint32_t* __restrict__ n_list,
+                                                        uint32_t* __restrict__ tmp_ids, uint32_t* __restrict__ tmp_end,
+                                                        uint32_t* __restrict__ scratch, unsigned long long scratch_words,
+                                                        unsigned long long* __restrict__ scratch_used, int* __restrict__ err, uint32_t huge_blocks) {
+    if (blockIdx.x < huge_blocks) {
+        bpe_merge_huge_body(t, text, (const QItem*)vlong.q, rows, vlong.row_base, list, n_list, tmp_ids, tmp_end, scratch, scratch_words, scratch_used, err, blockIdx.x, huge_blocks);
+    } else {
+        __shared__ uint32_t s_qpre[NSQ + 1];
+        bpe_merge_body<64>(t, text, v64, rows, tmp_ids, tmp_end, s_qpre, blockIdx.x - huge_blocks, gridDim.x - huge_blocks);
+    }
+}
diff --git a/tokenizers_amd/csrc/kernels/documents.hip b/tokenizers_amd/csrc/kernels/documents.hip
--- a/tokenizers_amd/csrc/kernels/documents.hip
+++ b/tokenizers_amd/csrc/kernels/documents.hip
@@ -1,4 +1,5 @@
 
+__device__ __forceinline__ bool doc_start_marked(int64_t g, int64_t g1, int64_t n_bytes) { return g >= 0 && g1 >= g && g1 <= n_bytes && g < n_bytes; }
 __global__ void k_mark_doc_starts(const int64_t* __restrict__ doc_off, int64_t n_docs, int64_t n_bytes_host,
                                   const int64_t* __restrict__ len_dev,
                                   unsigned long long* __restrict__ docmask, int* __restrict__ err) {
@@ -13,7 +14,23 @@
     }
     int64_t g1 = doc_off[d + 1];
     if (g < 0 || g1 < g || g1 > n_bytes) { atomicOr(err, ERR_BAD_OFFSETS); return; }
-    if (docmask && g < n_bytes) atomicOr(&docmask[g >> 6], 1ull << (g & 63));
+    if (docmask && doc_start_marked(g, g1, n_bytes)) atomicOr(&docmask[g >> 6], 1ull << (g & 63));
+}
+__global__ __launch_bounds__(256) void k_lean_prologue(const int64_t* __restrict__ doc_off, int64_t n_docs, int64_t n_bytes,
+                                                       unsigned long long* __restrict__ docmask, unsigned long long* __restrict__ csr_bad,
+                                                       unsigned long long stamp, uint32_t mark_blocks, ZeroRegions z) {
+    if (blockIdx.x >= mark_blocks) { zero_regions_role(z, blockIdx.x - mark_blocks, gridDim.x - mark_blocks); return; }
+    const int64_t d = (int64_t)blockIdx.x * 256 + threadIdx.x;
+    if (d > n_docs) return;
+    const int64_t g = doc_off[d];
+    bool bad = d == 0 && g != 0;
+    if (d == n_docs) bad = bad || g != n_bytes;
+    else {
+        const int64_t g1 = doc_off[d + 1];
+        bad = bad || g < 0 || g1 < g || g1 > n_bytes;
+        if (doc_start_marked(g, g1, n_bytes)) atomicOr(&docmask[g >> 6], 1ull << (g & 63));
+    }
+    if (bad) *csr_bad = stamp;
 }
 __global__ void k_sanitize_csr(const int64_t* __restrict__ doc_off, int64_t n_docs, int64_t n_bytes, const int* __restrict__ err,
                                int64_t* __restrict__ san) {
diff --git a/tokenizers_amd/csrc/kernels/launch.hip b/tokenizers_amd/csrc/kernels/launch.hip
--- a/tokenizers_amd/csrc/kernels/launch.hip
+++ b/tokenizers_amd/csrc/kernels/launch.hip
@@ -13,15 +13,20 @@
     hipLaunchKernelGGL(k_sanitize_csr, dim3(blocks_for(n_docs + 1, 256)), dim3(256), 0, st, doc_off, n_docs, n_bytes, (const int*)err, san);
 }
 void launch_pretok_gpt2(hipStream_t st, const uint8_t* text, int64_t n_bytes, const int64_t* len_dev, const unsigned long long* docmask,
-                        const uint16_t* uc1, const uint8_t* uc2, unsigned long long* startmask, unsigned long long* leadmask) {
-    if (leadmask) hipLaunchKernelGGL((k_pretok_gpt2_seq<SQ_LUT_COPIES, true>), dim3(blocks_for(n_bytes + 1, 256 * SQ_MAIN)), dim3(256), 0, st, text, n_bytes, len_dev, docmask, uc1, uc2, startmask, leadmask);
-    else hipLaunchKernelGGL((k_pretok_gpt2_seq<SQ_LUT_COPIES, false>), dim3(blocks_for(n_bytes + 1, 256 * SQ_MAIN)), dim3(256), 0, st, text, n_bytes, len_dev, docmask, uc1, uc2, startmask, (unsigned long long*)nullptr);
-}
+                        const uint16_t* uc1, const uint8_t* uc2, unsigned long long* startmask, unsigned long long* leadmask, uint32_t* gsum) {
+    if (leadmask) hipLaunchKernelGGL((k_pretok_gpt2_seq<SQ_LUT_COPIES, true>), dim3(blocks_for(n_bytes + 1, 256 * SQ_MAIN)), dim3(256), 0, st, text, n_bytes, len_dev, docmask, uc1, uc2, startmask, leadmask, gsum);
+    else hipLaunchKernelGGL((k_pretok_gpt2_seq<SQ_LUT_COPIES, false>), dim3(blocks_for(n_bytes + 1, 256 * SQ_MAIN)), dim3(256), 0, st, text, n_bytes, len_dev, docmask, uc1, uc2, startmask, (unsigned long long*)nullptr, gsum);
+}
+size_t pretok_gpt2_sums(int64_t n_bytes) { return (size_t)blocks_for(n_bytes + 1, 256 * SQ_MAIN) * (SQ_WG_WORDS / PT_SUM_WORDS); }
 void launch_mask_scan(hipStream_t st, const unsigned long long* mask, int64_t n_words, uint32_t* bsum, uint32_t* wprefix,
-                      int64_t* total, const int64_t* len_dev, uint32_t* tile_w) {
+                      int64_t* total, const int64_t* len_dev, uint32_t* tile_w, const uint32_t* gsum, int64_t n_gsum) {
     unsigned nb = blocks_for(n_words, 256 * WS_PER);
-    hipLaunchKernelGGL(k_words_reduce, dim3(nb), dim3(256), 0, st, mask, n_words, bsum, len_dev);
-    hipLaunchKernelGGL(k_scan_single, dim3(1), dim3(1024), 0, st, bsum, (int64_t)nb, (const int64_t*)nullptr, (int64_t)1, total);
+    if (gsum) {
+        hipLaunchKernelGGL(k_scan_groups, dim3(1), dim3(1024), 0, st, gsum, n_gsum, bsum, (int64_t)nb, total);
+    } else {
+        hipLaunchKernelGGL(k_words_reduce, dim3(nb), dim3(256), 0, st, mask, n_words, bsum, len_dev);
+        hipLaunchKernelGGL(k_scan_single, dim3(1), dim3(1024), 0, st, bsum, (int64_t)nb, (const int64_t*)nullptr, (int64_t)1, total);
+    }
     hipLaunchKernelGGL(k_words_down, dim3(nb), dim3(256), 0, st, mask, n_words, (const uint32_t*)bsum, wprefix, len_dev, tile_w);
 }
 void launch_emit_pretok(hipStream_t st, const unsigned long long* startmask, const uint32_t* wprefix, int64_t n_bytes,
@@ -30,9 +35,15 @@
 }
 void launch_doc_first_pretok(hipStream_t st, const int64_t* doc_off, int64_t n_docs, int64_t n_bytes,
                              const unsigned long long* startmask, const uint32_t* wprefix, const int64_t* n_pretok, uint32_t* doc_pt, uint32_t* chunk_lo,
-                             const int* err, int64_t* san) {
+                             int* err, int64_t* san, unsigned long long* docmask_clean, const unsigned long long* csr_bad, unsigned long long stamp) {
     hipLaunchKernelGGL(k_doc_first_pretok, dim3(blocks_for(n_docs + 1, 256)), dim3(256), 0, st, doc_off, n_docs, n_bytes, startmask, wprefix, n_pretok, doc_pt, chunk_lo,
-                       (uint32_t)COMPACT_CHUNK, err, san);
+                       (uint32_t)COMPACT_CHUNK, err, san, docmask_clean, csr_bad, stamp);
+}
+void launch_lean_prologue(hipStream_t st, const int64_t* doc_off, int64_t n_docs, int64_t n_bytes, unsigned long long* docmask, unsigned long long* csr_bad,
+                          unsigned long long stamp, int zero_grid, const ZeroRegions& z) {
+    const unsigned mark_blocks = blocks_for(n_docs + 1, 256);
+    hipLaunchKernelGGL(k_lean_prologue, dim3(mark_blocks + (z.n > 0 ? (unsigned)zero_grid : 0u)), dim3(256), 0, st, doc_off, n_docs, n_bytes, docmask, csr_bad, stamp,
+                       (uint32_t)mark_blocks, z);
 }
 
 void launch_lookup(hipStream_t st, int grid, const DevTables& t, const uint8_t* text, int64_t n_bytes, const int64_t* len_dev,
@@ -300,6 +311,13 @@
     hipLaunchKernelGGL(k_bpe_merge_huge, dim3(64), dim3(256), 0, st, t, text, (const QItem*)v.q, (uint4*)rows, v.row_base, (const uint32_t*)list_huge,
                        (const uint32_t*)n_huge, tmp_ids, tmp_end, scratch, scratch_words, scratch_used, err);
 }
+void launch_bpe_merge_long_tail(hipStream_t st, int grid, int grid64, const DevTables& t, const uint8_t* text, const QView& v64, const QView& v, void* rows,
+                                uint32_t* tmp_ids, uint32_t* tmp_end, uint32_t* list_huge, uint32_t* n_huge,
+                                uint32_t* scratch, unsigned long long scratch_words, unsigned long long* scratch_used, int* err) {
+    hipLaunchKernelGGL(k_bpe_merge_long, dim3(grid), dim3(256), long_kernel_lds_bytes(), st, t, text, v, (uint4*)rows, tmp_ids, tmp_end, list_huge, n_huge);
+    hipLaunchKernelGGL(k_bpe_merge_tail, dim3(64 + grid64), dim3(256), 0, st, t, text, v64, v, (uint4*)rows, (const uint32_t*)list_huge, (const uint32_t*)n_huge,
+                       tmp_ids, tmp_end, scratch, scratch_words, scratch_used, err, 64u);
+}
 void launch_bpe_merge_long_only(hipStream_t st, int grid, const DevTables& t, const uint8_t* text, const QView& v, void* rows, uint32_t* tmp_ids, uint32_t* tmp_end,
                                 uint32_t* list_huge, uint32_t* n_huge) {
     hipLaunchKernelGGL(k_bpe_merge_long, dim3(grid), dim3(256), long_kernel_lds_bytes(), st, t, text, v, (uint4*)rows, tmp_ids, tmp_end, list_huge, n_huge);
diff --git a/tokenizers_amd/csrc/kernels/pretok_gpt2.hip b/tokenizers_amd/csrc/kernels/pretok_gpt2.hip
--- a/tokenizers_amd/csrc/kernels/pretok_gpt2.hip
+++ b/tokenizers_amd/csrc/kernels/pretok_gpt2.hip
@@ -33,6 +33,9 @@
 }
 
 constexpr int SQ_MAIN = 48, SQ_HALO = 8, SQ_LUT_COPIES = 1;
+constexpr int PT_SUM_WORDS = 64;
+constexpr int SQ_WG_WORDS = 256 * SQ_MAIN / 64;
+static_assert(SQ_WG_WORDS % PT_SUM_WORDS == 0 && SQ_WG_WORDS <= 256, "a workgroup writes whole sums, a lane per word");
 struct __attribute__((packed, aligned(8))) SqChunk { uint32_t a, b, c, d; };
 
 template <int COPIES = SQ_LUT_COPIES, bool LEAD = false>
@@ -40,7 +43,8 @@
                                                          const int64_t* __restrict__ len_dev,
                                                          const unsigned long long* __restrict__ docmask,
                                                          const uint16_t* __restrict__ uc1, const uint8_t* __restrict__ uc2,
-                                                         unsigned long long* __restrict__ startmask, unsigned long long* __restrict__ leadmask) {
+                                                         unsigned long long* __restrict__ startmask, unsigned long long* __restrict__ leadmask,
+                                                         uint32_t* __restrict__ gsum) {
     __shared__ Gpt2Flags lut[COPIES * 256];
     {
         const Gpt2Flags f = gpt2_byte_flags(threadIdx.x);
@@ -56,9 +60,20 @@
                                                     lut + (threadIdx.x & (COPIES - 1)) * 256, Lg, uc1, uc2, LEAD ? &ld : nullptr);
     const unsigned long long nxt = __shfl_down(out, 1, 64);
     const int q = (int)(threadIdx.x & 3);
+    uint32_t bits = 0;
     if (q < 3) {
         const int64_t word = 3 * (Lg >> 2) + q;
-        if (word < n_words_host) startmask[word] = (out >> (16 * q)) | (nxt << (SQ_MAIN - 16 * q));
+        const unsigned long long m = (out >> (16 * q)) | (nxt << (SQ_MAIN - 16 * q));
+        if (word < n_words_host) { startmask[word] = m; bits = (uint32_t)__popcll(m); }
+    }
+    if (gsum) {
+        __shared__ uint32_t s_bits[SQ_WG_WORDS];
+        if (q < 3) s_bits[3 * (threadIdx.x >> 2) + q] = bits;
+        __syncthreads();
+        if (threadIdx.x < SQ_WG_WORDS) {
+            const uint32_t inc = wave_incl_scan(s_bits[threadIdx.x]);
+            if ((threadIdx.x & 63) == 63) gsum[(size_t)blockIdx.x * (SQ_WG_WORDS / PT_SUM_WORDS) + (threadIdx.x >> 6)] = inc;
+        }
     }
     if constexpr (LEAD) {
         const unsigned long long ld_n = __shfl_down((unsigned long long)ld, 1, 64);
diff --git a/tokenizers_amd/csrc/kernels/scan_emit.hip b/tokenizers_amd/csrc/kernels/scan_emit.hip
--- a/tokenizers_amd/csrc/kernels/scan_emit.hip
+++ b/tokenizers_amd/csrc/kernels/scan_emit.hip
@@ -16,6 +16,43 @@
     uint32_t tot;
     block256_excl_scan(v, sm, &tot);
     if (threadIdx.x == 0) bsum[blockIdx.x] = tot;
+}
+
+constexpr int SCAN_GROUP = 256 * WS_PER / PT_SUM_WORDS;
+static_assert(SCAN_GROUP * PT_SUM_WORDS == 256 * WS_PER && SCAN_GROUP % 4 == 0, "whole sums per scan block, read four at a time");
+__global__ __launch_bounds__(1024) void k_scan_groups(const uint32_t* __restrict__ gsum, int64_t n_gsum, uint32_t* __restrict__ bsum, int64_t n,
+                                                      int64_t* __restrict__ total_out) {
+    __shared__ uint32_t sm[16];
+    __shared__ uint64_t carry_s;
+    const int lane = lane_id(), wave = (int)(threadIdx.x >> 6);
+    if (threadIdx.x == 0) carry_s = 0;
+    __syncthreads();
+    for (int64_t base = 0; base < n; base += 1024) {
+        const int64_t i = base + threadIdx.x, g0 = i * SCAN_GROUP;
+        uint32_t v = 0;
+        if (i < n && g0 + SCAN_GROUP <= n_gsum) {
+            const uint4* const q = (const uint4*)(gsum + g0);
+#pragma unroll
+            for (int k = 0; k < SCAN_GROUP / 4; ++k) { const uint4 x = q[k]; v += x.x + x.y + x.z + x.w; }
+        } else if (i < n) {
+            for (int k = 0; k < SCAN_GROUP; ++k) v += (g0 + k < n_gsum) ? gsum[g0 + k] : 0u;
+        }
+        const uint32_t inc = wave_incl_scan(v);
+        if (lane == 63) sm[wave] = inc;
+        __syncthreads();
+        uint32_t wbase = 0, tot = 0;
+        for (int w = 0; w < 16; ++w) {
+            const uint32_t s = sm[w];
+            if (w < wave) wbase += s;
+            tot += s;
+        }
+        const uint64_t carry = carry_s;
+        if (i < n) bsum[i] = (uint32_t)(carry + wbase + inc - v);
+        __syncthreads();
+        if (threadIdx.x == 0) carry_s = carry + tot;
+        __syncthreads();
+    }
+    if (threadIdx.x == 0) *total_out = (int64_t)carry_s;
 }
 
 __global__ __launch_bounds__(256) void k_words_down(const unsigned long long* __restrict__ mask, int64_t n_words,
@@ -125,10 +162,16 @@
 __global__ void k_doc_first_pretok(const int64_t* __restrict__ doc_off, int64_t n_docs, int64_t n_bytes,
                                    const unsigned long long* __restrict__ startmask, const uint32_t* __restrict__ wprefix,
                                    const int64_t* __restrict__ n_pretok, uint32_t* __restrict__ doc_pt, uint32_t* __restrict__ chunk_lo, uint32_t chunk,
-                                   const int* __restrict__ err, int64_t* __restrict__ san) {
+                                   int* err, int64_t* __restrict__ san, unsigned long long* __restrict__ docmask_clean,
+                                   const unsigned long long* __restrict__ csr_bad, unsigned long long stamp) {
     int64_t d = (int64_t)blockIdx.x * blockDim.x + threadIdx.x;
     if (d > n_docs) return;
-    const bool bad = san && (*err & ERR_BAD_OFFSETS) != 0;
+    const bool bad = san && (csr_bad ? *csr_bad == stamp : (*err & ERR_BAD_OFFSETS) != 0);
+    if (csr_bad && bad && d == 0) atomicOr(err, ERR_BAD_OFFSETS);
+    if (docmask_clean && d < n_docs) {
+        const int64_t g0 = doc_off[d];
+        if (doc_start_marked(g0, doc_off[d + 1], n_bytes)) docmask_clean[g0 >> 6] = 0ull;
+    }
     const int64_t g = bad ? (d == n_docs ? n_bytes : 0) : doc_off[d];
     if (san) san[d] = g;
     const uint32_t r = doc_first_rank(g, n_bytes, startmask, wprefix, n_pretok);
diff --git a/tokenizers_amd/csrc/kernels/scan_util.hip b/tokenizers_amd/csrc/kernels/scan_util.hip
--- a/tokenizers_amd/csrc/kernels/scan_util.hip
+++ b/tokenizers_amd/csrc/kernels/scan_util.hip
@@ -37,16 +37,17 @@
     if (threadIdx.x == 0) *total_out = (int64_t)carry_s;
 }
 
-__global__ __launch_bounds__(256) void k_zero_regions(ZeroRegions z) {
+__device__ __forceinline__ void zero_regions_role(const ZeroRegions& z, size_t block, size_t n_blocks) {
     if (z.only_if && z.only_if[0] == 0u) return;
     const size_t extent = z.only_if ? (size_t)z.only_if[1] : ~(size_t)0;
-    const size_t stride = (size_t)gridDim.x * 256;
+    const size_t stride = n_blocks * 256;
     for (int r = 0; r < z.n; ++r) {
         uint4* const p = (uint4*)(r == 0 ? z.p[0] : r == 1 ? z.p[1] : r == 2 ? z.p[2] : r == 3 ? z.p[3] : r == 4 ? z.p[4] : z.p[5]);
         const size_t n = min(extent, (size_t)(r == 0 ? z.n16[0] : r == 1 ? z.n16[1] : r == 2 ? z.n16[2] : r == 3 ? z.n16[3] : r == 4 ? z.n16[4] : z.n16[5]));
-        for (size_t i = (size_t)blockIdx.x * 256 + threadIdx.x; i < n; i += stride) p[i] = make_uint4(0u, 0u, 0u, 0u);
+        for (size_t i = block * 256 + threadIdx.x; i < n; i += stride) p[i] = make_uint4(0u, 0u, 0u, 0u);
     }
 }
+__global__ __launch_bounds__(256) void k_zero_regions(ZeroRegions z) { zero_regions_role(z, blockIdx.x, gridDim.x); }
 __global__ void k_zero_tail(uint8_t* __restrict__ p, const int64_t* __restrict__ len, int n, unsigned long long* __restrict__ mask, int64_t mask_words) {
     const int i = (int)threadIdx.x;
     if (blockIdx.x == 0 && i < n) p[*len + i] = 0;
```

Result: no change. 267.4 (-0.7%).
